# sangminwoo/SVOL

Hardware: AMD Instinct MI355X
Metric: frames/sec (fwd+matcher+bwd), T=32·P=196·d=256 (higher is better)
Workload: dtype bf16

## Files before the change

include/svol_hip.h:

```cpp
#ifndef SVOL_HIP_H
#define SVOL_HIP_H

#include <stdint.h>

#ifdef __cplusplus
extern "C" {
#endif

#define SVOL_F32 0
#define SVOL_BF16 1
#define SVOL_F16 2

#define SVOL_OK 0
#define SVOL_E_INVALID (-1)
#define SVOL_E_UNSUPPORTED (-2)
#define SVOL_E_LAUNCH (-3)

#define SVOL_ACT_NONE 0
#define SVOL_ACT_RELU 1
#define SVOL_ACT_GELU 2
#define SVOL_ACT_SIGMOID 3
#define SVOL_ACT_GELU_D 5
#define SVOL_ACT_RELU_RES 4

int svol_abi_version(void);
const char* svol_strerror(int code);

int svol_cast(const void* src, int dtype_src, void* dst, int dtype_dst, int64_t n, void* stream);
int svol_cast_transpose(const float* src, void* dst, void* dstT, int dtype, int64_t R, int64_t C, void* stream);
int svol_cast_transpose_multi(const void* descs, int32_t n_desc, int64_t total_tiles, int dtype, void* stream);
int svol_cast_split(const float* src, int64_t ld_src, void* dst_hilo, int64_t R, int64_t C, void* stream);

int svol_adamw_flat(float* p, const float* g, float* m, float* v, int64_t n, float lr, float beta1, float beta2, float eps,
                    float weight_decay, int64_t step, float grad_scale, void* stream);
int svol_adamw_flat_zero(float* p, float* g, float* m, float* v, int64_t n, float lr, float beta1, float beta2, float eps,
                         float weight_decay, int64_t step, float grad_scale, void* stream);
int svol_grad_finite(const float* g, int64_t n, float* scaler_state, void* stream);
int svol_adamw_flat_scaled(float* p, const float* g, float* m, float* v, int64_t n, float lr, float beta1, float beta2, float eps,
                           float weight_decay, float grad_mul, const float* scaler_state, void* stream);
int svol_loss_scaler_update(float* scaler_state, float growth_factor, float backoff_factor, int64_t growth_interval, float min_scale,
                            float max_scale, void* stream);
int svol_sgd_flat(float* p, const float* g, float* buf, int64_t n, float lr, float momentum, float weight_decay, float grad_scale,
                  void* stream);
int svol_sgd_flat_zero(float* p, float* g, float* buf, int64_t n, float lr, float momentum, float weight_decay, float grad_scale,
                       void* stream);
int svol_sgd_flat_scaled(float* p, const float* g, float* buf, int64_t n, float lr, float momentum, float weight_decay, float grad_mul,
                         const float* scaler_state, void* stream);
int svol_adam_flat(float* p, const float* g, float* m, float* v, int64_t n, float lr, float beta1, float beta2, float eps,
                   float weight_decay, int64_t step, float grad_scale, void* stream);
int svol_adam_flat_zero(float* p, float* g, float* m, float* v, int64_t n, float lr, float beta1, float beta2, float eps,
                        float weight_decay, int64_t step, float grad_scale, void* stream);
int svol_adam_flat_scaled(float* p, const float* g, float* m, float* v, int64_t n, float lr, float beta1, float beta2, float eps,
                          float weight_decay, float grad_mul, const float* scaler_state, void* stream);
int64_t svol_grad_sqnorm_ws_bytes(int64_t n);
int svol_grad_sqnorm(const float* g, int64_t n, float* ws, float* out, void* stream);
int svol_grad_clip_state(const float* sq, int32_t nb, float grad_mul, float max_norm, float loss_scale, int64_t steps_taken,
                         float* scaler_state, float* state_out, void* stream);
int svol_sgd_flat_grouped(float* p, float* g, float* buf, int64_t n, const int32_t* seg_end, const int32_t* seg_group, int32_t nseg,
                          const float* hyper, int32_t ngroups, const float* state, float grad_mul, int zero, void* stream);
int svol_adam_flat_grouped(float* p, float* g, float* m, float* v, int64_t n, const int32_t* seg_end, const int32_t* seg_group,
                           int32_t nseg, const float* hyper, int32_t ngroups, const float* state, const float* step_count,
                           float grad_mul, int zero, void* stream);
int svol_adamw_flat_grouped(float* p, float* g, float* m, float* v, int64_t n, const int32_t* seg_end, const int32_t* seg_group,
                            int32_t nseg, const float* hyper, int32_t ngroups, const float* state, const float* step_count,
                            float grad_mul, int zero, void* stream);
int svol_flat_step_advance(float* step_count, const float* state, void* stream);

int svol_gemm_nt(const void* A, int64_t lda, const void* A2, int64_t n_split, const void* B, int64_t ldb,
                 void* C, int64_t ldc, const float* bias, const float* colscale, int act, void* pre_act_out,
                 int64_t ldp, const void* residual, int64_t ldr, int out_f32, int64_t M, int64_t N, int64_t K,
                 int dtype, void* stream);
int svol_gemm_nt_split(const void* A, int64_t lda, const void* W_hilo, int64_t ldw, void* C, int64_t ldc, const float* bias,
                       int64_t M, int64_t N, int64_t K, void* stream);
int svol_gemm_nt_dgelu(const void* A, int64_t lda, const void* B, int64_t ldb, void* C, int64_t ldc,
                       const void* pre, int64_t ldp, float* colsum, int64_t M, int64_t N, int64_t K, int dtype,
                       void* stream);
int svol_gemm_nt_dact(const void* A, int64_t lda, const void* B, int64_t ldb, void* C, int64_t ldc,
                      const void* aux, int64_t ldaux, int act, float* colsum, int64_t M, int64_t N, int64_t K,
                      int dtype, void* stream);

int svol_gemm_tn(const void* A, int64_t lda, const void* B, int64_t ldb, float* C, int64_t ldc, float* colsum,
                 int64_t Mc, int64_t N, int64_t K, int dtype, void* stream);
#define SVOL_TN_GROUP_MAX 6
typedef struct svol_tn_problem {
    const void* A; int64_t lda;
    const void* B; int64_t ldb;
    float* C; int64_t ldc;
    float* colsum;
    int64_t Mc, N, K;
} svol_tn_problem;
int svol_gemm_tn_grouped(const svol_tn_problem* problems, int32_t n, int dtype, void* stream);
int svol_colsum(const void* X, int64_t ldx, float* out, int64_t M, int64_t N, int dtype, void* stream);
int svol_act_bwd(const void* dy, const void* aux, void* dpre, int act, int64_t n, int dtype, void* stream);

int svol_layernorm_fwd(const void* x, int x_f32, const float* gamma, const float* beta, float* y32, void* y,
                       void* ypos, const void* pos, int64_t pos_rows, float* mean, float* rstd, int64_t M, int64_t D,
                       float dropout_p, uint64_t seed, const int64_t* seed_offset_dev, int dtype, void* stream);
int svol_layernorm_bwd(const float* dy32, const void* dy, const void* dy2, const void* x, int x_f32,
                       const float* gamma, const float* mean, const float* rstd, float* dx32, void* dx,
                       float* dgamma, float* dbeta, float* dx_colsum, int64_t M, int64_t D, float dropout_p,
                       uint64_t seed, const int64_t* seed_offset_dev, int dtype, void* stream);

int svol_dropout(const void* x, void* y, int64_t n, int64_t row_len, float p, uint64_t seed, int dtype, void* stream);
int svol_dropout_add(const float* t32, const float* res32, float* out32, int64_t n, int64_t row_len, float p, uint64_t seed, void* stream);
int svol_dropout_sd(const void* x, void* y, int64_t n, int64_t row_len, float p, uint64_t seed, const int64_t* seed_step_dev, int dtype,
                    void* stream);
int svol_dropout_add_sd(const float* t32, const float* res32, float* out32, int64_t n, int64_t row_len, float p, uint64_t seed,
                        const int64_t* seed_step_dev, void* stream);

int svol_posenc_sine(const float* mask, void* pos, int64_t B, int64_t L, int64_t D, int dtype, void* stream);

int64_t svol_attn_ws_bytes(int64_t B, int64_t H, int64_t Lq, int64_t Lk, int64_t dh);
int svol_attn_fwd(const void* q, int64_t ldq, const void* k, int64_t ldk, const void* v, int64_t ldv, void* o,
                  int64_t ldo, float* lse2, const float* kbias, int64_t B, int64_t H, int64_t Lq, int64_t Lk,
                  int64_t dh, float scale, float q_premul, void* ws, int64_t ws_bytes, int dtype, void* stream);
int svol_attn_bwd(const void* q, int64_t ldq, const void* k, int64_t ldk, const void* v, int64_t ldv, const void* o,
                  int64_t ldo, const void* d_o, int64_t lddo, const float* lse2, float* delta, const float* kbias,
                  void* dq, int64_t lddq, void* dk, int64_t lddk, void* dv, int64_t lddv, int64_t B, int64_t H,
                  int64_t Lq, int64_t Lk, int64_t dh, float scale, float q_premul, void* ws, int64_t ws_bytes,
                  int dtype, void* stream);

#define SVOL_ATTN_DQ_PREZEROED 1
int64_t svol_attn_bwd_sp_image_bytes(int64_t B, int64_t H, int64_t Lq, int64_t Lk, int64_t dh, int64_t ws_bytes, int dtype);
int svol_attn_bwd_zero_ws(void* ws, int64_t ws_bytes, int64_t B, int64_t H, int64_t Lq, int64_t Lk, int64_t dh, int dtype, void* stream);
int svol_attn_bwd_ex(const void* q, int64_t ldq, const void* k, int64_t ldk, const void* v, int64_t ldv, const void* o,
                     int64_t ldo, const void* d_o, int64_t lddo, const float* lse2, float* delta, const float* kbias,
                     void* dq, int64_t lddq, void* dk, int64_t lddk, void* dv, int64_t lddv, int64_t B, int64_t H,
                     int64_t Lq, int64_t Lk, int64_t dh, float scale, float q_premul, void* ws, int64_t ws_bytes,
                     int dtype, int flags, void* ev_prep, void* stream);

int svol_attn_fwd_dropout(const void* q, int64_t ldq, const void* k, int64_t ldk, const void* v, int64_t ldv, void* o,
                          int64_t ldo, float* lse2, const float* kbias, int64_t B, int64_t H, int64_t Lq, int64_t Lk,
                          int64_t dh, float scale, float q_premul, void* ws, int64_t ws_bytes, float dropout_p, uint64_t seed,
                          int dtype, void* stream);
int svol_attn_bwd_dropout(const void* q, int64_t ldq, const void* k, int64_t ldk, const void* v, int64_t ldv, const void* o,
                          int64_t ldo, const void* d_o, int64_t lddo, const float* lse2, float* delta, const float* kbias,
                          void* dq, int64_t lddq, void* dk, int64_t lddk, void* dv, int64_t lddv, int64_t B, int64_t H,
                          int64_t Lq, int64_t Lk, int64_t dh, float scale, float q_premul, void* ws, int64_t ws_bytes,
                          float dropout_p, uint64_t seed, int dtype, void* stream);
int svol_attn_fwd_dropout_sd(const void* q, int64_t ldq, const void* k, int64_t ldk, const void* v, int64_t ldv, void* o,
                             int64_t ldo, float* lse2, const float* kbias, int64_t B, int64_t H, int64_t Lq, int64_t Lk,
                             int64_t dh, float scale, float q_premul, void* ws, int64_t ws_bytes, float dropout_p, uint64_t seed,
                             const int64_t* seed_step_dev, int dtype, void* stream);
int svol_attn_bwd_dropout_sd(const void* q, int64_t ldq, const void* k, int64_t ldk, const void* v, int64_t ldv, const void* o,
                             int64_t ldo, const void* d_o, int64_t lddo, const float* lse2, float* delta, const float* kbias,
                             void* dq, int64_t lddq, void* dk, int64_t lddk, void* dv, int64_t lddv, int64_t B, int64_t H,
                             int64_t Lq, int64_t Lk, int64_t dh, float scale, float q_premul, void* ws, int64_t ws_bytes,
                             float dropout_p, uint64_t seed, const int64_t* seed_step_dev, int dtype, void* stream);

int svol_gate_fwd(const float* x32, const void* pos, const float* u, const float* gamma, const float* beta,
                  float* y32, void* y, void* ypos, float* a, float* mean, float* rstd, float* ws, int64_t B,
                  int64_t L, int64_t D, int64_t H, int dtype, void* stream);
int svol_gate_bwd(const float* dy32, const void* dy, const void* dy2, const float* x32, const void* pos,
                  const float* u, const float* gamma, const float* a, const float* mean, const float* rstd,
                  const float* ws, float* ws2, float* dx32, float* du, float* dgamma, float* dbeta, int64_t B,
                  int64_t L, int64_t D, int64_t H, int dtype, void* stream);

int svol_layernorm_gate_scores_fwd(const float* x32, const float* gamma, const float* beta, float* y32, void* y, void* ypos,
                                   const void* pos, float* mean, float* rstd, const float* u_next, float* scores_next,
                                   int64_t B, int64_t L, int64_t D, int64_t H, int dtype, void* stream);
int svol_gate_fwd_scored(const float* x32, const void* pos, const float* u, const float* gamma, const float* beta,
                         float* y32, void* y, void* ypos, float* a, float* mean, float* rstd, float* ws, int64_t B,
                         int64_t L, int64_t D, int64_t H, int dtype, void* stream);

int svol_gate_vectors_fwd(const float* skch, const float* W_in, const float* b_in, float* q_out, float* u_out, int64_t B, int64_t D,
                          int64_t H, void* stream);
int svol_gate_vectors_bwd(const float* du, const float* skch, const float* W_in, const float* q, float* dq_ws, float* dskch,
                          float* dW_in, float* db_in, int64_t B, int64_t D, int64_t H, void* stream);
#define SVOL_GATE_VEC_MAX_LAYERS 8
int svol_gate_vectors_fwd_multi(const float* skch, const float* const* W_in, const float* const* b_in, float* const* q_out,
                                float* const* u_out, int64_t n_layers, int64_t B, int64_t D, int64_t H, void* stream);
int svol_gate_vectors_bwd_multi(const float* const* du, const float* skch, const float* const* W_in, const float* const* q,
                                float* const* dq_ws, float* const* dskch, float* const* dW_in, float* const* db_in, int64_t n_layers,
// ... 109 lines not shown
#define SVOL_DIM_F 5
#define SVOL_DIM_DTYPE 6
#define SVOL_DIM_QDTYPE 7
#define SVOL_DIM_ATTN_WS_BYTES 8
#define SVOL_DIM_COUNT 9

#define SVOL_BLK_VIDEO_HALF 0
#define SVOL_BLK_QUERY_SELF 1
#define SVOL_BLK_QUERY_CROSS 2
const char* svol_block_slot_names(int block);
int svol_block_trace_dump(char* buf, int64_t cap);
int svol_clock_probe(uint64_t* samples, int32_t* count, int32_t max_samples, const int32_t* stop, int64_t period_us,
                     int64_t max_ms, int32_t* wall_khz, void* stream);


#define SVOL_VH_SLOTS(X) \
    X(X32) X(POS) X(U) X(G1) X(BT1) X(G2) X(BT2) X(G3) X(BT3) X(B_IN) X(B_O) X(B_FC1) X(B_FC2) X(QSCALE) \
    X(W_IN) X(WV_HILO) X(W_O) X(W_FC1) X(W_FC2) X(W_IN_T) X(W_O_T) X(W_FC1_T) X(W_FC2_T) \
    X(Y1) X(Y1POS) X(A) X(MEAN1) X(RSTD1) X(GATE_WS) X(GATE_PRE) X(U_NEXT) X(GATE_WS_NEXT) \
    X(QKV) X(O) X(LSE) X(S2) X(Y2) X(MEAN2) X(RSTD2) X(PRE) X(HID) X(S3) \
    X(MEAN3) X(RSTD3) X(M32) X(M) X(MPOS) X(Y1_32) X(Y2_32) X(ATTN_WS) \
    X(DM32) X(DM) X(DMPOS) X(DS32_3) X(DS3) X(DPRE) X(DY2) X(DS32_2) X(G2D) X(DO) X(DQKV) X(DELTA) X(DXQP) X(DXQ) X(GATE_WS2) \
    X(DX32) X(DU) \
    X(DG1) X(DBT1) X(DG2) X(DBT2) X(DG3) X(DBT3) X(DW_IN) X(DB_IN) X(DW_O) X(DB_O) X(DW_FC1) X(DB_FC1) X(DW_FC2) X(DB_FC2) \
    X(EV_A0) X(EV_A1) X(EV_CLEAN_IN) X(EV_PREP) X(ATTN_WS_NEXT) X(ZERO_STREAM) X(EV_CLEAN_OUT)
#define SVOL_QS_SLOTS(X) \
    X(O32) X(O) X(OPOS) X(QPOS) X(B_IN) X(B_O) X(G4) X(BT4) X(QSCALE) X(W_IN) X(WV_HILO) X(W_O) X(W_IN_T) X(W_O_T) \
    X(QKV) X(OA) X(LSE) X(S4) X(MEAN4) X(RSTD4) X(Y32) X(Y) X(YPOS) X(ATTN_WS) \
    X(DY32) X(DY) X(DYPOS) X(G) X(DOA) X(DQKV) X(DELTA) X(DO32) X(DXQ) X(DXQP) X(DQPOS) \
    X(DW_IN) X(DB_IN) X(DW_O) X(DB_O) X(DG4) X(DBT4)
#define SVOL_QC_SLOTS(X) \
    X(O32) X(O) X(OPOS) X(MV) X(MPOS) X(KBIAS) X(QPOS) X(B_IN) X(B_O) X(G5) X(BT5) X(B_FC1) X(B_FC2) X(G6) X(BT6) X(QSCALE) \
    X(W_INQ) X(W_INQ_T) X(W_KV) X(W_KV_T) X(WV_HILO) X(W_O) X(W_O_T) X(W_FC1) X(W_FC1_T) X(W_FC2) X(W_FC2_T) \
    X(Q) X(QC) X(KV) X(OA) X(OAQ) X(LSE) X(S5) X(Y5_32) X(Y5) X(MEAN5) X(RSTD5) X(PRE) X(HID) X(S6) X(MEAN6) X(RSTD6) \
    X(Y32) X(Y) X(YPOS) X(ATTN_WS) \
    X(DY32) X(DY) X(DYPOS) X(DS32_6) X(DS6) X(DPRE) X(DY5) X(DS32_5) X(G5D) X(DOAQ) X(DOA) X(DQC) X(DQ) X(DKV) X(DELTA) \
    X(DO32) X(DXQP) X(DMPOS) X(DMV) X(DQPOS) \
    X(DW_IN) X(DB_IN) X(DW_O) X(DB_O) X(DG5) X(DBT5) X(DW_FC1) X(DB_FC1) X(DW_FC2) X(DB_FC2) X(DG6) X(DBT6)
#define SVOL_SLOT_ENUM_VH(n) SVOL_VH_##n,
#define SVOL_SLOT_ENUM_QS(n) SVOL_QS_##n,
#define SVOL_SLOT_ENUM_QC(n) SVOL_QC_##n,
enum { SVOL_VH_SLOTS(SVOL_SLOT_ENUM_VH) SVOL_VH_COUNT };
enum { SVOL_QS_SLOTS(SVOL_SLOT_ENUM_QS) SVOL_QS_COUNT };
enum { SVOL_QC_SLOTS(SVOL_SLOT_ENUM_QC) SVOL_QC_COUNT };

int svol_video_half_fwd(const int64_t* dims, void* const* slots, void* stream);
int svol_video_half_bwd(const int64_t* dims, void* const* slots, int phase, void* stream);
int svol_video_half_wgrad(const int64_t* dims, void* const* slots, void* stream);
int svol_video_half_wgrad_part(const int64_t* dims, void* const* slots, int part, void* stream);
int svol_query_self_fwd(const int64_t* dims, void* const* slots, void* stream);
int svol_query_self_bwd(const int64_t* dims, void* const* slots, void* stream);
int svol_query_self_wgrad(const int64_t* dims, void* const* slots, void* stream);
int svol_query_cross_fwd(const int64_t* dims, void* const* slots, void* stream);
int svol_query_cross_bwd(const int64_t* dims, void* const* slots, void* stream);
int svol_query_cross_wgrad(const int64_t* dims, void* const* slots, void* stream);

#ifdef __cplusplus
}
#endif
#endif
```

svol_amd/_lib.py:

```python
from __future__ import annotations

import ctypes
import os

_HERE = os.path.dirname(os.path.abspath(__file__))
LIB_PATH = os.path.join(_HERE, 'libsvol_hip.so')

_p = ctypes.c_void_p
_i64 = ctypes.c_int64
_i32 = ctypes.c_int32
_int = ctypes.c_int
_f32 = ctypes.c_float
_u64 = ctypes.c_uint64

SIGNATURES = {
    'svol_block_trace_dump': [ctypes.c_char_p, _i64],
    'svol_lsap_solve': [_p, _i64, _i64, _p, _p],
    'svol_heads_fwd': [_p] * 13 + [_i64, _i64, _p],
    'svol_heads_bwd': [_p] * 17 + [_i64, _i64, _p],
    'svol_set_loss_bwd': [_p] * 6 + [_i64, _i64, _p],
    'svol_weighted_total': [_p, _p, _i64, _p, _p],
    'svol_weighted_total_bwd': [_p, _p, _i64, _p, _p],
    'svol_cast': [_p, _int, _p, _int, _i64, _p],
    'svol_cast_transpose': [_p, _p, _p, _int, _i64, _i64, _p],
# ... 60 lines not shown
    'svol_attn_small_fwd_h16': [_p, _i64, _p, _i64, _p, _i64, _p, _i64, _i64, _i64, _i64, _i64, _f32, _int, _p],
    'svol_attn_small_fwd_lse_h16': [_p, _i64, _p, _i64, _p, _i64, _p, _i64, _p, _i64, _i64, _i64, _i64, _f32, _int, _p],
    'svol_attn_small_bwd_h16': [_p, _i64, _p, _i64, _p, _i64, _p, _i64, _p, _i64, _p, _p, _i64, _p, _i64, _p, _i64, _i64, _i64, _i64,
                                _i64, _f32, _int, _p],
    'svol_attn_cls_fwd_h16': [_p, _i64, _p, _i64, _p, _i64, _p, _i64, _p, _i64, _i64, _i64, _i64, _f32, _int, _p],
    'svol_attn_cls_bwd_h16': [_p, _i64, _p, _i64, _p, _i64, _p, _i64, _p, _i64, _p, _p, _i64, _p, _i64, _p, _i64, _i64, _i64, _i64,
                              _i64, _f32, _int, _p],
    'svol_softmax_xent': [_p, _i64, _p, _p, _p, _i64, _p, _i64, _i64, _p],
    'svol_posenc_sine': [_p, _p, _i64, _i64, _i64, _int, _p],
    'svol_attn_ws_bytes': [_i64, _i64, _i64, _i64, _i64],
    'svol_attn_fwd': [_p, _i64, _p, _i64, _p, _i64, _p, _i64, _p, _p, _i64, _i64, _i64, _i64, _i64, _f32, _f32, _p, _i64,
                      _int, _p],
    'svol_attn_bwd': [_p, _i64, _p, _i64, _p, _i64, _p, _i64, _p, _i64, _p, _p, _p, _p, _i64, _p, _i64, _p, _i64,
                      _i64, _i64, _i64, _i64, _i64, _f32, _f32, _p, _i64, _int, _p],
    'svol_attn_bwd_ex': [_p, _i64, _p, _i64, _p, _i64, _p, _i64, _p, _i64, _p, _p, _p, _p, _i64, _p, _i64, _p, _i64,
                         _i64, _i64, _i64, _i64, _i64, _f32, _f32, _p, _i64, _int, _int, _p, _p],
    'svol_attn_bwd_sp_image_bytes': [_i64, _i64, _i64, _i64, _i64, _i64, _int],
    'svol_attn_bwd_zero_ws': [_p, _i64, _i64, _i64, _i64, _i64, _i64, _int, _p],
    'svol_attn_fwd_dropout': [_p, _i64, _p, _i64, _p, _i64, _p, _i64, _p, _p, _i64, _i64, _i64, _i64, _i64, _f32, _f32, _p, _i64,
                              _f32, _u64, _int, _p],
    'svol_attn_bwd_dropout': [_p, _i64, _p, _i64, _p, _i64, _p, _i64, _p, _i64, _p, _p, _p, _p, _i64, _p, _i64, _p, _i64,
                              _i64, _i64, _i64, _i64, _i64, _f32, _f32, _p, _i64, _f32, _u64, _int, _p],
    'svol_dropout': [_p, _p, _i64, _i64, _f32, _u64, _int, _p],
    'svol_dropout_add': [_p, _p, _p, _i64, _i64, _f32, _u64, _p],
    'svol_attn_fwd_dropout_sd': [_p, _i64, _p, _i64, _p, _i64, _p, _i64, _p, _p, _i64, _i64, _i64, _i64, _i64, _f32, _f32, _p, _i64,
                                 _f32, _u64, _p, _int, _p],
    'svol_attn_bwd_dropout_sd': [_p, _i64, _p, _i64, _p, _i64, _p, _i64, _p, _i64, _p, _p, _p, _p, _i64, _p, _i64, _p, _i64,
                                 _i64, _i64, _i64, _i64, _i64, _f32, _f32, _p, _i64, _f32, _u64, _p, _int, _p],
    'svol_dropout_sd': [_p, _p, _i64, _i64, _f32, _u64, _p, _int, _p],
    'svol_dropout_add_sd': [_p, _p, _p, _i64, _i64, _f32, _u64, _p, _p],
    'svol_gate_fwd': [_p, _p, _p, _p, _p, _p, _p, _p, _p, _p, _p, _p, _i64, _i64, _i64, _i64, _int, _p],
    'svol_gate_bwd': [_p, _p, _p, _p, _p, _p, _p, _p, _p, _p, _p, _p, _p, _p, _p, _p, _i64, _i64, _i64, _i64, _int,
                      _p],
    'svol_clock_probe': [_p, _p, _int, _p, _i64, _i64, _p, _p],
    'svol_gate_fwd_scored': [_p, _p, _p, _p, _p, _p, _p, _p, _p, _p, _p, _p, _i64, _i64, _i64, _i64, _int, _p],
    'svol_layernorm_gate_scores_fwd': [_p, _p, _p, _p, _p, _p, _p, _p, _p, _p, _p, _i64, _i64, _i64, _i64, _int, _p],
    'svol_gate_vectors_fwd': [_p, _p, _p, _p, _p, _i64, _i64, _i64, _p],
    'svol_gate_vectors_bwd': [_p, _p, _p, _p, _p, _p, _p, _p, _i64, _i64, _i64, _p],
    'svol_gate_vectors_fwd_multi': [_p, _p, _p, _p, _p, _i64, _i64, _i64, _i64, _p],
    'svol_gate_vectors_bwd_multi': [_p, _p, _p, _p, _p, _p, _p, _p, _i64, _i64, _i64, _i64, _p],
    'svol_match_cost': [_p, _p, _p, _p, _p, _p, _p, _p, _p, _i32, _f32, _f32, _f32, _p, _p],
    'svol_lsap_batched': [_p, _p, _p, _p, _p, _p, _p, _p, _i32, _i32, _p],
    'svol_set_loss': [_p, _p, _p, _p, _p, _p, _p, _p, _i32, _i32, _f32, _p, _i32, _p, _p, _i32, _p],
    'svol_video_half_fwd': [_p, _p, _p],
    'svol_video_half_bwd': [_p, _p, _int, _p],
    'svol_video_half_wgrad': [_p, _p, _p],
    'svol_video_half_wgrad_part': [_p, _p, _int, _p],
    'svol_query_self_fwd': [_p, _p, _p],
    'svol_query_self_bwd': [_p, _p, _p],
    'svol_query_self_wgrad': [_p, _p, _p],
    'svol_query_cross_fwd': [_p, _p, _p],
    'svol_query_cross_bwd': [_p, _p, _p],
    'svol_query_cross_wgrad': [_p, _p, _p],
}



class TnProblem(ctypes.Structure):
    _fields_ = [('A', _p), ('lda', _i64), ('B', _p), ('ldb', _i64), ('C', _p), ('ldc', _i64), ('colsum', _p),
                ('Mc', _i64), ('N', _i64), ('K', _i64)]


_LIB = None


class SvolHipError(RuntimeError):
    pass


def lib():
    global _LIB
    if _LIB is None:
        if not os.path.exists(LIB_PATH):
            raise SvolHipError(
                f'{LIB_PATH} not found: the SVOL hot path has no CPU fallback. '
                'Build it with `python -m svol_amd.build` (hipcc, gfx950).')
        L = ctypes.CDLL(LIB_PATH)
        L.svol_abi_version.restype = _int
        L.svol_abi_version.argtypes = []
        L.svol_strerror.restype = ctypes.c_char_p
        L.svol_strerror.argtypes = [_int]
        for name, at in SIGNATURES.items():
            f = getattr(L, name)
            f.restype = _int
            f.argtypes = at
        L.svol_attn_ws_bytes.restype = _i64
        L.svol_attn_bwd_sp_image_bytes.restype = _i64
        L.svol_grad_sqnorm_ws_bytes.restype = _i64
        L.svol_block_slot_names.restype = ctypes.c_char_p
        L.svol_block_slot_names.argtypes = [_int]
        _LIB = L
    return _LIB


def check(rc: int, name: str):
    if rc != 0:
        msg = lib().svol_strerror(rc).decode()
        raise SvolHipError(f'{name} failed: {msg} (code {rc})')
```

svol_amd/blocks.py:

```python
from __future__ import annotations

import ctypes
import math
import os
import weakref

import torch

from . import _lib, layers, ops, params, wgrad

ENABLED = os.environ.get('SVOL_NO_BLOCKS') is None
GATE_SCORES_FUSE = os.environ.get('SVOL_GATE_SCORES_FUSE') is not None
VH, QS, QC = 0, 1, 2
_F32, _BF16 = 0, 1
_ESZ = {torch.float32: 4, torch.bfloat16: 2, torch.float16: 2}
_SLOTS = {}


def _slots(block):
    m = _SLOTS.get(block)
    if m is None:
        names = _lib.lib().svol_block_slot_names(block).decode().rstrip(',').split(',')
        m = _SLOTS[block] = {n: i for i, n in enumerate(names)}
    return m
# ... 446 lines not shown
        e, R = _ESZ[qdt], B * N
        o32_, o_, opos_, qpos_ = _c(o32), _c(o), _c(opos), _c(qpos)
        assert o32_.dtype == torch.float32 and o_.dtype == qdt and opos_.dtype == qdt and qpos_.dtype == qdt
        wsb = ops.attn_ws_bytes(qdt, B, H, N, N, D // H)
        lay = _open(ctx, pl, QS, (B, N, D, H, qdt), _dims(B, 0, N, D, H, 0, qdt, qdt, wsb), len(params), o.device,
                    lambda: [('QKV', R * 3 * D * e), ('OA', R * D * e), ('LSE', B * H * N * 4), ('S4', R * D * 4), ('MEAN4', R * 4),
                             ('RSTD4', R * 4), ('Y32', R * D * 4), ('Y', R * D * e), ('YPOS', R * D * e)],
                    lambda: [('ATTN_WS', max(wsb, 16))], O32=o32_, O=o_, OPOS=opos_, QPOS=qpos_)
        _call('svol_query_self_fwd', ctx)
        ctx.shape = (B, N, D, H)
        ctx.save_for_backward(o32_, o_, opos_, qpos)
        return (lay.view(ctx.arena, 'Y32', torch.float32, (B, N, D)), lay.view(ctx.arena, 'Y', qdt, (B, N, D)),
                lay.view(ctx.arena, 'YPOS', qdt, (B, N, D)))

    @staticmethod
    def backward(ctx, dy32, dy, dypos):
        if dy32 is None and dy is None and dypos is None:
            return _no_grads(ctx, 5)
        B, N, D, H = ctx.shape
        o32_, o_, opos_, qpos = ctx.saved_tensors
        qdt = ctx.pl.qdt
        e, R = _ESZ[qdt], B * N
        gq = _qpos_target(ctx, qpos, ctx.needs_input_grad[4], N, D)
        lay, tmp, bufs, gs = _open_bwd(ctx, o_.device, lambda: [('G', R * D * e), ('DOA', R * D * e), ('DQKV', R * 3 * D * e),
                                                               ('DELTA', 3 * B * H * N * 4), ('DO32', R * D * 4), ('DXQ', R * D * e),
                                                               ('DXQP', R * D * e)], DY32=dy32, DY=dy, DYPOS=dypos)
        _call('svol_query_self_bwd', ctx)
        pg = _close_bwd(ctx, 'svol_query_self_wgrad', bufs, [ctx.arena, tmp, o_, opos_], 5)
        v = lambda n_, dt_: lay.view(tmp, n_, dt_, (B, N, D))
        return (None, v('DO32', torch.float32), v('DXQ', qdt), v('DXQP', qdt), _qpos_grad(gq, qdt)) + pg


def query_self(layer, out, qpos, dt, qdt):
    pl = plan(layer, QS, dt, qdt)
    o32, o, opos = out
    return QuerySelfFn.apply(pl, o32, o, opos, qpos, *pl.inputs(o32, o, opos))


def _qc_fwd_layout(B, N, L, D, H, F, e, qe):
    R, M = B * N, B * L
    return [('Q', R * D * qe), ('QC', R * D * e), ('KV', M * 2 * D * e), ('OA', R * D * e), ('OAQ', R * D * qe), ('LSE', B * H * N * 4),
            ('S5', R * D * 4), ('Y5_32', R * D * 4), ('Y5', R * D * qe), ('MEAN5', R * 4), ('RSTD5', R * 4), ('PRE', R * F * qe),
            ('HID', R * F * qe), ('S6', R * D * 4), ('MEAN6', R * 4), ('RSTD6', R * 4), ('Y32', R * D * 4), ('Y', R * D * qe),
            ('YPOS', R * D * qe)]


def _qc_bwd_layout(B, N, L, D, H, F, e, qe, merged):
    R, M = B * N, B * L
    return [('DS32_6', R * D * 4), ('DS6', R * D * qe), ('DPRE', R * F * qe), ('DY5', R * D * qe), ('G5D', R * D * qe), ('DOAQ', R * D * qe),
            ('DOA', R * D * e), ('DQC', R * D * e), ('DQ', R * D * qe), ('DKV', M * 2 * D * e), ('DELTA', 3 * B * H * N * 4),
            ('DO32', R * D * 4), ('DXQP', R * D * qe)] + ([] if merged else [('DMPOS', M * D * e)]) + [('DMV', M * D * e)]


class QueryCrossFn(torch.autograd.Function):

    @staticmethod
    def forward(ctx, pl, o32, o, opos, mv, mpos, kbias, qpos, merged, *params):
        B, N, D = o.shape
        L = mv.shape[1]
        layer = pl.layer()
        H, F = layer.nhead, layer.mlp2.fc1.weight.shape[0]
        dt, qdt = pl.dt, pl.qdt
        e, qe = _ESZ[dt], _ESZ[qdt]
        o32_, o_, opos_, mv_, mpos_, kb_, qpos_ = _c(o32), _c(o), _c(opos), _c(mv), _c(mpos), _c(kbias), _c(qpos)
        assert o32_.dtype == torch.float32 and o_.dtype == qdt and opos_.dtype == qdt and qpos_.dtype == qdt
        assert mv_.dtype == dt and mpos_.dtype == dt and kb_.dtype == torch.float32
        wsb = ops.attn_ws_bytes(dt, B, H, N, L, D // H)
        lay = _open(ctx, pl, QC, (B, N, L, D, H, F, dt, qdt, merged), _dims(B, L, N, D, H, F, dt, qdt, wsb), len(params), o.device,
                    lambda: _qc_fwd_layout(B, N, L, D, H, F, e, qe), lambda: [('ATTN_WS', max(wsb, 16))],
                    O32=o32_, O=o_, OPOS=opos_, MV=mv_, MPOS=mpos_, KBIAS=kb_, QPOS=qpos_)
        _call('svol_query_cross_fwd', ctx)
        ctx.shape = (B, N, L, D, H, F)
        ctx.merged = merged
        ctx.save_for_backward(o32_, o_, opos_, mv_, mpos_, kb_, qpos)
        return (lay.view(ctx.arena, 'Y32', torch.float32, (B, N, D)), lay.view(ctx.arena, 'Y', qdt, (B, N, D)),
                lay.view(ctx.arena, 'YPOS', qdt, (B, N, D)))

    @staticmethod
    def backward(ctx, dy32, dy, dypos):
        if dy32 is None and dy is None and dypos is None:
            return _no_grads(ctx, 9)
        B, N, L, D, H, F = ctx.shape
        o32_, o_, opos_, mv_, mpos_, kb_, qpos = ctx.saved_tensors
        dt, qdt = ctx.pl.dt, ctx.pl.qdt
        gq = _qpos_target(ctx, qpos, ctx.needs_input_grad[7], N, D)
        lay, tmp, bufs, gs = _open_bwd(ctx, o_.device, lambda: _qc_bwd_layout(B, N, L, D, H, F, _ESZ[dt], _ESZ[qdt], ctx.merged),
                                       DY32=dy32, DY=dy, DYPOS=dypos)
        _call('svol_query_cross_bwd', ctx)
        pg = _close_bwd(ctx, 'svol_query_cross_wgrad', bufs, [ctx.arena, tmp, opos_, mv_, mpos_], 9)
        vq = lambda n_, dt_: lay.view(tmp, n_, dt_, (B, N, D))
        vm = lambda n_: lay.view(tmp, n_, dt, (B, L, D))
        return (None, vq('DO32', torch.float32), None, vq('DXQP', qdt), vm('DMV'), None if ctx.merged else vm('DMPOS'), None,
                _qpos_grad(gq, qdt), None) + pg


def query_cross(layer, out, mv, mpos, kbias, qpos, dt, qdt):
    pl = plan(layer, QC, dt, qdt)
    o32, o, opos = out
    fn = mv.grad_fn
    merged = fn is not None and fn is mpos.grad_fn and isinstance(fn, VideoHalfFn._backward_cls)
    return QueryCrossFn.apply(pl, o32, o, opos, mv, mpos, kbias, qpos, merged, *pl.inputs(o32, opos, mv, mpos))


def trace_dump() -> str:
    buf = ctypes.create_string_buffer(1 << 20)
    _lib.check(_lib.lib().svol_block_trace_dump(buf, len(buf)), 'svol_block_trace_dump')
    return buf.value.decode()
```

svol_amd/csrc/attention.hip:

```cpp
#include "attn_call.h"

namespace {

constexpr float LOG2E = 1.4426950408889634f;

template <typename T_, int ND_> struct AT {
    typedef T_ T;
    static constexpr int ND = ND_;
    static constexpr bool H = sizeof(T) == 2;
    static_assert(ND == 2 || (ND == 1 && !H), "instances: <float, 1>, <float, 2>, <bf16_t, 2>, <f16_t, 2>");
    static constexpr int EPC = H ? 8 : 4, CPR = (H ? 4 : 8) * ND, NA1 = (H ? 2 : 4) * ND, NA2 = H ? 2 : 4;
    static constexpr int NAT_ROW = (H ? 64 : 128) * ND, TR_STRIDE = H ? 64 * 2 + 16 : 64 * 4 + 16;
    static constexpr int NAT = 64 * NAT_ROW, TR = 32 * ND * TR_STRIDE;
};

template <typename W>
__device__ __forceinline__ int nat_off(int row, int ch) {
    return row * W::NAT_ROW + ((ch ^ (row & (W::CPR - 1))) << 4);
}

template <typename W>
__device__ __forceinline__ void stage_tile(char* nat, char* tr, const typename W::T* g, int64_t ld, int row0, int limit, int dh, int tid) {
    constexpr int EPC = W::EPC, CPR = W::CPR, ST = W::TR_STRIDE;
    for (int c = tid; c < 64 * CPR; c += 256) {
// ... 518 lines not shown
    c.drop_p = dropout_p; c.drop_seed = seed; c.drop_step = seed_step_dev; c.stream = reinterpret_cast<hipStream_t>(stream);
    if (const int rc = check_call(c, false, B, H, Lq, Lk, dh, dtype)) return rc;
    if (dh > 32) return dtype == SVOL_BF16 ? fwd_launch<bf16_t, 2>(c) : dtype == SVOL_F16 ? fwd_launch<f16_t, 2>(c) : fwd_launch<float, 2>(c);
    if (svol_is16(dtype)) return (dtype == SVOL_BF16 ? svol_attn_fwd_bf16_launch : svol_attn_fwd_f16_launch)(c);
    return fwd_launch<float, 1>(c);
}
int svol_attn_fwd_dropout(const void* q, int64_t ldq, const void* k, int64_t ldk, const void* v, int64_t ldv, void* o,
                          int64_t ldo, float* lse2, const float* kbias, int64_t B, int64_t H, int64_t Lq, int64_t Lk, int64_t dh,
                          float scale, float q_premul, void* ws, int64_t ws_bytes, float dropout_p, uint64_t seed, int dtype,
                          void* stream) {
    return svol_attn_fwd_dropout_sd(q, ldq, k, ldk, v, ldv, o, ldo, lse2, kbias, B, H, Lq, Lk, dh, scale, q_premul, ws, ws_bytes,
                                    dropout_p, seed, nullptr, dtype, stream);
}
int svol_attn_fwd(const void* q, int64_t ldq, const void* k, int64_t ldk, const void* v, int64_t ldv, void* o,
                  int64_t ldo, float* lse2, const float* kbias, int64_t B, int64_t H, int64_t Lq, int64_t Lk, int64_t dh,
                  float scale, float q_premul, void* ws, int64_t ws_bytes, int dtype, void* stream) {
    return svol_attn_fwd_dropout(q, ldq, k, ldk, v, ldv, o, ldo, lse2, kbias, B, H, Lq, Lk, dh, scale, q_premul, ws, ws_bytes, 0.f, 0,
                                 dtype, stream);
}

static int attn_bwd_impl(const void* q, int64_t ldq, const void* k, int64_t ldk, const void* v, int64_t ldv, const void* o,
                         int64_t ldo, const void* d_o, int64_t lddo, const float* lse2, float* delta, const float* kbias, void* dq,
                         int64_t lddq, void* dk, int64_t lddk, void* dv, int64_t lddv, int64_t B, int64_t H, int64_t Lq, int64_t Lk,
                         int64_t dh, float scale, float q_premul, void* ws, int64_t ws_bytes, float drop_p, uint64_t drop_seed,
                         const int64_t* drop_step, int dtype, void* stream, int flags = 0, void* ev_prep = nullptr) {
    AttnCall c{};
    c.q = q; c.k = k; c.v = v; c.o = o; c.d_o = d_o; c.lse2 = const_cast<float*>(lse2); c.delta = delta; c.kbias = kbias;
    c.dq = dq; c.dk = dk; c.dv = dv;
    c.ldq = ldq; c.ldk = ldk; c.ldv = ldv; c.ldo = ldo; c.lddo = lddo; c.lddq = lddq; c.lddk = lddk; c.lddv = lddv;
    c.scale = scale; c.premul = q_premul; c.ws = static_cast<float*>(ws); c.ws_bytes = ws_bytes;
    c.drop_p = drop_p; c.drop_seed = drop_seed; c.drop_step = drop_step; c.flags = flags; c.ev_prep = ev_prep; c.stream = reinterpret_cast<hipStream_t>(stream);
    if (const int rc = check_call(c, true, B, H, Lq, Lk, dh, dtype)) return rc;
    if (dh > 32) return dtype == SVOL_BF16 ? bwd_launch<bf16_t, 2>(c) : dtype == SVOL_F16 ? bwd_launch<f16_t, 2>(c) : bwd_launch<float, 2>(c);
    if (svol_is16(dtype)) return (dtype == SVOL_BF16 ? svol_attn_bwd_bf16_launch : svol_attn_bwd_f16_launch)(c);
    return bwd_launch<float, 1>(c);
}

int svol_attn_bwd(const void* q, int64_t ldq, const void* k, int64_t ldk, const void* v, int64_t ldv, const void* o,
                  int64_t ldo, const void* d_o, int64_t lddo, const float* lse2, float* delta, const float* kbias, void* dq,
                  int64_t lddq, void* dk, int64_t lddk, void* dv, int64_t lddv, int64_t B, int64_t H, int64_t Lq, int64_t Lk,
                  int64_t dh, float scale, float q_premul, void* ws, int64_t ws_bytes, int dtype, void* stream) {
    return attn_bwd_impl(q, ldq, k, ldk, v, ldv, o, ldo, d_o, lddo, lse2, delta, kbias, dq, lddq, dk, lddk, dv, lddv, B, H, Lq, Lk, dh,
                         scale, q_premul, ws, ws_bytes, 0.f, 0, nullptr, dtype, stream);
}
int svol_attn_bwd_ex(const void* q, int64_t ldq, const void* k, int64_t ldk, const void* v, int64_t ldv, const void* o,
                     int64_t ldo, const void* d_o, int64_t lddo, const float* lse2, float* delta, const float* kbias, void* dq,
                     int64_t lddq, void* dk, int64_t lddk, void* dv, int64_t lddv, int64_t B, int64_t H, int64_t Lq, int64_t Lk,
                     int64_t dh, float scale, float q_premul, void* ws, int64_t ws_bytes, int dtype, int flags, void* ev_prep,
                     void* stream) {
    if (flags & ~SVOL_ATTN_DQ_PREZEROED) return SVOL_E_INVALID;
    return attn_bwd_impl(q, ldq, k, ldk, v, ldv, o, ldo, d_o, lddo, lse2, delta, kbias, dq, lddq, dk, lddk, dv, lddv, B, H, Lq, Lk, dh,
                         scale, q_premul, ws, ws_bytes, 0.f, 0, nullptr, dtype, stream, flags, ev_prep);
}
int64_t svol_attn_bwd_sp_image_bytes(int64_t B, int64_t H, int64_t Lq, int64_t Lk, int64_t dh, int64_t ws_bytes, int dtype) {
    if (!svol_is16(dtype) || dh > 32 || check_common(B, H, Lq, Lk, dh, dtype)) return 0;
    return (dtype == SVOL_BF16 ? svol_attn_sp_image_bytes_bf16 : svol_attn_sp_image_bytes_f16)((int)B, (int)H, (int)Lq, (int)Lk, (int)dh,
                                                                                              ws_bytes);
}
int svol_attn_bwd_zero_ws(void* ws, int64_t ws_bytes, int64_t B, int64_t H, int64_t Lq, int64_t Lk, int64_t dh, int dtype, void* stream) {
    if (!ws || !aligned16(ws)) return SVOL_E_INVALID;
    if (!svol_is16(dtype)) return SVOL_E_UNSUPPORTED;
    const int rc = check_common(B, H, Lq, Lk, dh, dtype);
    if (rc) return rc;
    if (dh > 32) return SVOL_E_UNSUPPORTED;
    return (dtype == SVOL_BF16 ? svol_attn_sp_zero_bf16_launch : svol_attn_sp_zero_f16_launch)(
        static_cast<float*>(ws), ws_bytes, (int)B, (int)H, (int)Lq, (int)Lk, (int)dh, reinterpret_cast<hipStream_t>(stream));
}
int svol_attn_bwd_dropout(const void* q, int64_t ldq, const void* k, int64_t ldk, const void* v, int64_t ldv, const void* o,
                          int64_t ldo, const void* d_o, int64_t lddo, const float* lse2, float* delta, const float* kbias, void* dq,
                          int64_t lddq, void* dk, int64_t lddk, void* dv, int64_t lddv, int64_t B, int64_t H, int64_t Lq, int64_t Lk,
                          int64_t dh, float scale, float q_premul, void* ws, int64_t ws_bytes, float dropout_p, uint64_t seed,
                          int dtype, void* stream) {
    return attn_bwd_impl(q, ldq, k, ldk, v, ldv, o, ldo, d_o, lddo, lse2, delta, kbias, dq, lddq, dk, lddk, dv, lddv, B, H, Lq, Lk, dh,
                         scale, q_premul, ws, ws_bytes, dropout_p, seed, nullptr, dtype, stream);
}
int svol_attn_bwd_dropout_sd(const void* q, int64_t ldq, const void* k, int64_t ldk, const void* v, int64_t ldv, const void* o,
                             int64_t ldo, const void* d_o, int64_t lddo, const float* lse2, float* delta, const float* kbias,
                             void* dq, int64_t lddq, void* dk, int64_t lddk, void* dv, int64_t lddv, int64_t B, int64_t H, int64_t Lq,
                             int64_t Lk, int64_t dh, float scale, float q_premul, void* ws, int64_t ws_bytes, float dropout_p,
                             uint64_t seed, const int64_t* seed_step_dev, int dtype, void* stream) {
    return attn_bwd_impl(q, ldq, k, ldk, v, ldv, o, ldo, d_o, lddo, lse2, delta, kbias, dq, lddq, dk, lddk, dv, lddv, B, H, Lq, Lk, dh,
                         scale, q_premul, ws, ws_bytes, dropout_p, seed, seed_step_dev, dtype, stream);
}

}
```

svol_amd/csrc/attention_bf16.hip:

```cpp
#include <cstdint>
#include <cstdlib>

#include "attn_call.h"

namespace {

constexpr float LOG2E = 1.4426950408889634f;
constexpr int KT = 128;
constexpr int IMG = KT * 64;
constexpr float LAZY_THR = 4.0f;

struct Args {
    const void *q, *k, *v, *o, *d_o;
    void *out_o, *dq, *dk, *dv;
    const float* kbias;
    float *lse2, *delta;
    int64_t ldq, ldk, ldv, ldo, lddo, lddq, lddk, lddv;
    int B, H, Lq, Lk, dh;
    float scale;
    float premul;
    int ksplit, tiles_per_split;
    float *ws_o, *ws_ml, *ws_dq;
    const int* tile_flags;
    int head_xcd, nxt;
    int tail_last;
    int* redo;
    unsigned *nl2, *nd2;
    float drop_p, drop_inv;
    uint64_t drop_seed;
    const int64_t* drop_step;
    int dq_rot;
};
__device__ __forceinline__ float attn_drop(uint64_t seed, uint64_t row, int key, float p, float inv) {
    return dropout_scale(seed, row, (uint32_t)key, p, inv);
}
__device__ __forceinline__ void attn_drop2(uint32_t rowmix, int key0, uint32_t thr16, float inv, float& s0, float& s1) {
    const uint32_t bits = drop_bits(rowmix, (uint32_t)key0 >> 1);
    s0 = drop_pick(bits, 0u, thr16, inv);
    s1 = drop_pick(bits, 1u, thr16, inv);
}

typedef __attribute__((address_space(3))) h16x4* lds_bf16x4_ptr;

__device__ __forceinline__ int img_off(int row, int ch) { return row * 64 + ((ch ^ ((row >> 2) & 3)) << 4); }

struct Stage { uint4 v[2]; };

__device__ __forceinline__ void load_regs(Stage& s, const h16_t* g, int64_t ld, int row0, int limit, int dh, int tid) {
#pragma unroll
    for (int i = 0; i < 2; ++i) {
        const int c = tid + 256 * i, row = c >> 2, ch = c & 3;
        s.v[i] = (row0 + row < limit && ch * 8 < dh) ? *reinterpret_cast<const uint4*>(g + (int64_t)(row0 + row) * ld + ch * 8)
                                                      : make_uint4(0, 0, 0, 0);
    }
}
__device__ __forceinline__ void store_lds(char* img, const Stage& s, int tid) {
#pragma unroll
    for (int i = 0; i < 2; ++i) {
        const int c = tid + 256 * i, row = c >> 2, ch = c & 3;
        *reinterpret_cast<uint4*>(img + img_off(row, ch)) = s.v[i];
    }
}

typedef __attribute__((address_space(3))) void* lds_vptr;
typedef const __attribute__((address_space(1))) void* gbl_vptr;
__device__ __forceinline__ void dma_piece(char* img, const h16_t* g, int64_t ld, int row0, int piece, int lane) {
    const int row = 16 * piece + (lane >> 2);
    const int ch = (lane & 3) ^ ((lane >> 4) & 3);
    const h16_t* src = g + (int64_t)(row0 + row) * ld + ch * 8;
    __builtin_amdgcn_global_load_lds((gbl_vptr)src, (lds_vptr)(img + piece * 1024), 16, 0, 0);
}
__device__ __forceinline__ void dma_tile(char* img, const h16_t* g, int64_t ld, int row0, int wave, int lane) {
    dma_piece(img, g, ld, row0, 2 * wave, lane);
    dma_piece(img, g, ld, row0, 2 * wave + 1, lane);
}
__device__ __forceinline__ void dma_wait_all() { asm volatile("s_waitcnt vmcnt(0)" ::: "memory"); }
__device__ __forceinline__ void dma_piece_async(char* img, const h16_t* g, int64_t ld, int row0, int piece, int lane) {
    const int row = 16 * piece + (lane >> 2);
    const int ch = (lane & 3) ^ ((lane >> 4) & 3);
    const h16_t* src = g + (int64_t)(row0 + row) * ld + ch * 8;
    const unsigned dst = __builtin_amdgcn_readfirstlane((unsigned)(size_t)(lds_vptr)(img + piece * 1024));
    asm volatile("s_mov_b32 m0, %0\n\tglobal_load_lds_dwordx4 %1, off" ::"s"(dst), "v"(src) : "m0");
}
__device__ __forceinline__ void dma_tile_async(char* img, const h16_t* g, int64_t ld, int row0, int wave, int lane) {
// ... 192 lines not shown
        l += (ls[0] + ls[1]) + (ls[2] + ls[3]);
        if (p.drop_p > 0.f) {
            const uint32_t rm = drop_row(drop_seed32(dseed), (((uint64_t)b * p.H + hh) * p.Lq + (qvalid ? qrow : 0)));
            const uint32_t thr = drop_thr16(p.drop_p);
#pragma unroll
            for (int sub = 0; sub < 4; ++sub)
#pragma unroll
                for (int g = 0; g < 4; ++g)
#pragma unroll
                    for (int e = 0; e < 4; e += 2) {
                        float s0, s1;
                        attn_drop2(rm, t * KT + sub * 32 + 8 * g + 4 * h + e, thr, p.drop_inv, s0, s1);
                        S[sub][4 * g + e] *= s0;
                        S[sub][4 * g + e + 1] *= s1;
                    }
        }
#pragma unroll
        for (int sub = 0; sub < 4; ++sub) {
            uint4 va[2];
            read_tr(va, vimg, sub, lane);
            mma_second(O, va, S[sub]);
        }
        if (t + 1 < nt) {
            store_lds(sK + (cur ^ 1) * IMG, sk, tid);
            store_lds(sV + (cur ^ 1) * IMG, sv, tid);
            if (MASKED) stage_bias(sB + (cur ^ 1) * KT, kb, (t + 1) * KT, p.Lk, tid);
        }
        __syncthreads();
    }
    const float lt = l + __shfl_xor(l, 32, 64);
    const float m2 = MASKED ? m : m * c;
    if (p.ksplit > 1) {
        if (qvalid) {
            float* wo = p.ws_o + (((int64_t)sp * p.B + b) * p.Lq + qrow) * (p.H * p.dh) + hh * p.dh;
#pragma unroll
            for (int g = 0; g < 4; ++g) {
                const int d0 = 8 * g + 4 * h;
                if (d0 < p.dh) *reinterpret_cast<f32x4*>(wo + d0) = f32x4{O[4 * g], O[4 * g + 1], O[4 * g + 2], O[4 * g + 3]};
            }
            if (h == 0) {
                float* wm = p.ws_ml + ((((int64_t)sp * p.B + b) * p.H + hh) * p.Lq + qrow) * 2;
                wm[0] = m2;
                wm[1] = lt;
            }
        }
        return;
    }
    const float inv = lt > 0.f ? 1.f / lt : 0.f;
    h16_t* Oo = reinterpret_cast<h16_t*>(p.out_o) + (int64_t)b * p.Lq * p.ldo + hh * p.dh;
    store_acc(O, Oo, p.ldo, qrow, qvalid, p.dh, h, inv);
    if (qvalid && h == 0) p.lse2[((int64_t)b * p.H + hh) * p.Lq + qrow] = m2 + __builtin_amdgcn_logf(lt);
}

__global__ void attn_combine_bf16(Args p) {
    const int64_t idx = (int64_t)blockIdx.x * blockDim.x + threadIdx.x;
    const int64_t total = (int64_t)p.B * p.Lq * p.H;
    if (idx >= total) return;
    const int hh = (int)(idx % p.H);
    const int64_t row = idx / p.H;
    const int b = (int)(row / p.Lq), q = (int)(row % p.Lq);
    float M = -INFINITY;
    for (int i = 0; i < p.ksplit; ++i) M = fmaxf(M, p.ws_ml[((((int64_t)i * p.B + b) * p.H + hh) * p.Lq + q) * 2]);
    float L = 0.f, acc[32];
#pragma unroll
    for (int d = 0; d < 32; ++d) acc[d] = 0.f;
    for (int i = 0; i < p.ksplit; ++i) {
        const float* ml = p.ws_ml + ((((int64_t)i * p.B + b) * p.H + hh) * p.Lq + q) * 2;
        if (ml[0] == -INFINITY) continue;
        const float w = __builtin_amdgcn_exp2f(ml[0] - M);
        L += w * ml[1];
        const float* po = p.ws_o + (((int64_t)i * p.B + b) * p.Lq + q) * (p.H * p.dh) + hh * p.dh;
#pragma unroll
        for (int d = 0; d < 32; d += 4) {
            if (d < p.dh) {
                const f32x4 t = *reinterpret_cast<const f32x4*>(po + d);
#pragma unroll
                for (int e = 0; e < 4; ++e) acc[d + e] += w * t[e];
            }
        }
    }
    const float inv = L > 0.f ? 1.f / L : 0.f;
    h16_t* o = reinterpret_cast<h16_t*>(p.out_o) + row * p.ldo + hh * p.dh;
#pragma unroll
    for (int d = 0; d < 32; d += 4) {
        if (d < p.dh) {
            h16x4 v;
#pragma unroll
            for (int e = 0; e < 4; ++e) v[e] = (h16_t)(acc[d + e] * inv);
            *reinterpret_cast<h16x4*>(o + d) = v;
        }
    }
    p.lse2[((int64_t)b * p.H + hh) * p.Lq + q] = M + __builtin_amdgcn_logf(L);
}

__global__ void attn_delta_bf16(Args p) {
    const int64_t idx = (int64_t)blockIdx.x * blockDim.x + threadIdx.x;
    const int64_t total = (int64_t)p.B * p.Lq * p.H;
    if (idx >= total) return;
    const int hh = (int)(idx % p.H);
    const int64_t row = idx / p.H;
    const int b = (int)(row / p.Lq), q = (int)(row % p.Lq);
    const h16_t* o = reinterpret_cast<const h16_t*>(p.o) + row * p.ldo + hh * p.dh;
    const h16_t* d = reinterpret_cast<const h16_t*>(p.d_o) + row * p.lddo + hh * p.dh;
    float s = 0.f;
    for (int i = 0; i < p.dh; i += 8) {
        const h16x8 a = *reinterpret_cast<const h16x8*>(o + i), c = *reinterpret_cast<const h16x8*>(d + i);
#pragma unroll
        for (int e = 0; e < 8; ++e) s += (float)a[e] * (float)c[e];
    }
    p.delta[((int64_t)b * p.H + hh) * p.Lq + q] = s;
    if (p.ksplit > 1) {
        float* z = p.ws_dq + row * (p.H * p.dh) + hh * p.dh;
        for (int i = 0; i < p.dh; i += 4) *reinterpret_cast<f32x4*>(z + i) = f32x4{0.f, 0.f, 0.f, 0.f};
    }
}

__global__ void attn_dq_finish_bf16(Args p) {
    const int64_t idx = (int64_t)blockIdx.x * blockDim.x + threadIdx.x;
    const int64_t total = (int64_t)p.B * p.Lq * p.H;
    if (idx >= total) return;
    const int hh = (int)(idx % p.H);
    const int64_t row = idx / p.H;
    const float* z = p.ws_dq + row * (p.H * p.dh) + hh * p.dh;
    h16_t* o = reinterpret_cast<h16_t*>(p.dq) + row * p.lddq + hh * p.dh;
    for (int i = 0; i < p.dh; i += 4) {
        const f32x4 t = *reinterpret_cast<const f32x4*>(z + i);
        h16x4 v;
#pragma unroll
        for (int e = 0; e < 4; ++e) v[e] = (h16_t)(t[e] * p.scale);
        *reinterpret_cast<h16x4*>(o + i) = v;
    }
}

template <bool MASKED>
__global__ __launch_bounds__(256, 2) void attn_bwd_dq_bf16(Args p) {
    const uint64_t dseed = drop_seed_at(p.drop_seed, p.drop_step);
    __shared__ __attribute__((aligned(16))) char smem[4 * IMG + 2 * KT * 4];
    char* sK = smem;
    char* sV = smem + 2 * IMG;
    float* sB = reinterpret_cast<float*>(smem + 4 * IMG);

    const int tid = threadIdx.x, lane = tid & 63, wave = tid >> 6;
    const int r = lane & 31, h = lane >> 5;
    const int b = blockIdx.z, hh = blockIdx.y;
    const int qt = blockIdx.x / p.ksplit, sp = blockIdx.x % p.ksplit;
    const int qrow = qt * 128 + wave * 32 + r;
    const bool qvalid = qrow < p.Lq;
    const h16_t* Q = reinterpret_cast<const h16_t*>(p.q) + (int64_t)b * p.Lq * p.ldq + hh * p.dh;
    const h16_t* dO = reinterpret_cast<const h16_t*>(p.d_o) + (int64_t)b * p.Lq * p.lddo + hh * p.dh;
    const h16_t* K = reinterpret_cast<const h16_t*>(p.k) + (int64_t)b * p.Lk * p.ldk + hh * p.dh;
    const h16_t* V = reinterpret_cast<const h16_t*>(p.v) + (int64_t)b * p.Lk * p.ldv + hh * p.dh;
    const float* kb = p.kbias ? p.kbias + (int64_t)b * p.Lk : nullptr;
    const float c = p.premul != 0.f ? 1.f : p.scale * LOG2E;

    uint4 qb[2], dob[2];
    load_lane_block(qb, Q, p.ldq, qrow, qvalid, p.dh, h);
    load_lane_block(dob, dO, p.lddo, qrow, qvalid, p.dh, h);
    const int64_t sidx = ((int64_t)b * p.H + hh) * p.Lq + qrow;
    const float nlse = qvalid ? -p.lse2[sidx] : -INFINITY;
    const float dl = qvalid ? p.delta[sidx] : 0.f;

    f32x16 dQ = zero16();
    const int t0 = sp * p.tiles_per_split;
    const int nt = min((p.Lk + KT - 1) / KT, t0 + p.tiles_per_split);
    Stage sk, sv;
    load_regs(sk, K, p.ldk, t0 * KT, p.Lk, p.dh, tid);
    load_regs(sv, V, p.ldv, t0 * KT, p.Lk, p.dh, tid);
    store_lds(sK, sk, tid);
    store_lds(sV, sv, tid);
    if (MASKED) stage_bias(sB, kb, t0 * KT, p.Lk, tid);
    __syncthreads();

    for (int t = t0; t < nt; ++t) {
        const int cur = (t - t0) & 1;
        if (t + 1 < nt) {
            load_regs(sk, K, p.ldk, (t + 1) * KT, p.Lk, p.dh, tid);
            load_regs(sv, V, p.ldv, (t + 1) * KT, p.Lk, p.dh, tid);
        }
        const char* kimg = sK + cur * IMG;
        const char* vimg = sV + cur * IMG;
        const float* bias = sB + cur * KT;
#pragma unroll 2
        for (int sub = 0; sub < 4; ++sub) {
// ... 1994 lines not shown
    const int hx = (pl.pre && (B * H) % 8 == 0) ? (((B * H) % 16 == 0 && H % 2 == 0 && dh == 32) ? 2 : 1) : 0;
    auto grid = [&](int nx) {
        return hx ? Grid{dim3((unsigned)(B * H * nx)), hx, nx, 0} : Grid{dim3((unsigned)nx, (unsigned)H, (unsigned)B), 0, 0, 0};
    };
    pl.gf = grid(nq128 * pl.fwd_ksplit);
    pl.gq = pl.pre ? grid((Lq + 255) / 256) : grid(nq128 * pl.bwd_ksplit);
    if (hx) pl.gq.tail_last = (Lq % 256 >= 1 && Lq % 256 <= 128 && pl.gq.nxt > 1) ? 1 : 0;
    pl.gk = grid((Lk + 127) / 128);
    if (pl.pre && pl.masked) pl.fwd = Fwd::pre_masked;
    else if (pl.pre) pl.fwd = (hx && dh == 32 && ws && ws_bytes >= 4 * pl.need_redo) ? Fwd::fast2_redo : Fwd::pre_all;
    else if (pl.fwd_ksplit > 1) pl.fwd = pl.masked ? Fwd::ksplit_m : Fwd::ksplit_u;
    else pl.fwd = pl.masked ? Fwd::general_m : Fwd::general_u;
    if (pl.pre && pl.masked) pl.bwd = Bwd::bwd_pre_masked;
    else if (pl.pre && hx && sp_shape && ws && ws_bytes >= 4 * pl.need_sp) pl.bwd = Bwd::bwd_sp;
    else if (pl.pre && dh == 32) pl.bwd = Lq % KT == 0 ? Bwd::bwd_rot_dma : Bwd::bwd_rot;
    else if (pl.pre) pl.bwd = Bwd::bwd_pre;
    else if (!no_fewq && !det && pl.bwd_ksplit > 1 && Lq <= KT && dh == 32 && !dropout) pl.bwd = kbias ? Bwd::fq_m : Bwd::fq_u;
    else pl.bwd = pl.masked ? Bwd::two_pass_m : Bwd::two_pass_u;
    const int chunks = min(ntk, max(1, 512 / (B * H)));
    pl.fq_tps = (ntk + chunks - 1) / chunks;
    pl.fq_grid = dim3((unsigned)((ntk + pl.fq_tps - 1) / pl.fq_tps), (unsigned)H, (unsigned)B);
    return pl;
}
static Plan attn_plan(const AttnCall& c) {
    return attn_plan(c.B, c.H, c.Lq, c.Lk, c.dh, c.premul != 0.f, c.kbias != nullptr, c.drop_p > 0.f, c.ws != nullptr, c.ws_bytes);
}
int64_t svol_attn_ws_floats_bf16(int B, int H, int Lq, int Lk, int dh) {
    return attn_plan(B, H, Lq, Lk, dh, false, false, false,  false, 0).need;
}
static bool sp_planned(int B, int H, int Lq, int Lk, int dh, bool ws, int64_t ws_bytes) {
    return attn_plan(B, H, Lq, Lk, dh,  true,  false,  false, ws, ws_bytes).bwd == Bwd::bwd_sp;
}
int64_t svol_attn_sp_image_bytes_bf16(int B, int H, int Lq, int Lk, int dh, int64_t ws_bytes) {
    return sp_planned(B, H, Lq, Lk, dh, true, ws_bytes) ? (int64_t)B * Lq * H * 32 * 4 : 0;
}
constexpr int SP_ZERO_WGS = 64;
int svol_attn_sp_zero_bf16_launch(float* ws, int64_t ws_bytes, int B, int H, int Lq, int Lk, int dh, hipStream_t s) {
    if (!sp_planned(B, H, Lq, Lk, dh, ws != nullptr, ws_bytes)) return SVOL_E_UNSUPPORTED;
    const int64_t n4 = (int64_t)B * Lq * H * 32 / 4;
    const int64_t want = (n4 + 255) / 256;
    hipLaunchKernelGGL(attn_sp_zero_image, dim3((unsigned)(want < SP_ZERO_WGS ? want : SP_ZERO_WGS)), dim3(256), 0, s, ws, n4);
    return hipGetLastError() == hipSuccess ? SVOL_OK : SVOL_E_LAUNCH;
}
static Args make_args(const AttnCall& c, int ksplit, int tiles_per_split, const Grid& g) {
    Args p{};
    attn_fill(p, c);
    p.ksplit = ksplit; p.tiles_per_split = tiles_per_split;
    if (ksplit > 1) {
        p.ws_o = c.ws;
        p.ws_ml = p.ws_o + (int64_t)p.ksplit * p.B * p.Lq * p.H * p.dh;
        p.ws_dq = p.ws_ml + (int64_t)p.ksplit * p.B * p.H * p.Lq * 2;
    }
    p.head_xcd = g.head_xcd; p.nxt = g.nxt; p.tail_last = g.tail_last;
    return p;
}

int svol_attn_fwd_bf16_launch(const AttnCall& c) {
    const Plan pl = attn_plan(c);
    Args p = make_args(c, pl.fwd_ksplit, pl.fwd_tps, pl.gf);
    const dim3 grid = pl.gf.dim, wg(256);
    hipStream_t s = c.stream;
    switch (pl.fwd) {
    case Fwd::pre_masked:
        p.tile_flags = reinterpret_cast<const int*>(c.ws);
        hipLaunchKernelGGL(attn_tile_flags_bf16, dim3((unsigned)pl.ntk, (unsigned)c.B), dim3(64), 0, s, c.kbias, c.Lk, pl.ntk, reinterpret_cast<int*>(c.ws));
        hipLaunchKernelGGL(attn_fwd_bf16_pre_masked, grid, wg, 0, s, p);
        break;
    case Fwd::fast2_redo:
        p.redo = reinterpret_cast<int*>(c.ws);
        hipLaunchKernelGGL(attn_fwd_bf16_fast2, grid, wg, 0, s, p);
        [[fallthrough]];
    case Fwd::pre_all: hipLaunchKernelGGL(attn_fwd_bf16_pre, grid, wg, 0, s, p); break;
    case Fwd::general_m:
    case Fwd::ksplit_m: hipLaunchKernelGGL(attn_fwd_bf16<true>, grid, wg, 0, s, p); break;
    case Fwd::general_u:
    case Fwd::ksplit_u: hipLaunchKernelGGL(attn_fwd_bf16<false>, grid, wg, 0, s, p); break;
    }
    const int64_t total = (int64_t)c.B * c.Lq * c.H;
    if (pl.fwd_ksplit > 1) hipLaunchKernelGGL(attn_combine_bf16, dim3((unsigned)((total + 127) / 128)), dim3(128), 0, s, p);
    return hipGetLastError() == hipSuccess ? SVOL_OK : SVOL_E_LAUNCH;
}

int svol_attn_bwd_bf16_launch(const AttnCall& c) {
    const Plan pl = attn_plan(c);
    Args pq = make_args(c, pl.bwd_ksplit, pl.bwd_tps, pl.gq), pk = make_args(c, pl.bwd_ksplit, pl.bwd_tps, pl.gk);
    const int64_t total = (int64_t)c.B * c.Lq * c.H;
    const dim3 gd((unsigned)((total + 255) / 256)), wg(256);
    hipStream_t s = c.stream;
    auto bind_rows = [&](Args& a) { a.nl2 = reinterpret_cast<unsigned*>(c.delta + total); a.nd2 = reinterpret_cast<unsigned*>(c.delta + 2 * total); };
    void (*dq)(Args) = nullptr, (*dkdv)(Args) = nullptr;
    if (!pl.pre) hipLaunchKernelGGL(attn_delta_bf16, gd, wg, 0, s, pq);
    switch (pl.bwd) {
    case Bwd::bwd_pre_masked:
        pq.tile_flags = pk.tile_flags = reinterpret_cast<const int*>(c.ws);
        hipLaunchKernelGGL(attn_tile_flags_bf16, dim3((unsigned)pl.ntk, (unsigned)c.B), dim3(64), 0, s, c.kbias, c.Lk, pl.ntk, reinterpret_cast<int*>(c.ws));
        dq = attn_bwd_dq_bf16_pre_masked, dkdv = attn_bwd_dkdv_bf16_pre_masked;
        break;
    case Bwd::bwd_sp:
        pq.ws_dq = c.ws;
        bind_rows(pq);
        hipLaunchKernelGGL((c.flags & SVOL_ATTN_DQ_PREZEROED) ? attn_bwd_sp_prep_bf16<false> : attn_bwd_sp_prep_bf16<true>,
                           dim3((unsigned)((int64_t)c.B * c.Lq / 32)), wg, 0, s, pq);
        break;
    case Bwd::bwd_rot_dma:
        bind_rows(pq), bind_rows(pk);
        dq = attn_bwd_dq_bf16_rot, dkdv = attn_bwd_dkdv_bf16_pre_dma;
        break;
// ... 26 lines not shown
```

svol_amd/csrc/attn_call.h:

```cpp
#pragma once
#include "common.h"

struct AttnCall {
    const void *q, *k, *v, *o, *d_o;
    void *out_o, *dq, *dk, *dv;
    const float* kbias;
    float *lse2, *delta;
    int64_t ldq, ldk, ldv, ldo, lddo, lddq, lddk, lddv;
    int B, H, Lq, Lk, dh;
    float scale, premul, drop_p;
    uint64_t drop_seed;
    const int64_t* drop_step;
    float* ws;
    int64_t ws_bytes;
    int flags;
    void* ev_prep;
    hipStream_t stream;
};

template <typename A> static inline void attn_fill(A& p, const AttnCall& c) {
    p.q = c.q; p.k = c.k; p.v = c.v; p.o = c.o; p.d_o = c.d_o; p.out_o = c.out_o; p.dq = c.dq; p.dk = c.dk; p.dv = c.dv;
    p.kbias = c.kbias; p.lse2 = c.lse2; p.delta = c.delta;
    p.ldq = c.ldq; p.ldk = c.ldk; p.ldv = c.ldv; p.ldo = c.ldo; p.lddo = c.lddo; p.lddq = c.lddq; p.lddk = c.lddk; p.lddv = c.lddv;
    p.B = c.B; p.H = c.H; p.Lq = c.Lq; p.Lk = c.Lk; p.dh = c.dh; p.scale = c.scale; p.premul = c.premul;
    p.drop_p = c.drop_p; p.drop_inv = c.drop_p > 0.f ? 1.f / (1.f - c.drop_p) : 1.f; p.drop_seed = c.drop_seed; p.drop_step = c.drop_step;
}

#define SVOL_ATTN_H16_ENTRIES(T)                                                                                      \
    int svol_attn_fwd_##T##_launch(const AttnCall& c);                                                                \
    int svol_attn_bwd_##T##_launch(const AttnCall& c);                                                                \
    int64_t svol_attn_ws_floats_##T(int B, int H, int Lq, int Lk, int dh);                                            \
    int64_t svol_attn_sp_image_bytes_##T(int B, int H, int Lq, int Lk, int dh, int64_t ws_bytes);                     \
    int svol_attn_sp_zero_##T##_launch(float* ws, int64_t ws_bytes, int B, int H, int Lq, int Lk, int dh, hipStream_t s);
SVOL_ATTN_H16_ENTRIES(bf16)
SVOL_ATTN_H16_ENTRIES(f16)
#undef SVOL_ATTN_H16_ENTRIES
```

svol_amd/csrc/blocks.hip:

```cpp
#include <math.h>
#include <stdio.h>
#include <stdlib.h>
#include <string.h>

#include <map>
#include <mutex>
#include <string>
#include <vector>

#include "common.h"

namespace {

const bool kTrace = getenv("SVOL_BLOCK_TRACE") != nullptr;
struct TraceRec { const char* prog; const char* site; hipEvent_t e0, e1; };
std::mutex g_trace_mu;
std::vector<TraceRec> g_trace_log;
struct Trace {
    const char* prog;
    hipStream_t s;
    hipEvent_t last = nullptr;
    Trace* prev;
    static thread_local Trace* cur;
    Trace(const char* prog_, void* s_) : prog(prog_), s(static_cast<hipStream_t>(s_)), prev(cur) {
// ... 238 lines not shown
    if (!d.ok() || d.N <= 0) return SVOL_E_INVALID;
    const int64_t R = d.B * d.N, D = d.D, dh = D / d.H;
    const int qdt = d.qdt, xf = qdt != SVOL_F32;
#define P(n) p[SVOL_QS_##n]
    RUN(nt(P(OPOS), D, P(W_IN), D, P(QKV), 3 * D, P(B_IN), P(QSCALE), R, 2 * D, D, qdt, s));
    if (P(WV_HILO))
        RUN(svol_gemm_nt_split(P(O), D, P(WV_HILO), 2 * D, at(P(QKV), 2 * D, qdt), 3 * D, f32(P(B_IN)) + 2 * D, R, D, D, s));
    else
        RUN(nt(P(O), D, at(P(W_IN), 2 * D * D, qdt), D, at(P(QKV), 2 * D, qdt), 3 * D, f32(P(B_IN)) + 2 * D, nullptr, R, D, D, qdt, s));
    RUN(svol_attn_fwd(P(QKV), 3 * D, at(P(QKV), D, qdt), 3 * D, at(P(QKV), 2 * D, qdt), 3 * D, P(OA), D, f32(P(LSE)), nullptr, d.B, d.H,
                      d.N, d.N, dh, attn_scale(dh), attn_premul(dh, qdt), P(ATTN_WS), d.ws_bytes, qdt, s));
    RUN(nt_res(P(OA), D, P(W_O), D, P(S4), P(B_O), P(O32), R, D, D, qdt, s));
    RUN(svol_layernorm_fwd(P(S4), xf, f32(P(G4)), f32(P(BT4)), f32(P(Y32)), P(Y), P(YPOS), P(QPOS), d.N, f32(P(MEAN4)), f32(P(RSTD4)), R, D,
                           0.f, 0, nullptr, qdt, s));
    return SVOL_OK;
}

int svol_query_self_bwd(const int64_t* dims, void* const* p, void* s) {
    if (!dims || !p) return SVOL_E_INVALID;
    Trace tr_("query_self_bwd", s);
    const Dims d(dims);
    if (!d.ok() || d.N <= 0) return SVOL_E_INVALID;
    const int64_t R = d.B * d.N, D = d.D, dh = D / d.H;
    const int qdt = d.qdt, xf = qdt != SVOL_F32;
    RUN(svol_layernorm_bwd(f32(P(DY32)), P(DY), P(DYPOS), P(S4), xf, f32(P(G4)), f32(P(MEAN4)), f32(P(RSTD4)), f32(P(DO32)), P(G),
                           f32(P(DG4)), f32(P(DBT4)), f32(P(DB_O)), R, D, 0.f, 0, nullptr, qdt, s));
    if (P(DQPOS) && P(DYPOS))
        RUN(svol_colsum(P(DYPOS), d.N * D, f32(P(DQPOS)), d.B, d.N * D, qdt, s));
    RUN(nt(P(G), D, P(W_O_T), D, P(DOA), D, nullptr, nullptr, R, D, D, qdt, s));
    RUN(svol_attn_bwd(P(QKV), 3 * D, at(P(QKV), D, qdt), 3 * D, at(P(QKV), 2 * D, qdt), 3 * D, P(OA), D, P(DOA), D, f32(P(LSE)),
                      f32(P(DELTA)), nullptr, P(DQKV), 3 * D, at(P(DQKV), D, qdt), 3 * D, at(P(DQKV), 2 * D, qdt), 3 * D, d.B, d.H, d.N,
                      d.N, dh, attn_scale(dh), attn_premul(dh, qdt), P(ATTN_WS), d.ws_bytes, qdt, s));
    RUN(nt(P(DQKV), 3 * D, P(W_IN_T), 3 * D, P(DXQP), D, nullptr, nullptr, R, D, 2 * D, qdt, s));
    RUN(nt(at(P(DQKV), 2 * D, qdt), 3 * D, at(P(W_IN_T), 2 * D, qdt), 3 * D, P(DXQ), D, nullptr, nullptr, R, D, D, qdt, s));
    return SVOL_OK;
}

int svol_query_self_wgrad(const int64_t* dims, void* const* p, void* s) {
    if (!dims || !p) return SVOL_E_INVALID;
    Trace tr_("query_self_wgrad", s);
    const Dims d(dims);
    if (!d.ok()) return SVOL_E_INVALID;
    const int64_t R = d.B * d.N, D = d.D;
    const int qdt = d.qdt;
    const svol_tn_problem pr[3] = {
        {P(G), D, P(OA), D, f32(P(DW_O)), D, nullptr, R, D, D},
        {P(DQKV), 3 * D, P(OPOS), D, f32(P(DW_IN)), D, f32(P(DB_IN)), R, 2 * D, D},
        {at(P(DQKV), 2 * D, qdt), 3 * D, P(O), D, f32(P(DW_IN)) + 2 * D * D, D, f32(P(DB_IN)) + 2 * D, R, D, D}};
    RUN(svol_gemm_tn_grouped(pr, 3, qdt, s));
    return SVOL_OK;
#undef P
}

int svol_query_cross_fwd(const int64_t* dims, void* const* p, void* s) {
    if (!dims || !p) return SVOL_E_INVALID;
    Trace tr_("query_cross_fwd", s);
    const Dims d(dims);
    if (!d.ok() || d.N <= 0 || d.L <= 0 || d.F <= 0) return SVOL_E_INVALID;
    const int64_t R = d.B * d.N, M = d.B * d.L, D = d.D, F = d.F, dh = D / d.H;
    const int dt = d.dt, qdt = d.qdt, xf = qdt != SVOL_F32;
    const bool mixed = qdt != dt;
#define P(n) p[SVOL_QC_##n]
    if (mixed) {
        RUN(nt(P(OPOS), D, P(W_INQ), D, P(Q), D, P(B_IN), P(QSCALE), R, D, D, qdt, s));
        RUN(svol_cast(P(Q), qdt, P(QC), dt, R * D, s));
    } else {
        RUN(nt(P(OPOS), D, P(W_KV), D, P(QC), D, P(B_IN), P(QSCALE), R, D, D, dt, s));
    }
    RUN(nt(P(MPOS), D, at(P(W_KV), D * D, dt), D, P(KV), 2 * D, f32(P(B_IN)) + D, nullptr, M, D, D, dt, s));
    if (P(WV_HILO))
        RUN(svol_gemm_nt_split(P(MV), D, P(WV_HILO), 2 * D, at(P(KV), D, dt), 2 * D, f32(P(B_IN)) + 2 * D, M, D, D, s));
    else
        RUN(nt(P(MV), D, at(P(W_KV), 2 * D * D, dt), D, at(P(KV), D, dt), 2 * D, f32(P(B_IN)) + 2 * D, nullptr, M, D, D, dt, s));
    RUN(svol_attn_fwd(P(QC), D, P(KV), 2 * D, at(P(KV), D, dt), 2 * D, P(OA), D, f32(P(LSE)), f32(P(KBIAS)), d.B, d.H, d.N, d.L, dh,
                      attn_scale(dh), attn_premul(dh, dt), P(ATTN_WS), d.ws_bytes, dt, s));
    const void* oq = P(OA);
    if (mixed) {
        RUN(svol_cast(P(OA), dt, P(OAQ), qdt, R * D, s));
        oq = P(OAQ);
    }
    RUN(nt_res(oq, D, P(W_O), D, P(S5), P(B_O), P(O32), R, D, D, qdt, s));
    RUN(svol_layernorm_fwd(P(S5), xf, f32(P(G5)), f32(P(BT5)), f32(P(Y5_32)), P(Y5), nullptr, nullptr, 0, f32(P(MEAN5)), f32(P(RSTD5)), R,
                           D, 0.f, 0, nullptr, qdt, s));
    RUN(svol_gemm_nt(P(Y5), D, nullptr, 0, P(W_FC1), D, P(HID), F, f32(P(B_FC1)), nullptr, SVOL_ACT_GELU, P(PRE), F, nullptr, 0, 0, R, F, D,
                     qdt, s));
    RUN(nt_res(P(HID), F, P(W_FC2), F, P(S6), P(B_FC2), P(Y5_32), R, D, F, qdt, s));
    RUN(svol_layernorm_fwd(P(S6), xf, f32(P(G6)), f32(P(BT6)), f32(P(Y32)), P(Y), P(YPOS), P(QPOS), d.N, f32(P(MEAN6)), f32(P(RSTD6)), R, D,
                           0.f, 0, nullptr, qdt, s));
    return SVOL_OK;
}

int svol_query_cross_bwd(const int64_t* dims, void* const* p, void* s) {
    if (!dims || !p) return SVOL_E_INVALID;
    Trace tr_("query_cross_bwd", s);
    const Dims d(dims);
    if (!d.ok() || d.N <= 0 || d.L <= 0 || d.F <= 0) return SVOL_E_INVALID;
    const int64_t R = d.B * d.N, M = d.B * d.L, D = d.D, F = d.F, dh = D / d.H;
    const int dt = d.dt, qdt = d.qdt, xf = qdt != SVOL_F32;
    const bool mixed = qdt != dt;
    RUN(svol_layernorm_bwd(f32(P(DY32)), P(DY), P(DYPOS), P(S6), xf, f32(P(G6)), f32(P(MEAN6)), f32(P(RSTD6)), f32(P(DS32_6)), P(DS6),
                           f32(P(DG6)), f32(P(DBT6)), f32(P(DB_FC2)), R, D, 0.f, 0, nullptr, qdt, s));
    if (P(DQPOS) && P(DYPOS)) RUN(svol_colsum(P(DYPOS), d.N * D, f32(P(DQPOS)), d.B, d.N * D, qdt, s));
    RUN(svol_gemm_nt_dact(P(DS6), D, P(W_FC2_T), D, P(DPRE), F, P(PRE), F, SVOL_ACT_GELU, f32(P(DB_FC1)), R, F, D, qdt, s));
    RUN(nt(P(DPRE), F, P(W_FC1_T), F, P(DY5), D, nullptr, nullptr, R, D, F, qdt, s));
    RUN(svol_layernorm_bwd(f32(P(DS32_6)), P(DY5), nullptr, P(S5), xf, f32(P(G5)), f32(P(MEAN5)), f32(P(RSTD5)), f32(P(DO32)), P(G5D),
                           f32(P(DG5)), f32(P(DBT5)), f32(P(DB_O)), R, D, 0.f, 0, nullptr, qdt, s));
    RUN(nt(P(G5D), D, P(W_O_T), D, P(DOAQ), D, nullptr, nullptr, R, D, D, qdt, s));
    const void* d_o = P(DOAQ);
    if (mixed) {
        RUN(svol_cast(P(DOAQ), qdt, P(DOA), dt, R * D, s));
        d_o = P(DOA);
    }
    RUN(svol_attn_bwd(P(QC), D, P(KV), 2 * D, at(P(KV), D, dt), 2 * D, P(OA), D, d_o, D, f32(P(LSE)), f32(P(DELTA)), f32(P(KBIAS)), P(DQC), D,
                      P(DKV), 2 * D, at(P(DKV), D, dt), 2 * D, d.B, d.H, d.N, d.L, dh, attn_scale(dh), attn_premul(dh, dt), P(ATTN_WS),
                      d.ws_bytes, dt, s));
    if (P(DMPOS)) {
        RUN(nt(P(DKV), 2 * D, at(P(W_KV_T), D, dt), 3 * D, P(DMPOS), D, nullptr, nullptr, M, D, D, dt, s));
        RUN(nt(at(P(DKV), D, dt), 2 * D, at(P(W_KV_T), 2 * D, dt), 3 * D, P(DMV), D, nullptr, nullptr, M, D, D, dt, s));
    } else {
        RUN(nt(P(DKV), 2 * D, at(P(W_KV_T), D, dt), 3 * D, P(DMV), D, nullptr, nullptr, M, D, 2 * D, dt, s));
    }
    const void* dq = P(DQC);
    if (mixed) {
        RUN(svol_cast(P(DQC), dt, P(DQ), qdt, R * D, s));
        dq = P(DQ);
    }
    RUN(nt(dq, D, mixed ? P(W_INQ_T) : P(W_KV_T), 3 * D, P(DXQP), D, nullptr, nullptr, R, D, D, qdt, s));
    return SVOL_OK;
}

int svol_query_cross_wgrad(const int64_t* dims, void* const* p, void* s) {
    if (!dims || !p) return SVOL_E_INVALID;
    Trace tr_("query_cross_wgrad", s);
    const Dims d(dims);
    if (!d.ok()) return SVOL_E_INVALID;
    const int64_t R = d.B * d.N, M = d.B * d.L, D = d.D, F = d.F;
    const int dt = d.dt, qdt = d.qdt;
    const bool mixed = qdt != dt;
    const svol_tn_problem pv[2] = {
        {P(DKV), 2 * D, P(MPOS), D, f32(P(DW_IN)) + D * D, D, f32(P(DB_IN)) + D, M, D, D},
        {at(P(DKV), D, dt), 2 * D, P(MV), D, f32(P(DW_IN)) + 2 * D * D, D, f32(P(DB_IN)) + 2 * D, M, D, D}};
    RUN(svol_gemm_tn_grouped(pv, 2, dt, s));
    const svol_tn_problem pq[4] = {
        {P(DS6), D, P(HID), F, f32(P(DW_FC2)), F, nullptr, R, D, F},
        {P(DPRE), F, P(Y5), D, f32(P(DW_FC1)), D, nullptr, R, F, D},
        {P(G5D), D, mixed ? P(OAQ) : P(OA), D, f32(P(DW_O)), D, nullptr, R, D, D},
        {mixed ? P(DQ) : P(DQC), D, P(OPOS), D, f32(P(DW_IN)), D, f32(P(DB_IN)), R, D, D}};
    RUN(svol_gemm_tn_grouped(pq, 4, qdt, s));
    return SVOL_OK;
#undef P
}

}
```

svol_amd/csrc/common.h:

```cpp
#pragma once
#include <hip/hip_runtime.h>
#include <stdint.h>

#include "../../include/svol_hip.h"

typedef __bf16 bf16_t;
typedef __attribute__((ext_vector_type(8))) __bf16 bf16x8;
typedef __attribute__((ext_vector_type(4))) __bf16 bf16x4;
typedef __attribute__((ext_vector_type(2))) __bf16 bf16x2;
typedef _Float16 f16_t;
typedef __attribute__((ext_vector_type(8))) _Float16 f16x8;
typedef __attribute__((ext_vector_type(4))) _Float16 f16x4;
typedef __attribute__((ext_vector_type(2))) _Float16 f16x2;
typedef __attribute__((ext_vector_type(4))) float f32x4;
typedef __attribute__((ext_vector_type(16))) float f32x16;

#ifdef SVOL_H16_FP16
typedef f16_t h16_t;
typedef f16x8 h16x8;
typedef f16x4 h16x4;
typedef f16x2 h16x2;
#define SVOL_MFMA_16x16x32_H16 __builtin_amdgcn_mfma_f32_16x16x32_f16
#define SVOL_MFMA_32x32x16_H16 __builtin_amdgcn_mfma_f32_32x32x16_f16
#define SVOL_DS_READ_TR16_H16 svol_ds_read_tr16_f16
#define SVOL_H16_ASM "f16"
#define SVOL_H16_ONE2 0x3C003C00u
#define SVOL_H16_NINF_LO 0x0000FC00u
#define SVOL_H16_DTYPE SVOL_F16
#define SVOL_H16_NEG_BIG (-6.0e4f)
#define SVOL_H16_PSUM_MAX 6.5e4f
#define svol_gemm_nt_bf16_fast svol_gemm_nt_f16_fast
#define svol_gemm_tn_bf16_fast svol_gemm_tn_f16_fast
#define svol_gemm_tn_bf16_grouped svol_gemm_tn_f16_grouped
#define svol_conv_wgrad_bf16_fast svol_conv_wgrad_f16_fast
#define svol_conv_nhwc_bf16_launch svol_conv_nhwc_f16_launch
#define svol_gemm_ws_bf16 svol_gemm_ws_f16
#define svol_gemm_n256_bf16 svol_gemm_n256_f16
#define svol_attn_fwd_bf16_launch svol_attn_fwd_f16_launch
#define svol_attn_bwd_bf16_launch svol_attn_bwd_f16_launch
#define svol_attn_ws_floats_bf16 svol_attn_ws_floats_f16
#define svol_attn_sp_image_bytes_bf16 svol_attn_sp_image_bytes_f16
#define svol_attn_sp_zero_bf16_launch svol_attn_sp_zero_f16_launch
#else
typedef bf16_t h16_t;
typedef bf16x8 h16x8;
typedef bf16x4 h16x4;
typedef bf16x2 h16x2;
#define SVOL_MFMA_16x16x32_H16 __builtin_amdgcn_mfma_f32_16x16x32_bf16
#define SVOL_MFMA_32x32x16_H16 __builtin_amdgcn_mfma_f32_32x32x16_bf16
#define SVOL_DS_READ_TR16_H16 __builtin_amdgcn_ds_read_tr16_b64_v4bf16
#define SVOL_H16_ASM "bf16"
#define SVOL_H16_ONE2 0x3F803F80u
#define SVOL_H16_NINF_LO 0x0000FF80u
#define SVOL_H16_DTYPE SVOL_BF16
#define SVOL_H16_NEG_BIG (-3.0e38f)
#define SVOL_H16_PSUM_MAX 1.0e30f
#endif
typedef __attribute__((ext_vector_type(4))) short i16x4;
__device__ __forceinline__ f16x4 svol_ds_read_tr16_f16(__attribute__((address_space(3))) f16x4* p) {
    return __builtin_bit_cast(f16x4, __builtin_amdgcn_ds_read_tr16_b64_v4i16((__attribute__((address_space(3))) i16x4*)p));
}
typedef __attribute__((ext_vector_type(2))) float f32x2;
__device__ __forceinline__ h16x2 cvt_pk_h16(float a, float b) {
#ifdef SVOL_H16_FP16
    return __builtin_convertvector((f32x2){a, b}, f16x2);
#else
    return h16x2{(bf16_t)a, (bf16_t)b};
#endif
}
static inline bool svol_is16(int dtype) { return dtype == SVOL_BF16 || dtype == SVOL_F16; }

template <typename T> struct H16;
template <> struct H16<bf16_t> {
    typedef bf16x8 v8;
    typedef bf16x4 v4;
    typedef __attribute__((address_space(3))) bf16x4* lds_v4_ptr;
    static __device__ __forceinline__ f32x4 mfma16(v8 a, v8 b, f32x4 c) { return __builtin_amdgcn_mfma_f32_16x16x32_bf16(a, b, c, 0, 0, 0); }
    static __device__ __forceinline__ f32x16 mfma32(v8 a, v8 b, f32x16 c) { return __builtin_amdgcn_mfma_f32_32x32x16_bf16(a, b, c, 0, 0, 0); }
    static __device__ __forceinline__ v4 read_tr(lds_v4_ptr p) { return __builtin_amdgcn_ds_read_tr16_b64_v4bf16(p); }
    static __device__ __forceinline__ v4 cvt4(f32x4 x) { return v4{(bf16_t)x[0], (bf16_t)x[1], (bf16_t)x[2], (bf16_t)x[3]}; }
};
template <> struct H16<f16_t> {
    typedef f16x8 v8;
    typedef f16x4 v4;
    typedef __attribute__((address_space(3))) f16x4* lds_v4_ptr;
    static __device__ __forceinline__ f32x4 mfma16(v8 a, v8 b, f32x4 c) { return __builtin_amdgcn_mfma_f32_16x16x32_f16(a, b, c, 0, 0, 0); }
    static __device__ __forceinline__ f32x16 mfma32(v8 a, v8 b, f32x16 c) { return __builtin_amdgcn_mfma_f32_32x32x16_f16(a, b, c, 0, 0, 0); }
    static __device__ __forceinline__ v4 read_tr(lds_v4_ptr p) { return svol_ds_read_tr16_f16(p); }
    static __device__ __forceinline__ v4 cvt4(f32x4 x) { return __builtin_convertvector(x, f16x4); }
};

#define SVOL_CHECK_LAUNCH()                                   \
// ... 184 lines not shown
```

svol_amd/csrc/gemm.hip:

```cpp
#include "gemm_call.h"

namespace {

template <typename T> struct Tr;
template <> struct Tr<bf16_t> { static constexpr int EPC = 8; };
template <> struct Tr<f16_t> { static constexpr int EPC = 8; };
template <> struct Tr<float> { static constexpr int EPC = 4; };

__device__ __forceinline__ void mma_chunk(f32x4& acc, const uint4& a, const uint4& b, bf16_t) {
    acc = __builtin_amdgcn_mfma_f32_16x16x32_bf16(__builtin_bit_cast(bf16x8, a), __builtin_bit_cast(bf16x8, b), acc,
                                                  0, 0, 0);
}
__device__ __forceinline__ void mma_chunk(f32x4& acc, const uint4& a, const uint4& b, f16_t) {
    acc = __builtin_amdgcn_mfma_f32_16x16x32_f16(__builtin_bit_cast(f16x8, a), __builtin_bit_cast(f16x8, b), acc, 0, 0, 0);
}
__device__ __forceinline__ void mma_chunk(f32x4& acc, const uint4& a, const uint4& b, float) {
    f32x4 af = __builtin_bit_cast(f32x4, a), bf = __builtin_bit_cast(f32x4, b);
#pragma unroll
    for (int e = 0; e < 4; ++e) acc = __builtin_amdgcn_mfma_f32_16x16x4f32(af[e], bf[e], acc, 0, 0, 0);
}

struct NtArgs {
    const void* A; const void* A2; const void* B; void* C;
    const float* bias; const float* colscale; void* pre; const void* res;
// ... 336 lines not shown
        int lo = 0, hi = n_desc - 1;
        while (lo < hi) {
            const int mid = (lo + hi + 1) >> 1;
            if (descs[mid].tile_begin <= (int)blockIdx.x) lo = mid; else hi = mid - 1;
        }
        which = lo;
    }
    __syncthreads();
    const CastDesc d = descs[which];
    const int t = blockIdx.x - d.tile_begin;
    const int tx = threadIdx.x & 31, ty = threadIdx.x >> 5;
    const int r0 = (t / d.tiles_c) * 32, c0 = (t % d.tiles_c) * 32;
    T* dst = reinterpret_cast<T*>(d.dst);
    T* dstT = reinterpret_cast<T*>(d.dstT);
#pragma unroll
    for (int j = 0; j < 4; ++j) {
        const int r = r0 + ty + 8 * j, c = c0 + tx;
        float v = (r < d.R && c < d.C) ? d.src[(int64_t)r * d.C + c] : 0.f;
        tile[ty + 8 * j][tx] = v;
        if (dst && r < d.R && c < d.C) dst[(int64_t)r * d.C + c] = from_f32<T>(v);
        if (d.dstS && r < d.R && c < d.C) store_split(d.dstS, r, c, d.C, v);
    }
    __syncthreads();
    if (dstT) {
#pragma unroll
        for (int j = 0; j < 4; ++j) {
            const int c = c0 + ty + 8 * j, r = r0 + tx;
            if (r < d.R && c < d.C) dstT[(int64_t)c * d.R + r] = from_f32<T>(tile[tx][ty + 8 * j]);
        }
    }
}

template <typename T>
__global__ void act_bwd_kernel(const T* dy, const T* aux, T* dpre, int act, int64_t n) {
    int64_t i = (int64_t)blockIdx.x * blockDim.x + threadIdx.x;
    const int64_t stride = (int64_t)gridDim.x * blockDim.x;
    for (; i < n; i += stride) {
        const float g = to_f32(dy[i]), a = to_f32(aux[i]);
        float d;
        if (act == SVOL_ACT_RELU) d = a > 0.f ? g : 0.f;
        else if (act == SVOL_ACT_GELU) d = g * dgelu_f(a);
        else if (act == SVOL_ACT_GELU_D) d = g * a;
        else if (act == SVOL_ACT_SIGMOID) d = g * a * (1.f - a);
        else d = g;
        dpre[i] = from_f32<T>(d);
    }
}

struct SkArgs {
    const float* A; const float* B; float* C;
    const float* bias; const float* colscale; float* pre; const float* res; const float* aux; float* colsum;
    int64_t lda, ldb, ldc, ldp, ldr, ldaux;
    int M, N, K, act, epi;
};
constexpr int SKF_T = 32, SKF_LD = SKF_T + 4;

__global__ __launch_bounds__(256) void gemm_nt_f32_skinny(SkArgs p) {
    __shared__ __attribute__((aligned(16))) float red[4][SKF_T][SKF_LD];
    const int tid = threadIdx.x, lane = tid & 63, wave = tid >> 6;
    const int r = lane & 31, h = lane >> 5;
    const int bm = blockIdx.y * SKF_T, bn = blockIdx.x * SKF_T;
    const int kslice = p.K >> 2;
    const int nb = kslice >> 5;
    const bool va = bm + r < p.M, vb = bn + r < p.N;
    const float* pa = p.A + (int64_t)(bm + r) * p.lda + wave * kslice + h * 4;
    const float* pb = p.B + (int64_t)(bn + r) * p.ldb + wave * kslice + h * 4;
    const f32x4 z4 = f32x4{0.f, 0.f, 0.f, 0.f};
    f32x4 a[4], b[4], na[4], nb_[4];
    auto load = [&](f32x4 (&xa)[4], f32x4 (&xb)[4], int bt) {
#pragma unroll
        for (int c = 0; c < 4; ++c) {
            xa[c] = va ? *reinterpret_cast<const f32x4*>(pa + bt * 32 + c * 8) : z4;
            xb[c] = vb ? *reinterpret_cast<const f32x4*>(pb + bt * 32 + c * 8) : z4;
        }
    };
    f32x16 acc;
#pragma unroll
    for (int i = 0; i < 16; ++i) acc[i] = 0.f;
    load(a, b, 0);
    for (int bt = 0; bt < nb; ++bt) {
        if (bt + 1 < nb) load(na, nb_, bt + 1);
#pragma unroll
        for (int c = 0; c < 4; ++c)
#pragma unroll
            for (int e = 0; e < 4; ++e) acc = __builtin_amdgcn_mfma_f32_32x32x2f32(a[c][e], b[c][e], acc, 0, 0, 0);
        if (bt + 1 < nb) {
#pragma unroll
            for (int c = 0; c < 4; ++c) { a[c] = na[c]; b[c] = nb_[c]; }
        }
    }
#pragma unroll
    for (int g = 0; g < 4; ++g)
#pragma unroll
        for (int e = 0; e < 4; ++e) red[wave][8 * g + 4 * h + e][r] = acc[4 * g + e];
    __syncthreads();
    const int row = tid >> 3, c0 = (tid & 7) * 4;
    const int m = bm + row, n0 = bn + c0;
    f32x4 v = *reinterpret_cast<const f32x4*>(&red[0][row][c0]);
#pragma unroll
    for (int w = 1; w < 4; ++w) {
        const f32x4 u = *reinterpret_cast<const f32x4*>(&red[w][row][c0]);
#pragma unroll
        for (int e = 0; e < 4; ++e) v[e] += u[e];
    }
    const bool mv = m < p.M;
    if (p.epi == 0) {
        if (mv) {
#pragma unroll
            for (int e = 0; e < 4; ++e) {
                if (p.bias) v[e] += p.bias[n0 + e];
                if (p.colscale) v[e] *= p.colscale[n0 + e];
            }
            if (p.pre) {
                f32x4 sv = v;
                if (p.act == SVOL_ACT_GELU_D) {
#pragma unroll
                    for (int e = 0; e < 4; ++e) sv[e] = dgelu_f(v[e]);
                }
                *reinterpret_cast<f32x4*>(p.pre + (int64_t)m * p.ldp + n0) = sv;
            }
#pragma unroll
            for (int e = 0; e < 4; ++e) {
                if (p.act == SVOL_ACT_RELU) v[e] = fmaxf(v[e], 0.f);
                else if (act_is_gelu(p.act)) v[e] = gelu_f(v[e]);
                else if (p.act == SVOL_ACT_SIGMOID) v[e] = 1.f / (1.f + __expf(-v[e]));
            }
            if (p.res) {
                const f32x4 rr = *reinterpret_cast<const f32x4*>(p.res + (int64_t)m * p.ldr + n0);
#pragma unroll
                for (int e = 0; e < 4; ++e) v[e] += rr[e];
            }
            if (p.act == SVOL_ACT_RELU_RES) {
#pragma unroll
                for (int e = 0; e < 4; ++e) v[e] = fmaxf(v[e], 0.f);
            }
        }
    } else {
        if (mv) {
            const f32x4 x = *reinterpret_cast<const f32x4*>(p.aux + (int64_t)m * p.ldaux + n0);
#pragma unroll
            for (int e = 0; e < 4; ++e) v[e] *= p.act == SVOL_ACT_RELU ? (x[e] > 0.f ? 1.f : 0.f) : (p.act == SVOL_ACT_GELU_D ? x[e] : dgelu_f(x[e]));
        } else {
            v = f32x4{0.f, 0.f, 0.f, 0.f};
        }
        if (p.colsum) {
            __syncthreads();
            *reinterpret_cast<f32x4*>(&red[0][row][c0]) = v;
            __syncthreads();
            if (tid < SKF_T) {
                float sacc = 0.f;
#pragma unroll 8
                for (int i = 0; i < SKF_T; ++i) sacc += red[0][i][tid];
                atomicAdd(p.colsum + bn + tid, sacc);
            }
        }
    }
    if (mv) *reinterpret_cast<f32x4*>(p.C + (int64_t)m * p.ldc + n0) = v;
}

inline bool skinny_f32_ok(const GemmCall& c) {
    constexpr int64_t max_m = 2048;
    auto rows16 = [](const void* p, int64_t ld) { return !p || (ld % 4 == 0 && aligned16(p)); };
    return c.kwrap == c.K && c.M <= max_m && c.K % 128 == 0 && c.N % 32 == 0 && c.lda % 4 == 0 && c.ldb % 4 == 0 && c.ldc % 4 == 0 && aligned16(c.A) &&
           aligned16(c.B) && aligned16(c.C) && (c.M + 31) / 32 <= 65535 && rows16(c.res, c.ldr) && rows16(c.pre, c.ldp) && rows16(c.aux, c.ldaux);
}

inline int grid_1d(int64_t n, int block) {
    int64_t g = (n + block - 1) / block;
    return (int)(g > 4096 ? 4096 : (g < 1 ? 1 : g));
}

}

static int tn_generic_plan(const svol_tn_problem& q, int dtype, TnArgs& out, int64_t& wgs) {
    const int64_t Mc = q.Mc, N = q.N, K = q.K;
    const int epc = svol_is16(dtype) ? 8 : 4;
    if (N % epc || K % epc || q.lda % epc || q.ldb % epc) return SVOL_E_UNSUPPORTED;
    if (!aligned16(q.A) || !aligned16(q.B)) return SVOL_E_INVALID;
    if (Mc > (1 << 30) || N > (1 << 30) || K > (1 << 30)) return SVOL_E_UNSUPPORTED;
    const int ct = svol_is16(dtype) ? 64 : 32;
    const int64_t tiles = ((N + 127) / 128) * ((K + 127) / 128);
    constexpr int small_wgs = 64;
    const int target_wgs = (dtype == SVOL_F32 && Mc <= 4096) ? small_wgs : (tiles <= 8 ? 256 : 512);
    int64_t want = (target_wgs + tiles - 1) / tiles;
    if (svol_deterministic()) want = 1;
    int64_t chunk = (Mc + want - 1) / want;
    chunk = ((chunk + ct - 1) / ct) * ct;
    const int64_t floor_rows = (dtype == SVOL_F32 && Mc <= 4096) ? ct : 4 * ct;
    if (chunk < floor_rows) chunk = floor_rows;
    int64_t splits = (Mc + chunk - 1) / chunk;
    if (splits > 8 && splits % 8) {
        const int64_t s8 = (splits + 7) / 8 * 8;
        int64_t c8 = (Mc + s8 - 1) / s8;
        c8 = ((c8 + ct - 1) / ct) * ct;
        if (c8 >= floor_rows && (Mc + c8 - 1) / c8 == s8) { chunk = c8; splits = s8; }
    }
    const int64_t ktiles = (K + 127) / 128;
    if (splits * tiles > (1ll << 30)) return SVOL_E_UNSUPPORTED;
    out = TnArgs{q.A, q.B, q.C, q.colsum, q.lda, q.ldb, q.ldc, (int)Mc, (int)N, (int)K, (int)chunk, (int)ktiles, (int)splits};
    wgs = splits * tiles;
    return SVOL_OK;
}

extern "C" {

int svol_abi_version(void) { return 7; }

const char* svol_strerror(int code) {
    switch (code) {
        case SVOL_OK: return "ok";
        case SVOL_E_INVALID: return "invalid argument (null pointer, bad size or misaligned buffer)";
        case SVOL_E_UNSUPPORTED: return "shape not supported by the gfx950 kernels";
        case SVOL_E_LAUNCH: return "kernel launch failed";
        default: return "unknown error";
    }
}

static int gemm_nt_dispatch(const GemmCall& c, const void* A2, int64_t n_split, int dtype) {
    const int64_t M = c.M, N = c.N, K = c.K;
    if (!c.A || !c.B || !c.C || (c.epi && !c.aux) || M < 0 || N < 0 || K <= 0) return SVOL_E_INVALID;
    const bool act_ok = c.epi ? (c.act == SVOL_ACT_GELU || c.act == SVOL_ACT_RELU || c.act == SVOL_ACT_GELU_D) : (c.act != SVOL_ACT_GELU_D || c.pre);
    if (!act_ok) return SVOL_E_INVALID;
    if (M == 0 || N == 0) return SVOL_OK;
    if (c.epi && c.colsum && svol_deterministic()) {
        GemmCall d = c; d.colsum = nullptr;
        const int rc = gemm_nt_dispatch(d, A2, n_split, dtype);
        return rc ? rc : svol_colsum(c.C, c.ldc, c.colsum, M, N, dtype, c.stream);
    }
    if (!c.epi) {
        const int epc = svol_is16(dtype) ? 8 : 4;
        if (!svol_is16(dtype) && dtype != SVOL_F32) return SVOL_E_INVALID;
        if (K % epc || c.lda % epc || c.ldb % epc) return SVOL_E_UNSUPPORTED;
        if (!aligned16(c.A) || !aligned16(c.B) || (A2 && !aligned16(A2))) return SVOL_E_INVALID;
        if (A2 && (n_split % 128)) return SVOL_E_UNSUPPORTED;
        if (M > (1 << 30) || N > (1 << 30) || K > (1 << 30)) return SVOL_E_UNSUPPORTED;
        if ((M + 127) / 128 > 65535) return SVOL_E_UNSUPPORTED;
    }
    if (svol_is16(dtype) && !A2) {
        const int rc = (dtype == SVOL_BF16 ? svol_gemm_nt_bf16_fast : svol_gemm_nt_f16_fast)(c);
        if (rc != SVOL_E_UNSUPPORTED) return rc;
    }
    if (dtype == SVOL_F32 && !A2 && skinny_f32_ok(c)) {
        SkArgs q{(const float*)c.A, (const float*)c.B, (float*)c.C, c.bias, c.colscale, (float*)c.pre, (const float*)c.res, (const float*)c.aux,
                 c.colsum, c.lda, c.ldb, c.ldc, c.ldp, c.ldr, c.ldaux, (int)M, (int)N, (int)K, c.act, c.epi};
        hipLaunchKernelGGL(gemm_nt_f32_skinny, dim3((unsigned)(N / 32), (unsigned)((M + 31) / 32)), dim3(256), 0, c.stream, q);
        SVOL_CHECK_LAUNCH();
        return SVOL_OK;
    }
    if (c.epi) {
        if (c.ldc != N || c.ldaux != N) return SVOL_E_UNSUPPORTED;
        GemmCall g = c;
        g.aux = nullptr; g.ldaux = 0; g.colsum = nullptr; g.act = SVOL_ACT_NONE; g.epi = 0;
        if (const int rc = gemm_nt_dispatch(g, nullptr, 0, dtype)) return rc;
        if (const int rc = svol_act_bwd(c.C, c.aux, c.C, c.act, M * N, dtype, c.stream)) return rc;
        return c.colsum ? svol_colsum(c.C, c.ldc, c.colsum, M, N, dtype, c.stream) : SVOL_OK;
    }
    NtArgs p{c.A, A2, c.B, c.C, c.bias, c.colscale, c.pre, c.res, c.lda, c.ldb, c.ldc, c.ldr, c.ldp, n_split, (int)M, (int)N, (int)K, c.act, (int)c.kwrap};
    const dim3 grid((unsigned)((N + 127) / 128), (unsigned)((M + 127) / 128)), g64((unsigned)((N + 63) / 64), (unsigned)((M + 63) / 64));
    const bool small = (int64_t)grid.x * grid.y < 256 && (M + 63) / 64 <= 65535;
    void (*kern)(NtArgs) = dtype == SVOL_BF16 ? (c.out_f32 ? gemm_nt_kernel<bf16_t, float> : gemm_nt_kernel<bf16_t, bf16_t>)
                           : dtype == SVOL_F16 ? (c.out_f32 ? gemm_nt_kernel<f16_t, float> : gemm_nt_kernel<f16_t, f16_t>)
                           : small ? gemm_nt_kernel<float, float, 64> : gemm_nt_kernel<float, float>;
    hipLaunchKernelGGL(kern, dtype == SVOL_F32 && small ? g64 : grid, dim3(256), 0, c.stream, p);
    SVOL_CHECK_LAUNCH();
    return SVOL_OK;
}

int svol_gemm_nt(const void* A, int64_t lda, const void* A2, int64_t n_split, const void* B, int64_t ldb, void* C,
                 int64_t ldc, const float* bias, const float* colscale, int act, void* pre_act_out, int64_t ldp,
                 const void* residual, int64_t ldr, int out_f32, int64_t M, int64_t N, int64_t K, int dtype, void* stream) {
    GemmCall c{};
    c.A = A; c.lda = lda; c.B = B; c.ldb = ldb; c.C = C; c.ldc = ldc; c.pre = pre_act_out; c.ldp = ldp; c.res = residual; c.ldr = ldr;
    c.bias = bias; c.colscale = colscale; c.act = act; c.out_f32 = out_f32; c.M = M; c.N = N; c.K = K; c.kwrap = K;
    c.stream = reinterpret_cast<hipStream_t>(stream);
    return gemm_nt_dispatch(c, A2, n_split, dtype);
}

int svol_gemm_nt_split(const void* A, int64_t lda, const void* W_hilo, int64_t ldw, void* C, int64_t ldc, const float* bias,
                       int64_t M, int64_t N, int64_t K, void* stream) {
    if (K <= 0 || K % 8) return SVOL_E_UNSUPPORTED;
    GemmCall c{};
    c.A = A; c.lda = lda; c.B = W_hilo; c.ldb = ldw; c.C = C; c.ldc = ldc; c.bias = bias;
    c.M = M; c.N = N; c.K = 2 * K; c.kwrap = K;
    c.stream = reinterpret_cast<hipStream_t>(stream);
    return gemm_nt_dispatch(c, nullptr, 0, SVOL_BF16);
}

int svol_gemm_nt_dact(const void* A, int64_t lda, const void* B, int64_t ldb, void* C, int64_t ldc, const void* aux,
                      int64_t ldaux, int act, float* colsum, int64_t M, int64_t N, int64_t K, int dtype, void* stream) {
    GemmCall c{};
    c.A = A; c.lda = lda; c.B = B; c.ldb = ldb; c.C = C; c.ldc = ldc; c.aux = aux; c.ldaux = ldaux; c.colsum = colsum;
    c.M = M; c.N = N; c.K = K; c.kwrap = K; c.act = act; c.epi = 1;
    c.stream = reinterpret_cast<hipStream_t>(stream);
    return gemm_nt_dispatch(c, nullptr, 0, dtype);
}

int svol_gemm_nt_dgelu(const void* A, int64_t lda, const void* B, int64_t ldb, void* C, int64_t ldc, const void* pre,
                       int64_t ldp, float* colsum, int64_t M, int64_t N, int64_t K, int dtype, void* stream) {
    return svol_gemm_nt_dact(A, lda, B, ldb, C, ldc, pre, ldp, SVOL_ACT_GELU, colsum, M, N, K, dtype, stream);
}

static int gemm_tn_dispatch(const svol_tn_problem& q, int dtype, hipStream_t s) {
    if (!q.A || !q.B || !q.C || q.Mc < 0 || q.N <= 0 || q.K <= 0) return SVOL_E_INVALID;
    if (q.Mc == 0) return SVOL_OK;
    if (!svol_is16(dtype) && dtype != SVOL_F32) return SVOL_E_INVALID;
    if (svol_is16(dtype)) {
        const int rc = (dtype == SVOL_BF16 ? svol_gemm_tn_bf16_fast : svol_gemm_tn_f16_fast)(q, s);
        if (rc != SVOL_E_UNSUPPORTED) return rc;
    }
    TnArgs p{};
    int64_t wgs = 0;
    if (const int rc = tn_generic_plan(q, dtype, p, wgs)) return rc;
    if (dtype == SVOL_BF16) hipLaunchKernelGGL(gemm_tn_kernel<bf16_t>, dim3((unsigned)wgs), dim3(256), 0, s, p);
    else if (dtype == SVOL_F16) hipLaunchKernelGGL(gemm_tn_kernel<f16_t>, dim3((unsigned)wgs), dim3(256), 0, s, p);
    else hipLaunchKernelGGL(gemm_tn_kernel<float>, dim3((unsigned)wgs), dim3(256), 0, s, p);
    SVOL_CHECK_LAUNCH();
    return SVOL_OK;
}

int svol_gemm_tn(const void* A, int64_t lda, const void* B, int64_t ldb, float* C, int64_t ldc, float* colsum, int64_t Mc,
                 int64_t N, int64_t K, int dtype, void* stream) {
    return gemm_tn_dispatch(svol_tn_problem{A, lda, B, ldb, C, ldc, colsum, Mc, N, K}, dtype, reinterpret_cast<hipStream_t>(stream));
}

int svol_gemm_tn_grouped(const svol_tn_problem* pr, int32_t n, int dtype, void* stream) {
    if (!pr || n < 0) return SVOL_E_INVALID;
    if (!svol_is16(dtype) && dtype != SVOL_F32) return SVOL_E_INVALID;
    hipStream_t s = reinterpret_cast<hipStream_t>(stream);
// ... 151 lines not shown
```

svol_amd/csrc/norm.hip:

```cpp
#include "common.h"

namespace {

constexpr int LN_MAX_PASSES = 4;

template <typename T, typename TX, int NP>
__global__ __launch_bounds__(256) void ln_fwd_kernel(const TX* __restrict__ x, const float* __restrict__ gamma,
                                                     const float* __restrict__ beta, float* __restrict__ y32,
                                                     T* __restrict__ y, T* __restrict__ ypos, const T* __restrict__ pos,
                                                     int64_t pos_rows, float* __restrict__ mean, float* __restrict__ rstd,
                                                     int64_t M, int D, float p, float inv_keep, uint64_t seed0,
                                                     const int64_t* __restrict__ soff) {
    const uint64_t seed = seed0 + (soff ? ((uint64_t)soff[0] << 8) : 0ull);
    const int lane = threadIdx.x & 63;
    const int64_t row = (int64_t)blockIdx.x * 4 + (threadIdx.x >> 6);
    if (row >= M) return;
    const TX* xr = x + row * D;
    float v[NP][4];
    float s = 0.f;
    const T* pr = pos ? pos + (row % pos_rows) * D : nullptr;
    Vec4<TX> t[NP];
    Vec4<T> pv[NP];
    Vec4<float> gv[NP], bv[NP];
#pragma unroll
    for (int j = 0; j < NP; ++j) {
        const int c = (lane + 64 * j) * 4;
        if (c < D) {
            t[j].load(xr + c);
            if (pr) pv[j].load(pr + c);
            gv[j].load(gamma + c);
            bv[j].load(beta + c);
        }
    }
#pragma unroll
    for (int j = 0; j < NP; ++j) {
        const int c = (lane + 64 * j) * 4;
#pragma unroll
        for (int e = 0; e < 4; ++e) {
            v[j][e] = c < D ? t[j].get(e) : 0.f;
            s += v[j][e];
        }
    }
    const float mu = wave_sum(s) / (float)D;
    float q = 0.f;
#pragma unroll
    for (int j = 0; j < NP; ++j) {
        const int c = (lane + 64 * j) * 4;
        if (c < D) {
#pragma unroll
            for (int e = 0; e < 4; ++e) { const float d = v[j][e] - mu; q += d * d; }
        }
    }
    const float rs = rsqrtf(wave_sum(q) / (float)D + 1e-5f);
    if (lane == 0) { mean[row] = mu; rstd[row] = rs; }
#pragma unroll
    for (int j = 0; j < NP; ++j) {
        const int c = (lane + 64 * j) * 4;
        if (c < D) {
            Vec4<T> o, op;
            Vec4<float> o32;
#pragma unroll
            for (int e = 0; e < 4; ++e) {
                float r = (v[j][e] - mu) * rs * gv[j].get(e) + bv[j].get(e);
                if (p > 0.f) r *= dropout_scale(seed, (uint64_t)row, (uint32_t)(c + e), p, inv_keep);
                o.set(e, r);
                o32.set(e, r);
                if (pr) op.set(e, r + pv[j].get(e));
            }
            if (y32) o32.store(y32 + row * D + c);
            if (y) o.store(y + row * D + c);
            if (ypos) op.store(ypos + row * D + c);
        }
    }
}

template <typename T, typename TX, int NP>
__global__ __launch_bounds__(256) void ln_bwd_kernel(const float* __restrict__ dy32, const T* __restrict__ dy,
                                                     const T* __restrict__ dy2, const TX* __restrict__ x,
                                                     const float* __restrict__ gamma, const float* __restrict__ mean,
                                                     const float* __restrict__ rstd, float* __restrict__ dx32,
                                                     T* __restrict__ dx, float* __restrict__ dgamma,
                                                     float* __restrict__ dbeta, float* __restrict__ dxsum, int64_t M, int D,
                                                     float p, float inv_keep, uint64_t seed0, const int64_t* __restrict__ soff, int rows_per_wave,
                                                     float* __restrict__ det_part) {
    const uint64_t seed = seed0 + (soff ? ((uint64_t)soff[0] << 8) : 0ull);
    const int lane = threadIdx.x & 63;
    const int64_t wave_id = (int64_t)blockIdx.x * 4 + (threadIdx.x >> 6);
    const int64_t r0 = wave_id * rows_per_wave;
    float dg[NP][4], db[NP][4], dxs[NP][4], gm[NP][4];
#pragma unroll
    for (int j = 0; j < NP; ++j) {
        const int c = (lane + 64 * j) * 4;
#pragma unroll
        for (int e = 0; e < 4; ++e) { dg[j][e] = 0.f; db[j][e] = 0.f; dxs[j][e] = 0.f; gm[j][e] = c < D ? gamma[c + e] : 0.f; }
    }
    struct Row { Vec4<float> a32[NP]; Vec4<T> a[NP], b[NP]; Vec4<TX> xv[NP]; float mu, rs; };
    auto fetch = [&](int64_t row, Row& r) {
#pragma unroll
        for (int j = 0; j < NP; ++j) {
            const int c = (lane + 64 * j) * 4;
            if (c < D) {
                if (dy32) r.a32[j].load(dy32 + row * D + c);
                if (dy) r.a[j].load(dy + row * D + c);
                if (dy2) r.b[j].load(dy2 + row * D + c);
                r.xv[j].load(x + row * D + c);
            }
        }
        r.mu = mean[row];
        r.rs = rstd[row];
    };
    const int64_t rend = (r0 + rows_per_wave < M) ? r0 + rows_per_wave : M;
    Row cur, nxt;
    if (r0 < rend) fetch(r0, cur);
    for (int64_t row = r0; row < rend; ++row) {
        if (row + 1 < rend) fetch(row + 1, nxt);
        const float mu = cur.mu, rs = cur.rs;
        float g[NP][4], xh[NP][4];
        float s1 = 0.f, s2 = 0.f;
#pragma unroll
        for (int j = 0; j < NP; ++j) {
            const int c = (lane + 64 * j) * 4;
            if (c < D) {
#pragma unroll
                for (int e = 0; e < 4; ++e) {
                    float d = (dy32 ? cur.a32[j].get(e) : 0.f) + (dy ? cur.a[j].get(e) : 0.f) + (dy2 ? cur.b[j].get(e) : 0.f);
                    if (p > 0.f) d *= dropout_scale(seed, (uint64_t)row, (uint32_t)(c + e), p, inv_keep);
                    const float h = (cur.xv[j].get(e) - mu) * rs;
                    xh[j][e] = h;
                    dg[j][e] += d * h;
                    db[j][e] += d;
                    const float gg = d * gm[j][e];
                    g[j][e] = gg;
                    s1 += gg;
                    s2 += gg * h;
                }
            }
        }
        s1 = wave_sum(s1) / (float)D;
        s2 = wave_sum(s2) / (float)D;
#pragma unroll
        for (int j = 0; j < NP; ++j) {
            const int c = (lane + 64 * j) * 4;
            if (c < D) {
                Vec4<T> o;
                Vec4<float> o32;
#pragma unroll
                for (int e = 0; e < 4; ++e) {
                    const float r = rs * (g[j][e] - s1 - xh[j][e] * s2);
                    dxs[j][e] += r;
                    o.set(e, r);
                    o32.set(e, r);
                }
                if (dx32) o32.store(dx32 + row * D + c);
                if (dx) o.store(dx + row * D + c);
            }
        }
        cur = nxt;
    }
    __shared__ float red[3][NP * 256];
    const int wave = threadIdx.x >> 6;
    for (int w = 0; w < 4; ++w) {
        if (wave == w) {
#pragma unroll
            for (int j = 0; j < NP; ++j) {
                const int c = (lane + 64 * j) * 4;
                if (c < D) {
#pragma unroll
                    for (int e = 0; e < 4; ++e) {
                        if (w == 0) { red[0][c + e] = dg[j][e]; red[1][c + e] = db[j][e]; red[2][c + e] = dxs[j][e]; }
                        else { red[0][c + e] += dg[j][e]; red[1][c + e] += db[j][e]; red[2][c + e] += dxs[j][e]; }
                    }
                }
            }
        }
        __syncthreads();
    }
    if (det_part) {
        float* row = det_part + (int64_t)blockIdx.x * 3 * D;
        for (int c = threadIdx.x; c < D; c += 256) { row[c] = red[0][c]; row[D + c] = red[1][c]; row[2 * D + c] = red[2][c]; }
        return;
// ... 39 lines not shown
        if constexpr (sizeof(T) == 4) {
            for (int t = 0; t < ntok; ++t) {
                const float a = xe[t] / dim_t;
                out[(int64_t)t * D] = from_f32<T>(odd ? cosf(a) : sinf(a));
            }
        } else {
            const float inv = 0.15915494309189535f / dim_t;
            for (int t = 0; t < ntok; ++t) {
                const float rev = xe[t] * inv;
                out[(int64_t)t * D] = from_f32<T>(odd ? __builtin_amdgcn_cosf(rev) : __builtin_amdgcn_sinf(rev));
            }
        }
    }
}


template <typename T>
__global__ __launch_bounds__(256) void dropout_kernel(const T* __restrict__ x, T* __restrict__ y, int64_t n, int64_t row_len, float p,
                                                      float inv_keep, uint64_t seed, const int64_t* __restrict__ step) {
    const uint32_t s0 = drop_seed32(drop_seed_at(seed, step));
    int64_t i = ((int64_t)blockIdx.x * blockDim.x + threadIdx.x) * 4;
    const int64_t stride = (int64_t)gridDim.x * blockDim.x * 4;
    for (; i < n; i += stride) {
        int64_t r = i / row_len;
        int64_t k = i - r * row_len;
        uint32_t rm = drop_row(s0, (uint64_t)r);
#pragma unroll
        for (int e = 0; e < 4; ++e) {
            if (i + e >= n) break;
            y[i + e] = from_f32<T>(to_f32(x[i + e]) * drop_scale_rk(rm, (uint32_t)k, p, inv_keep));
            if (++k == row_len) { k = 0; ++r; rm = drop_row(s0, (uint64_t)r); }
        }
    }
}
__global__ __launch_bounds__(256) void dropout_add_kernel(const float* t, const float* res, float* out, int64_t n, int64_t row_len, float p,
                                                          float inv_keep, uint64_t seed, const int64_t* __restrict__ step) {
    const uint32_t s0 = drop_seed32(drop_seed_at(seed, step));
    int64_t i = ((int64_t)blockIdx.x * blockDim.x + threadIdx.x) * 4;
    const int64_t stride = (int64_t)gridDim.x * blockDim.x * 4;
    for (; i < n; i += stride) {
        int64_t r = i / row_len;
        int64_t k = i - r * row_len;
        uint32_t rm = drop_row(s0, (uint64_t)r);
#pragma unroll
        for (int e = 0; e < 4; ++e) {
            if (i + e >= n) break;
            out[i + e] = res[i + e] + t[i + e] * drop_scale_rk(rm, (uint32_t)k, p, inv_keep);
            if (++k == row_len) { k = 0; ++r; rm = drop_row(s0, (uint64_t)r); }
        }
    }
}
}

extern "C" {

int svol_layernorm_fwd(const void* x, int x_f32, const float* gamma, const float* beta, float* y32, void* y,
                       void* ypos, const void* pos, int64_t pos_rows, float* mean, float* rstd, int64_t M, int64_t D,
                       float dropout_p, uint64_t seed, const int64_t* seed_offset_dev, int dtype, void* stream) {
    if (!x || !gamma || !beta || (!y && !y32) || !mean || !rstd || M < 0 || D <= 0) return SVOL_E_INVALID;
    if (!aligned16(gamma) || !aligned16(beta)) return SVOL_E_INVALID;
    if ((ypos != nullptr) != (pos != nullptr)) return SVOL_E_INVALID;
    if (pos && pos_rows <= 0) return SVOL_E_INVALID;
    if (D % 4 || D > LN_MAX_PASSES * 256) return SVOL_E_UNSUPPORTED;
    if (dropout_p < 0.f || dropout_p >= 1.f) return SVOL_E_INVALID;
    if (!svol_is16(dtype) && dtype != SVOL_F32) return SVOL_E_INVALID;
    if (M == 0) return SVOL_OK;
    const float inv_keep = 1.f / (1.f - dropout_p);
    const unsigned grid = (unsigned)((M + 3) / 4);
    hipStream_t s = reinterpret_cast<hipStream_t>(stream);
#define SVOL_LNF(TT, TXX, NPP)                                                                                              \
    hipLaunchKernelGGL((ln_fwd_kernel<TT, TXX, NPP>), dim3(grid), dim3(256), 0, s, (const TXX*)x, gamma, beta, y32, (TT*)y,      \
                       (TT*)ypos, (const TT*)pos, pos_rows, mean, rstd, M, (int)D, dropout_p, inv_keep, seed, seed_offset_dev)
#define SVOL_LNF_NP(TT, TXX)                     \
    do {                                         \
        if (D <= 256) SVOL_LNF(TT, TXX, 1);      \
        else if (D <= 512) SVOL_LNF(TT, TXX, 2); \
        else SVOL_LNF(TT, TXX, 4);               \
    } while (0)
    if (dtype == SVOL_BF16 && x_f32) SVOL_LNF_NP(bf16_t, float);
    else if (dtype == SVOL_BF16) SVOL_LNF_NP(bf16_t, bf16_t);
    else if (dtype == SVOL_F16 && x_f32) SVOL_LNF_NP(f16_t, float);
    else if (dtype == SVOL_F16) SVOL_LNF_NP(f16_t, f16_t);
    else SVOL_LNF_NP(float, float);
#undef SVOL_LNF_NP
#undef SVOL_LNF
    SVOL_CHECK_LAUNCH();
    return SVOL_OK;
}

int svol_layernorm_bwd(const float* dy32, const void* dy, const void* dy2, const void* x, int x_f32, const float* gamma,
                       const float* mean, const float* rstd, float* dx32, void* dx, float* dgamma, float* dbeta,
                       float* dx_colsum, int64_t M, int64_t D, float dropout_p, uint64_t seed, const int64_t* seed_offset_dev,
                       int dtype, void* stream) {
    if ((!dy32 && !dy && !dy2) || !x || !gamma || !mean || !rstd || (!dx && !dx32) || !dgamma || !dbeta || M < 0 || D <= 0)
        return SVOL_E_INVALID;
    if (D % 4 || D > LN_MAX_PASSES * 256) return SVOL_E_UNSUPPORTED;
    if (dropout_p < 0.f || dropout_p >= 1.f) return SVOL_E_INVALID;
    if (!svol_is16(dtype) && dtype != SVOL_F32) return SVOL_E_INVALID;
    if (M == 0) return SVOL_OK;
    const float inv_keep = 1.f / (1.f - dropout_p);
    int64_t rpw = (M + 2047) / 2048;
    if (rpw < 1) rpw = 1;
    const int64_t waves = (M + rpw - 1) / rpw;
    const unsigned grid = (unsigned)((waves + 3) / 4);
    hipStream_t s = reinterpret_cast<hipStream_t>(stream);
    const bool det_mode = svol_deterministic();
    DetScratch det(det_mode ? (size_t)grid * 3 * (size_t)D : 0, s);
    if (det_mode && !det.p) return SVOL_E_LAUNCH;
#define SVOL_LNB(TT, TXX, NPP)                                                                                                      \
    hipLaunchKernelGGL((ln_bwd_kernel<TT, TXX, NPP>), dim3(grid), dim3(256), 0, s, dy32, (const TT*)dy, (const TT*)dy2, (const TXX*)x, \
                       gamma, mean, rstd, dx32, (TT*)dx, dgamma, dbeta, dx_colsum, M, (int)D, dropout_p, inv_keep, seed,              \
                       seed_offset_dev, (int)rpw, det.p)
#define SVOL_LNB_NP(TT, TXX)                  \
    do {                                      \
        if (D <= 256) SVOL_LNB(TT, TXX, 1);   \
        else if (D <= 512) SVOL_LNB(TT, TXX, 2); \
        else SVOL_LNB(TT, TXX, 4);            \
    } while (0)
    if (dtype == SVOL_BF16 && x_f32) SVOL_LNB_NP(bf16_t, float);
    else if (dtype == SVOL_BF16) SVOL_LNB_NP(bf16_t, bf16_t);
    else if (dtype == SVOL_F16 && x_f32) SVOL_LNB_NP(f16_t, float);
    else if (dtype == SVOL_F16) SVOL_LNB_NP(f16_t, f16_t);
    else SVOL_LNB_NP(float, float);
#undef SVOL_LNB_NP
#undef SVOL_LNB
    if (det_mode) {
        det_fold(det.p, (int)grid, 3 * D, dgamma, D, s);
        det_fold(det.p + D, (int)grid, 3 * D, dbeta, D, s);
        det_fold(det.p + 2 * D, (int)grid, 3 * D, dx_colsum, D, s);
    }
    SVOL_CHECK_LAUNCH();
    return SVOL_OK;
}

int svol_dropout_sd(const void* x, void* y, int64_t n, int64_t row_len, float p, uint64_t seed, const int64_t* seed_step_dev, int dtype,
                    void* stream) {
    if (!x || !y || n < 0 || row_len <= 0 || row_len > 0xffffffffll || !(p >= 0.f && p < 1.f)) return SVOL_E_INVALID;
    if (n == 0) return SVOL_OK;
    const float inv = 1.f / (1.f - p);
    int64_t g = (n + 1023) / 1024;
    if (g > 8192) g = 8192;
    hipStream_t s = reinterpret_cast<hipStream_t>(stream);
    if (dtype == SVOL_F32) hipLaunchKernelGGL(dropout_kernel<float>, dim3((unsigned)g), dim3(256), 0, s, (const float*)x, (float*)y, n, row_len, p, inv, seed, seed_step_dev);
    else if (dtype == SVOL_BF16) hipLaunchKernelGGL(dropout_kernel<bf16_t>, dim3((unsigned)g), dim3(256), 0, s, (const bf16_t*)x, (bf16_t*)y, n, row_len, p, inv, seed, seed_step_dev);
    else if (dtype == SVOL_F16) hipLaunchKernelGGL(dropout_kernel<f16_t>, dim3((unsigned)g), dim3(256), 0, s, (const f16_t*)x, (f16_t*)y, n, row_len, p, inv, seed, seed_step_dev);
    else return SVOL_E_INVALID;
    SVOL_CHECK_LAUNCH();
    return SVOL_OK;
}

int svol_dropout(const void* x, void* y, int64_t n, int64_t row_len, float p, uint64_t seed, int dtype, void* stream) {
    return svol_dropout_sd(x, y, n, row_len, p, seed, nullptr, dtype, stream);
}

int svol_dropout_add_sd(const float* t32, const float* res32, float* out32, int64_t n, int64_t row_len, float p, uint64_t seed,
                        const int64_t* seed_step_dev, void* stream) {
    if (!t32 || !res32 || !out32 || n < 0 || row_len <= 0 || row_len > 0xffffffffll || !(p >= 0.f && p < 1.f)) return SVOL_E_INVALID;
    if (n == 0) return SVOL_OK;
    int64_t g = (n + 1023) / 1024;
    if (g > 8192) g = 8192;
    hipLaunchKernelGGL(dropout_add_kernel, dim3((unsigned)g), dim3(256), 0, reinterpret_cast<hipStream_t>(stream), t32, res32, out32, n,
                       row_len, p, 1.f / (1.f - p), seed, seed_step_dev);
    SVOL_CHECK_LAUNCH();
    return SVOL_OK;
}
int svol_dropout_add(const float* t32, const float* res32, float* out32, int64_t n, int64_t row_len, float p, uint64_t seed, void* stream) {
    return svol_dropout_add_sd(t32, res32, out32, n, row_len, p, seed, nullptr, stream);
}

int svol_posenc_sine(const float* mask, void* pos, int64_t B, int64_t L, int64_t D, int dtype, void* stream) {
    if (!mask || !pos || B <= 0 || L <= 0 || D <= 0) return SVOL_E_INVALID;
    if (L > (1 << 24) || D > 4096) return SVOL_E_UNSUPPORTED;
    hipStream_t s = reinterpret_cast<hipStream_t>(stream);
    if (B > 65535) return SVOL_E_UNSUPPORTED;
    dim3 grid((unsigned)((L + 63) / 64), (unsigned)B);
    if (dtype == SVOL_BF16)
        hipLaunchKernelGGL(posenc_kernel<bf16_t>, grid, dim3(256), 0, s, mask, (bf16_t*)pos, (int)L, (int)D);
    else if (dtype == SVOL_F16)
        hipLaunchKernelGGL(posenc_kernel<f16_t>, grid, dim3(256), 0, s, mask, (f16_t*)pos, (int)L, (int)D);
    else if (dtype == SVOL_F32)
        hipLaunchKernelGGL(posenc_kernel<float>, grid, dim3(256), 0, s, mask, (float*)pos, (int)L, (int)D);
    else return SVOL_E_INVALID;
    SVOL_CHECK_LAUNCH();
    return SVOL_OK;
}
// ... 3 lines not shown
```

svol_amd/layers.py:

```python
from __future__ import annotations

import math
import os

import torch

from . import _lib
from .ops import (ACT_GELU, ACT_NONE, ACT_RELU, _DT, _ptr, _stream, act_bwd, attn_bwd, attn_fwd, attn_weights_mean, cast, colsum,
                  dropout, dropout_add, gemm_nt, gemm_nt_dact, gemm_nt_split, layernorm_bwd, layernorm_fwd)
from .params import SPLIT_V, GradGroup, claim, sink_view, unless_sunk, weights


def _pos_grad(dypos, pos_shape, D):
    rows = 1
    for n in pos_shape[:-1]:
        rows *= n
    g = colsum(dypos.reshape(-1, rows * D).contiguous())
    return cast(g.view(pos_shape), dypos.dtype)


class LayerNormFn(torch.autograd.Function):

    @staticmethod
    def forward(ctx, x, gamma, beta, p, seed, seed_dev):
        shp = x.shape
        x2 = x.reshape(-1, shp[-1])
        _, y, _, mean, rstd = layernorm_fwd(x2, gamma, beta, x.dtype, None, p, seed, seed_dev=seed_dev)
        ctx.save_for_backward(x2, gamma, mean, rstd, seed_dev)
        ctx.p, ctx.seed, ctx.shp = p, seed, shp
        ctx.sinks = (claim(gamma, ctx.needs_input_grad[1]), claim(beta, ctx.needs_input_grad[2]))
        return y.view(shp)

    @staticmethod
    def backward(ctx, dy):
        x2, gamma, mean, rstd, seed_dev = ctx.saved_tensors
        sg, sb = ctx.sinks
        _, dx, dg, db = layernorm_bwd(None, dy, None, x2, gamma, mean, rstd, x2.dtype, ctx.p, ctx.seed, seed_dev=seed_dev,
                                      dg_out=sink_view(sg), db_out=sink_view(sb))
        return dx.view(ctx.shp), unless_sunk(sg, dg), unless_sunk(sb, db), None, None, None


def layer_norm(x, gamma, beta, p=0.0, seed=0, seed_dev=None):
    return LayerNormFn.apply(x, gamma, beta, p, seed, seed_dev)


class LinearFn(torch.autograd.Function):

    @staticmethod
    def forward(ctx, x, W, b, act, out_f32):
        if act == ACT_GELU:
            raise _lib.SvolHipError('LinearFn: GELU is only available fused in MLPLNFn')
        shp = x.shape
        x2 = x.reshape(-1, shp[-1])
        Wc, WcT = weights.get(W, x.dtype)
        y = gemm_nt(x2, Wc, b, act, out_f32=out_f32)
        ctx.save_for_backward(x2, y if act != ACT_NONE else None)
        ctx.WcT, ctx.act, ctx.shp, ctx.has_b = WcT, act, shp, b is not None
        ctx.need_dx = ctx.needs_input_grad[0]
        epc = 4 if x.dtype == torch.float32 else 8
        ok = W.shape[0] % epc == 0
        ctx.sinks = (claim(W, ok and ctx.needs_input_grad[1]), claim(b, ok and ctx.needs_input_grad[2]))
        return y.view(*shp[:-1], W.shape[0])

    @staticmethod
    def backward(ctx, dy):
        x2, y = ctx.saved_tensors
        N = dy.shape[-1]
        d = dy.reshape(-1, N)
        if not d.is_contiguous():
            d = d.contiguous()
        if d.dtype != x2.dtype:
            d = cast(d, x2.dtype)
        if ctx.act != ACT_NONE:
            d = act_bwd(d, y, ctx.act)
        epc = 4 if d.dtype == torch.float32 else 8
        WcT = ctx.WcT
        Np = (N + epc - 1) // epc * epc
        if N % epc:
            dp = torch.zeros((d.shape[0], Np), dtype=d.dtype, device=d.device)
            dp[:, :N] = d
            wp = torch.zeros((WcT.shape[0], Np), dtype=WcT.dtype, device=WcT.device)
            wp[:, :N] = WcT
            d, WcT = dp, wp
        K_ = x2.shape[1]
        sW, sb = ctx.sinks
        grads = GradGroup(((sW, (Np, K_)), (sb, (Np,), ctx.has_b)), d.device)
        grads.tn(d, x2, 0, 1 if ctx.has_b else None)
        dW, db = grads.finish()
        if N != Np:
            dW, db = dW[:N], db[:N] if ctx.has_b else None
        dx = gemm_nt(d, WcT).view(ctx.shp) if ctx.need_dx else None
        return dx, dW, db, None, None


def linear(x, W, b=None, act=ACT_NONE, out_f32=False):
    return LinearFn.apply(x, W, b, act, out_f32)
# ... 500 lines not shown
```

svol_amd/modeling/cross_modal_transformer.py:

```python
from __future__ import annotations

import copy
import os

import torch
from torch import nn

from .. import _lib, blocks, layers, ops
from ..params import GradGroup, claim, weights

D_FF = 2048


class MLP(nn.Module):

    def __init__(self, in_features, hidden_features):
        super().__init__()
        self.fc1 = nn.Linear(in_features, hidden_features)
        self.fc2 = nn.Linear(hidden_features, in_features)


OVERLAP_QUERY_STREAM = os.environ.get('SVOL_NO_STREAM_OVERLAP') is None
QUERY_FP32 = os.environ.get('SVOL_QUERY_BF16') is None
_SIDE = {}
# ... 108 lines not shown
    return list(_GateVectorsAllFn.apply(skch, layers[0].nhead, *params))


class CrossModalTransformerLayer(nn.Module):
    def __init__(self, d_model=512, nhead=8, dim_feedforward=D_FF):
        super().__init__()
        self.sketch_video_cross_attn = nn.MultiheadAttention(d_model, nhead)
        self.norm1 = nn.LayerNorm(d_model)
        self.content_self_attn = nn.MultiheadAttention(d_model, nhead)
        self.norm2 = nn.LayerNorm(d_model)
        self.mlp1 = MLP(d_model, dim_feedforward)
        self.norm3 = nn.LayerNorm(d_model)
        self.token_self_attn = nn.MultiheadAttention(d_model, nhead)
        self.norm4 = nn.LayerNorm(d_model)
        self.content_token_cross_attn = nn.MultiheadAttention(d_model, nhead)
        self.norm5 = nn.LayerNorm(d_model)
        self.mlp2 = MLP(d_model, dim_feedforward)
        self.norm6 = nn.LayerNorm(d_model)
        self.d_model, self.nhead = d_model, nhead

    def gate_vectors(self, skch):
        m = self.sketch_video_cross_attn
        return _GateVectorsFn.apply(skch, m.in_proj_weight, m.in_proj_bias, self.nhead)

    def forward(self, mem32, skch32, out, pos, qpos, kbias, u=None):
        m32, m, mpos = self.video_half(mem32, skch32, pos, u)
        return m32, self.query_half(out, m, mpos, qpos, kbias)

    def video_half(self, mem32, skch32, pos, u=None, u_next=None, sc_in=None):
        if blocks.ENABLED:
            uu = self.gate_vectors(skch32) if u is None else u
            m32, m, mpos, sc = blocks.video_half(self, mem32, pos, uu, pos.dtype, u_next, sc_in)
            return (m32, m, mpos) if u_next is None else (m32, m, mpos, sc)
        assert sc_in is None
        h = self.nhead
        n = lambda m: (m.weight, m.bias)
        mha = lambda m: (m.in_proj_weight, m.in_proj_bias, m.out_proj.weight, m.out_proj.bias)
        mlp = lambda m: (m.fc1.weight, m.fc1.bias, m.fc2.weight, m.fc2.bias)
        m32, m, mpos = layers.gate(mem32, pos, self.gate_vectors(skch32) if u is None else u, *n(self.norm1), h)
        m32, m = layers.self_attn_ln(m32, m, mpos, *mha(self.content_self_attn), *n(self.norm2), None, h)
        return layers.mlp_ln(m32, m, *mlp(self.mlp1), *n(self.norm3), pos)

    def query_half(self, out, m, mpos, qpos, kbias):
        return self.query_cross(self.query_self(out, qpos, m.dtype), m, mpos, qpos, kbias)

    def query_self(self, out, qpos, dt=None):
        if blocks.ENABLED:
            return blocks.query_self(self, out, qpos, dt if dt is not None else qpos.dtype, qpos.dtype)
        n = lambda m_: (m_.weight, m_.bias)
        mha = lambda m_: (m_.in_proj_weight, m_.in_proj_bias, m_.out_proj.weight, m_.out_proj.bias)
        o32, o, opos = out
        return layers.self_attn_ln(o32, o, opos, *mha(self.token_self_attn), *n(self.norm4), qpos, self.nhead)

    def query_cross(self, out, m, mpos, qpos, kbias):
        n = lambda m_: (m_.weight, m_.bias)
        mha = lambda m_: (m_.in_proj_weight, m_.in_proj_bias, m_.out_proj.weight, m_.out_proj.bias)
        mlp = lambda m_: (m_.fc1.weight, m_.fc1.bias, m_.fc2.weight, m_.fc2.bias)
        if blocks.ENABLED:
            return blocks.query_cross(self, out, m, mpos, kbias, qpos, m.dtype, qpos.dtype)
        o32, o, opos = out
        o32, o = layers.cross_attn_ln(o32, o, opos, mpos, m, *mha(self.content_token_cross_attn), *n(self.norm5), None, self.nhead,
                                   kbias)
        return layers.mlp_ln(o32, o, *mlp(self.mlp2), *n(self.norm6), qpos)


class CrossModalTransformer(nn.Module):
    def __init__(self, d_model=512, nhead=8, num_layers=6, dim_feedforward=D_FF):
        super().__init__()
        layer = CrossModalTransformerLayer(d_model, nhead, dim_feedforward)
        self.layers = nn.ModuleList([copy.deepcopy(layer) for _ in range(num_layers)])
        for p in self.parameters():
            if p.dim() > 1:
                nn.init.xavier_uniform_(p)
        self.d_model, self.nhead, self.num_layers = d_model, nhead, num_layers
        self._epoch_seen = -1

    def forward(self, src_vid32, src_skch32, kbias, vid_pos, query_embed, us=None):
        if weights.epoch == self._epoch_seen:
            weights.new_epoch()
        self._epoch_seen = weights.epoch
        B = src_vid32.shape[0]
        dt = torch.float32 if QUERY_FP32 else vid_pos.dtype
        qpos = layers.cast_ag(query_embed, dt)
        N, d = qpos.shape
        def initial_queries():
            return (torch.zeros((B, N, d), dtype=torch.float32, device=vid_pos.device),
                    torch.zeros((B, N, d), dtype=dt, device=vid_pos.device),
                    qpos.unsqueeze(0).expand(B, -1, -1).contiguous())
        mem32 = src_vid32
        outputs = []
        if us is None:
            us = all_gate_vectors(list(self.layers), src_skch32)
        if not OVERLAP_QUERY_STREAM:
            out = initial_queries()
            for layer, u in zip(self.layers, us):
                mem32, out = layer(mem32, src_skch32, out, vid_pos, qpos, kbias, u)
                outputs.append(out[0])
            return torch.stack(outputs)
        main = torch.cuda.current_stream()
        side = _side_stream(main.device)
        side.wait_stream(main)
        qpos.record_stream(side)
        kbias.record_stream(side)
        with torch.cuda.stream(side):
            out = initial_queries()
        sc = None
        for li, (layer, u) in enumerate(zip(self.layers, us)):
            with torch.cuda.stream(side):
                out_sa = layer.query_self(out, qpos, vid_pos.dtype)
            if blocks.ENABLED and blocks.GATE_SCORES_FUSE and li + 1 < len(us):
                m32, m, mpos, sc = layer.video_half(mem32, src_skch32, vid_pos, u, us[li + 1], sc)
            elif sc is not None:
                m32, m, mpos = layer.video_half(mem32, src_skch32, vid_pos, u, None, sc)
            else:
                m32, m, mpos = layer.video_half(mem32, src_skch32, vid_pos, u)
            side.wait_stream(main)
            m.record_stream(side)
            mpos.record_stream(side)
            with torch.cuda.stream(side):
                out = layer.query_cross(out_sa, m, mpos, qpos, kbias)
                outputs.append(out[0])
            mem32 = m32
        main.wait_stream(side)
        for t in outputs:
            t.record_stream(main)
        return torch.stack(outputs)


def build_cross_modal_transformer(args):
    return CrossModalTransformer(d_model=args.hidden_dim, nhead=args.nheads, num_layers=args.num_layers,
                                 dim_feedforward=D_FF)
```

svol_amd/modeling/svanet.py:

```python
from __future__ import annotations

import os

import torch
from torch import nn

from .. import layers, ops, params
from . import cross_modal_transformer as cmt
from .cross_modal_transformer import build_cross_modal_transformer
from .position_encoding import build_position_encoding

INPUT_OVERLAP = os.environ.get('SVOL_NO_INPUT_OVERLAP') is None

_DTYPES = {'bf16': torch.bfloat16, 'fp32': torch.float32, 'fp16': torch.float16, torch.float16: torch.float16, torch.bfloat16: torch.bfloat16,
           torch.float32: torch.float32}


class MLP(nn.Module):

    def __init__(self, input_dim, hidden_dim, output_dim, num_layers):
        super().__init__()
        self.num_layers = num_layers
        h = [hidden_dim] * (num_layers - 1)
        self.layers = nn.ModuleList(nn.Linear(n, k) for n, k in zip([input_dim] + h, h + [output_dim]))

    def forward(self, x, last_act=ops.ACT_NONE):
        for i, layer in enumerate(self.layers):
            act = ops.ACT_RELU if i < self.num_layers - 1 else last_act
            x = layers.linear(x, layer.weight, layer.bias, act)
        return x


class LinearLayer(nn.Module):

    def __init__(self, in_hsz, out_hsz, layer_norm=True, dropout=0.1, relu=True):
        super().__init__()
        self.relu = relu
        self.layer_norm = layer_norm
        self.p = dropout
        if layer_norm:
            self.LayerNorm = nn.LayerNorm(in_hsz)
        self.net = nn.Sequential(nn.Dropout(dropout), nn.Linear(in_hsz, out_hsz))

    def forward(self, x, seed=0, out_f32=False, seed_dev=None):
        p = self.p if self.training else 0.0
        if self.layer_norm:
            x = layers.layer_norm(x, self.LayerNorm.weight, self.LayerNorm.bias, p, seed, seed_dev)
        elif p > 0.0:
            raise NotImplementedError('dropout without LayerNorm is not on the reference path')
        lin = self.net[1]
        return layers.linear(x, lin.weight, lin.bias, ops.ACT_RELU if self.relu else ops.ACT_NONE, out_f32)


class SVANet(nn.Module):
    def __init__(self, transformer, sketch_position_embed, video_position_embed, input_vid_dim, input_skch_dim,
                 num_queries, input_dropout=0.1, aux_loss=True, use_sketch_pos=True, n_input_proj=2, num_classes=2,
                 vis_mode=None, compute_dtype='bf16'):
        super().__init__()
        self.num_queries = num_queries
        self.num_classes = num_classes
        self.transformer = transformer
        self.sketch_position_embed = sketch_position_embed
        self.video_position_embed = video_position_embed
        hidden_dim = transformer.d_model
        self.bbox_embed = MLP(hidden_dim, hidden_dim, 4, 3)
        self.use_sketch_pos = use_sketch_pos
        self.class_embed = nn.Linear(hidden_dim, 2)
        self.n_input_proj = n_input_proj
        self.class_head = nn.Linear(hidden_dim, num_classes)
        self.query_embed = nn.Embedding(num_queries, hidden_dim)
        relu_args = [True] * 3
        relu_args[n_input_proj - 1] = False
        self.input_video_proj = nn.Sequential(*[
            LinearLayer(input_vid_dim, hidden_dim, dropout=input_dropout, relu=relu_args[0]),
            LinearLayer(hidden_dim, hidden_dim, dropout=input_dropout, relu=relu_args[1]),
            LinearLayer(hidden_dim, hidden_dim, dropout=input_dropout, relu=relu_args[2])][:n_input_proj])
        self.input_sketch_proj = nn.Sequential(*[
            LinearLayer(input_skch_dim, hidden_dim, dropout=input_dropout, relu=relu_args[0]),
            LinearLayer(hidden_dim, hidden_dim, dropout=input_dropout, relu=relu_args[1]),
            LinearLayer(hidden_dim, hidden_dim, dropout=input_dropout, relu=relu_args[2])][:n_input_proj])
        self.vis_mode = vis_mode
        self.aux_loss = aux_loss
        self.compute_dtype = _DTYPES[compute_dtype]
        self._step = 0
        self.base_seed = 1
        self.step_dev = None

    def _proj(self, seq, x, salt):
        n = len(seq)
        for j, layer in enumerate(seq):
            x = layer(x, seed=(self.base_seed << 32) + (self._step << 8) + salt * 16 + j, out_f32=(j == n - 1),
                      seed_dev=self.step_dev)
        return x

    def forward(self, src_sketch, src_sketch_mask, src_video, src_video_mask):
        if not src_video.is_cuda:
            raise RuntimeError('svol_amd.SVANet runs on the MI355X HIP kernels only; move the module and its '
                               'inputs to cuda (there is no CPU path — the CPU oracle lives under oracle/).')
        dt = self.compute_dtype
        d = self.transformer.d_model
        overlap = INPUT_OVERLAP and cmt.OVERLAP_QUERY_STREAM and isinstance(self.transformer, cmt.CrossModalTransformer)
        if not overlap:
            params.weights.new_epoch()
        if self.training:
            self._step += 1
        def mask_side(with_us):
            mask_f = src_video_mask.to(torch.float32)
            pos_video = self.video_position_embed(mask_f, d, dt)
            skch = self._proj(self.input_sketch_proj, layers.cast_ag(src_sketch.float(), dt), 1)
            skch = skch.reshape(skch.shape[0], -1)
            kbias = torch.zeros_like(mask_f).masked_fill_(mask_f == 0, float('-inf'))
            us = cmt.all_gate_vectors(list(self.transformer.layers), skch) if with_us else None
            return pos_video, skch, kbias, us

        if overlap:
            main = torch.cuda.current_stream()
            side = cmt._side_stream(main.device)
            side.wait_stream(main)
            with torch.cuda.stream(side):
                params.weights.new_epoch()
                casts_done = side.record_event()
            xv = layers.cast_ag(src_video.float(), dt)
            with torch.cuda.stream(side):
                pos_video, skch, kbias, us = mask_side(True)
            main.wait_event(casts_done)
            vid = self._proj(self.input_video_proj, xv, 0)
            main.wait_stream(side)
            for t in [pos_video, skch, kbias] + list(us or []):
                t.record_stream(main)
        else:
            vid = self._proj(self.input_video_proj, layers.cast_ag(src_video.float(), dt), 0)
            pos_video, skch, kbias, us = mask_side(False)
        hs = (self.transformer(vid, skch, kbias, pos_video, self.query_embed.weight, us) if us is not None else
              self.transformer(vid, skch, kbias, pos_video, self.query_embed.weight))
        if layers.heads_fusable(hs, self.class_embed, self.bbox_embed):
            outputs_class, outputs_coord = layers.heads(hs, self.class_embed, self.bbox_embed)
        else:
            outputs_class = layers.linear(hs, self.class_embed.weight, self.class_embed.bias)
            outputs_coord = self.bbox_embed(hs, last_act=ops.ACT_SIGMOID)
        out = {'pred_logits': outputs_class[-1], 'pred_boxes': outputs_coord[-1]}
        if self.aux_loss:
            out['aux_outputs'] = [{'pred_logits': a, 'pred_boxes': b}
                                  for a, b in zip(outputs_class[:-1], outputs_coord[:-1])]
        out['_svol_stacked'] = (outputs_class, outputs_coord)
        if self.vis_mode is not None:
            return out, hs
        return out


def build_svanet(args):
    transformer = build_cross_modal_transformer(args)
    sketch_position_embed, video_position_embed = build_position_encoding(args)
    return SVANet(transformer, sketch_position_embed, video_position_embed, input_vid_dim=args.input_vid_dim,
                  input_skch_dim=args.input_skch_dim, num_queries=args.num_queries,
                  input_dropout=args.input_dropout, aux_loss=args.aux_loss, use_sketch_pos=args.use_sketch_pos,
                  n_input_proj=args.n_input_proj, vis_mode=args.vis_mode,
                  compute_dtype=getattr(args, 'compute_dtype', 'bf16'))
```

svol_amd/ops.py:

```python
from __future__ import annotations

import ctypes
import math
import os
from typing import Optional

import torch

from . import _lib, wgrad

ACT_NONE, ACT_RELU, ACT_GELU, ACT_SIGMOID, ACT_RELU_RES, ACT_GELU_D = 0, 1, 2, 3, 4, 5
_DT = {torch.float32: 0, torch.bfloat16: 1, torch.float16: 2}


def _dt(t: torch.Tensor) -> int:
    try:
        return _DT[t.dtype]
    except KeyError:
        raise _lib.SvolHipError(f'unsupported dtype {t.dtype}')


_RAW_STREAM = getattr(torch._C, '_cuda_getCurrentRawStream', None)
_CUR_DEVICE = getattr(torch._C, '_cuda_getDevice', None)

# ... 136 lines not shown
    arr = (_lib.TnProblem * n)()
    dt = None
    for i, (A, B, out, cs) in enumerate(problems):
        assert A.dim() == 2 and B.dim() == 2 and A.shape[0] == B.shape[0] and A.stride(1) == 1 and B.stride(1) == 1 and A.dtype == B.dtype
        assert dt is None or dt == A.dtype
        dt = A.dtype
        arr[i] = _lib.TnProblem(_ptr(A), A.stride(0), _ptr(B), B.stride(0), _ptr(out), out.stride(0), _ptr(cs), A.shape[0], A.shape[1],
                                B.shape[1])
    rc = _lib.lib().svol_gemm_tn_grouped(ctypes.cast(arr, ctypes.c_void_p), n, _DT[dt], _stream() if stream is None else stream)
    _lib.check(rc, 'svol_gemm_tn_grouped')


def gemm_tn_sink(A, B, out, colsum=None):
    if not wgrad.issue(lambda ws: gemm_tn(A, B, out=out, colsum=colsum, stream=ws.cuda_stream), (A, B), _current_stream_obj()):
        gemm_tn(A, B, out=out, colsum=colsum)
    return out


def gemm_nt_dact(A, B, aux, act, want_colsum=True, colsum_out=None):
    M, K = A.shape
    N = B.shape[0]
    out = torch.empty((M, N), dtype=A.dtype, device=A.device)
    cs = colsum_out
    if cs is None and want_colsum:
        cs = torch.zeros((N,), dtype=torch.float32, device=A.device)
    rc = _lib.lib().svol_gemm_nt_dact(_ptr(A), A.stride(0), _ptr(B), B.stride(0), _ptr(out), out.stride(0), _ptr(aux),
                                      aux.stride(0), act, _ptr(cs), M, N, K, _dt(A), _stream())
    _lib.check(rc, 'svol_gemm_nt_dact')
    return out, cs


def gemm_nt_dgelu(A, B, pre, want_colsum=True, colsum_out=None):
    return gemm_nt_dact(A, B, pre, ACT_GELU, want_colsum, colsum_out)


def colsum(X, out=None):
    assert X.dim() == 2 and X.stride(1) == 1
    M, N = X.shape
    if out is None:
        out = torch.zeros((N,), dtype=torch.float32, device=X.device)
    _lib.check(_lib.lib().svol_colsum(_ptr(X), X.stride(0), _ptr(out), M, N, _dt(X), _stream()), 'svol_colsum')
    return out


def act_bwd(dy, aux, act):
    dy = dy.contiguous()
    aux = aux.contiguous()
    out = torch.empty_like(dy)
    _lib.check(_lib.lib().svol_act_bwd(_ptr(dy), _ptr(aux), _ptr(out), act, dy.numel(), _dt(dy), _stream()),
               'svol_act_bwd')
    return out


def layernorm_fwd(x, gamma, beta, dtype, pos=None, p=0.0, seed=0, want32=False, want_t=True, seed_dev=None):
    x = x.contiguous()
    M, D = x.shape
    x_f32 = 1 if (x.dtype == torch.float32 and dtype != torch.float32) else 0
    assert x.dtype in (dtype, torch.float32)
    y32 = torch.empty((M, D), dtype=torch.float32, device=x.device) if want32 else None
    y = torch.empty((M, D), dtype=dtype, device=x.device) if want_t else None
    ypos = torch.empty((M, D), dtype=dtype, device=x.device) if pos is not None else None
    mean = torch.empty((M,), dtype=torch.float32, device=x.device)
    rstd = torch.empty((M,), dtype=torch.float32, device=x.device)
    if pos is not None:
        pos = pos.contiguous()
        assert pos.dtype == dtype and pos.shape[-1] == D
    rc = _lib.lib().svol_layernorm_fwd(_ptr(x), x_f32, _ptr(gamma), _ptr(beta), _ptr(y32), _ptr(y), _ptr(ypos),
                                       _ptr(pos), pos.numel() // D if pos is not None else 0, _ptr(mean), _ptr(rstd),
                                       M, D, float(p), int(seed), _ptr(seed_dev), _DT[dtype], _stream())
    _lib.check(rc, 'svol_layernorm_fwd')
    return y32, y, ypos, mean, rstd


def layernorm_bwd(dy32, dy, dy2, x, gamma, mean, rstd, dtype, p=0.0, seed=0, want32=False, want_t=True,
                  want_colsum=False, seed_dev=None, dg_out=None, db_out=None, cs_out=None):
    M, D = x.shape
    x_f32 = 1 if (x.dtype == torch.float32 and dtype != torch.float32) else 0
    cont = lambda t: None if t is None else t.reshape(M, D).contiguous()
    dy32, dy, dy2 = cont(dy32), cont(dy), cont(dy2)
    assert dy32 is None or dy32.dtype == torch.float32
    assert (dy is None or dy.dtype == dtype) and (dy2 is None or dy2.dtype == dtype)
    dx32 = torch.empty((M, D), dtype=torch.float32, device=x.device) if want32 else None
    dx = torch.empty((M, D), dtype=dtype, device=x.device) if want_t else None
    dg, db, cs = dg_out, db_out, (cs_out if want_colsum else None)
    if dg is None or db is None or (want_colsum and cs is None):
        red = torch.zeros((3, D), dtype=torch.float32, device=x.device)
        dg = red[0] if dg is None else dg
        db = red[1] if db is None else db
        cs = (red[2] if cs is None else cs) if want_colsum else None
    rc = _lib.lib().svol_layernorm_bwd(_ptr(dy32), _ptr(dy), _ptr(dy2), _ptr(x), x_f32, _ptr(gamma), _ptr(mean),
                                       _ptr(rstd), _ptr(dx32), _ptr(dx), _ptr(dg), _ptr(db), _ptr(cs), M, D, float(p),
                                       int(seed), _ptr(seed_dev), _DT[dtype], _stream())
    _lib.check(rc, 'svol_layernorm_bwd')
    if want_colsum:
        return dx32, dx, dg, db, cs
    return dx32, dx, dg, db


def posenc_sine(mask_f32: torch.Tensor, D: int, dtype: torch.dtype) -> torch.Tensor:
    mask_f32 = mask_f32.contiguous()
    B, L = mask_f32.shape
    pos = torch.empty((B, L, D), dtype=dtype, device=mask_f32.device)
    _lib.check(_lib.lib().svol_posenc_sine(_ptr(mask_f32), _ptr(pos), B, L, D, _DT[dtype], _stream()),
               'svol_posenc_sine')
    return pos


def attn_ws_bytes(dtype, B, H, Lq, Lk, dh):
    return max(int(_lib.lib().svol_attn_ws_bytes(B, H, Lq, Lk, dh)), 0) if dtype != torch.float32 else 0


def _attn_ws(q, B, H, Lq, Lk, dh):
    n = attn_ws_bytes(q.dtype, B, H, Lq, Lk, dh)
    return torch.empty((n // 4,), dtype=torch.float32, device=q.device) if n else None


def dropout(x, p, seed, out=None, seed_dev=None):
    assert x.is_contiguous()
    out = torch.empty_like(x) if out is None else out
    args = (_ptr(x), _ptr(out), x.numel(), max(1, x.shape[-1] if x.dim() else 1), float(p), int(seed))
    if seed_dev is None:
        _lib.check(_lib.lib().svol_dropout(*args, _dt(x), _stream()), 'svol_dropout')
    else:
        _lib.check(_lib.lib().svol_dropout_sd(*args, _ptr(seed_dev), _dt(x), _stream()), 'svol_dropout_sd')
    return out


def dropout_add(t32, res32, p, seed, seed_dev=None):
    assert t32.is_contiguous() and res32.is_contiguous() and t32.dtype == torch.float32 and res32.dtype == torch.float32
    args = (_ptr(t32), _ptr(res32), _ptr(t32), t32.numel(), max(1, t32.shape[-1]), float(p), int(seed))
    if seed_dev is None:
        _lib.check(_lib.lib().svol_dropout_add(*args, _stream()), 'svol_dropout_add')
    else:
        _lib.check(_lib.lib().svol_dropout_add_sd(*args, _ptr(seed_dev), _stream()), 'svol_dropout_add_sd')
    return t32


def _attn_drop(drop):
    if drop is None or drop[0] <= 0.0:
        return 0.0, 0, None
    return float(drop[0]), int(drop[1]), (drop[2] if len(drop) > 2 else None)


def attn_fwd(q, k, v, B, H, Lq, Lk, dh, kbias=None, premul=0.0, drop=None):
    o = torch.empty((B * Lq, H * dh), dtype=q.dtype, device=q.device)
    lse2 = torch.empty((B, H, Lq), dtype=torch.float32, device=q.device)
# ... 275 lines not shown
```

Before: 15050.

## Fuse f32 widening/casts into attention, layernorm, GEMM and precompute cross-attn Q

Adds f32-aware variants of attention forward and backward that write or read f32 copies (o32, d_o32, dq32) inside the combine, delta and dq kernels, so separate cast passes are no longer needed. Adds layernorm entry points that take f32 input directly, so the video projection no longer runs a separate cast to bf16 first. Adds a GEMM variant that emits both f32 and 16-bit outputs. Splits query-cross forward so its Q projection runs earlier on the side stream, overlapping with the video half. The cost is more kernel entry points and extra plumbing of pre-computed state through autograd.

```diff
diff --git a/include/svol_hip.h b/include/svol_hip.h
--- a/include/svol_hip.h
+++ b/include/svol_hip.h
@@ -70,6 +70,8 @@
                  void* C, int64_t ldc, const float* bias, const float* colscale, int act, void* pre_act_out,
                  int64_t ldp, const void* residual, int64_t ldr, int out_f32, int64_t M, int64_t N, int64_t K,
                  int dtype, void* stream);
+int svol_gemm_nt_f32_c16(const void* A, int64_t lda, const void* B, int64_t ldb, void* C, int64_t ldc, const float* bias,
+                         const float* colscale, void* C16, int64_t ldc16, int dtype16, int64_t M, int64_t N, int64_t K, void* stream);
 int svol_gemm_nt_split(const void* A, int64_t lda, const void* W_hilo, int64_t ldw, void* C, int64_t ldc, const float* bias,
                        int64_t M, int64_t N, int64_t K, void* stream);
 int svol_gemm_nt_dgelu(const void* A, int64_t lda, const void* B, int64_t ldb, void* C, int64_t ldc,
@@ -100,6 +102,12 @@
                        const float* gamma, const float* mean, const float* rstd, float* dx32, void* dx,
                        float* dgamma, float* dbeta, float* dx_colsum, int64_t M, int64_t D, float dropout_p,
                        uint64_t seed, const int64_t* seed_offset_dev, int dtype, void* stream);
+int svol_layernorm_fwd_x32r(const float* x32, const float* gamma, const float* beta, float* y32, void* y, void* ypos, const void* pos,
+                            int64_t pos_rows, float* mean, float* rstd, int64_t M, int64_t D, float dropout_p, uint64_t seed,
+                            const int64_t* seed_offset_dev, int dtype, void* stream);
+int svol_layernorm_bwd_x32r(const float* dy32, const void* dy, const void* dy2, const float* x32, const float* gamma, const float* mean,
+                            const float* rstd, float* dx32, void* dx, float* dgamma, float* dbeta, float* dx_colsum, int64_t M, int64_t D,
+                            float dropout_p, uint64_t seed, const int64_t* seed_offset_dev, int dtype, void* stream);
 
 int svol_dropout(const void* x, void* y, int64_t n, int64_t row_len, float p, uint64_t seed, int dtype, void* stream);
 int svol_dropout_add(const float* t32, const float* res32, float* out32, int64_t n, int64_t row_len, float p, uint64_t seed, void* stream);
@@ -119,6 +127,13 @@
                   void* dq, int64_t lddq, void* dk, int64_t lddk, void* dv, int64_t lddv, int64_t B, int64_t H,
                   int64_t Lq, int64_t Lk, int64_t dh, float scale, float q_premul, void* ws, int64_t ws_bytes,
                   int dtype, void* stream);
+int svol_attn_fwd_o32(const void* q, int64_t ldq, const void* k, int64_t ldk, const void* v, int64_t ldv, void* o, int64_t ldo,
+                      float* o32, float* lse2, const float* kbias, int64_t B, int64_t H, int64_t Lq, int64_t Lk, int64_t dh, float scale,
+                      float q_premul, void* ws, int64_t ws_bytes, int dtype, void* stream);
+int svol_attn_bwd_x32(const void* q, int64_t ldq, const void* k, int64_t ldk, const void* v, int64_t ldv, const void* o, int64_t ldo,
+                      const float* d_o32, void* d_o, int64_t lddo, const float* lse2, float* delta, const float* kbias, void* dq,
+                      int64_t lddq, float* dq32, void* dk, int64_t lddk, void* dv, int64_t lddv, int64_t B, int64_t H, int64_t Lq,
+                      int64_t Lk, int64_t dh, float scale, float q_premul, void* ws, int64_t ws_bytes, int dtype, void* stream);
 
 #define SVOL_ATTN_DQ_PREZEROED 1
 int64_t svol_attn_bwd_sp_image_bytes(int64_t B, int64_t H, int64_t Lq, int64_t Lk, int64_t dh, int64_t ws_bytes, int dtype);
@@ -334,6 +349,7 @@
 int svol_query_self_bwd(const int64_t* dims, void* const* slots, void* stream);
 int svol_query_self_wgrad(const int64_t* dims, void* const* slots, void* stream);
 int svol_query_cross_fwd(const int64_t* dims, void* const* slots, void* stream);
+int svol_query_cross_fwd_phase(const int64_t* dims, void* const* slots, int phase, void* stream);
 int svol_query_cross_bwd(const int64_t* dims, void* const* slots, void* stream);
 int svol_query_cross_wgrad(const int64_t* dims, void* const* slots, void* stream);
 
diff --git a/svol_amd/_lib.py b/svol_amd/_lib.py
--- a/svol_amd/_lib.py
+++ b/svol_amd/_lib.py
@@ -136,6 +136,14 @@
     'svol_query_cross_fwd': [_p, _p, _p],
     'svol_query_cross_bwd': [_p, _p, _p],
     'svol_query_cross_wgrad': [_p, _p, _p],
+    'svol_query_cross_fwd_phase': [_p, _p, _int, _p],
+    'svol_gemm_nt_f32_c16': [_p, _i64, _p, _i64, _p, _i64, _p, _p, _p, _i64, _int, _i64, _i64, _i64, _p],
+    'svol_attn_fwd_o32': [_p, _i64, _p, _i64, _p, _i64, _p, _i64, _p, _p, _p, _i64, _i64, _i64, _i64, _i64, _f32, _f32, _p, _i64,
+                          _int, _p],
+    'svol_attn_bwd_x32': [_p, _i64, _p, _i64, _p, _i64, _p, _i64, _p, _p, _i64, _p, _p, _p, _p, _i64, _p, _p, _i64, _p, _i64,
+                          _i64, _i64, _i64, _i64, _i64, _f32, _f32, _p, _i64, _int, _p],
+    'svol_layernorm_fwd_x32r': [_p, _p, _p, _p, _p, _p, _p, _i64, _p, _p, _i64, _i64, _f32, _u64, _p, _int, _p],
+    'svol_layernorm_bwd_x32r': [_p, _p, _p, _p, _p, _p, _p, _p, _p, _p, _p, _p, _i64, _i64, _f32, _u64, _p, _int, _p],
 }
 
 
diff --git a/svol_amd/blocks.py b/svol_amd/blocks.py
--- a/svol_amd/blocks.py
+++ b/svol_amd/blocks.py
@@ -522,10 +522,33 @@
             ('DO32', R * D * 4), ('DXQP', R * D * qe)] + ([] if merged else [('DMPOS', M * D * e)]) + [('DMV', M * D * e)]
 
 
+class CrossQ:
+    __slots__ = ('pl', 'opos', 'buf', 'q', 'qc')
+
+
+def query_cross_q(layer, out, dt, qdt):
+    pl = plan(layer, QC, dt, qdt)
+    opos = _c(out[2].detach())
+    B, N, D = opos.shape
+    R = B * N
+    h = CrossQ()
+    h.pl, h.opos = pl, opos
+    nq = _align(R * D * _ESZ[qdt])
+    h.buf = torch.empty((nq + _align(R * D * _ESZ[dt]),), dtype=torch.uint8, device=opos.device)
+    h.q, h.qc = h.buf.data_ptr(), h.buf.data_ptr() + nq
+    tbl = _Table(QC, pl.tpl)
+    tbl.set('OPOS', opos.data_ptr())
+    tbl.set('Q', h.q)
+    tbl.set('QC', h.qc)
+    dims = _dims(B, 0, N, D, layer.nhead, 0, dt, qdt, 0)
+    _lib.check(_lib.lib().svol_query_cross_fwd_phase(dims, tbl.arr, 1, ops._stream()), 'svol_query_cross_fwd_phase')
+    return h
+
+
 class QueryCrossFn(torch.autograd.Function):
 
     @staticmethod
-    def forward(ctx, pl, o32, o, opos, mv, mpos, kbias, qpos, merged, *params):
+    def forward(ctx, pl, o32, o, opos, mv, mpos, kbias, qpos, merged, pre, *params):
         B, N, D = o.shape
         L = mv.shape[1]
         layer = pl.layer()
@@ -539,7 +562,14 @@
         lay = _open(ctx, pl, QC, (B, N, L, D, H, F, dt, qdt, merged), _dims(B, L, N, D, H, F, dt, qdt, wsb), len(params), o.device,
                     lambda: _qc_fwd_layout(B, N, L, D, H, F, e, qe), lambda: [('ATTN_WS', max(wsb, 16))],
                     O32=o32_, O=o_, OPOS=opos_, MV=mv_, MPOS=mpos_, KBIAS=kb_, QPOS=qpos_)
-        _call('svol_query_cross_fwd', ctx)
+        if pre is not None:
+            assert pre.pl is pl and pre.opos.data_ptr() == opos_.data_ptr()
+            ctx.tbl.set('Q', pre.q)
+            ctx.tbl.set('QC', pre.qc)
+            ctx.pre = pre
+            _call('svol_query_cross_fwd_phase', ctx, 2)
+        else:
+            _call('svol_query_cross_fwd', ctx)
         ctx.shape = (B, N, L, D, H, F)
         ctx.merged = merged
         ctx.save_for_backward(o32_, o_, opos_, mv_, mpos_, kb_, qpos)
@@ -549,7 +579,7 @@
     @staticmethod
     def backward(ctx, dy32, dy, dypos):
         if dy32 is None and dy is None and dypos is None:
-            return _no_grads(ctx, 9)
+            return _no_grads(ctx, 10)
         B, N, L, D, H, F = ctx.shape
         o32_, o_, opos_, mv_, mpos_, kb_, qpos = ctx.saved_tensors
         dt, qdt = ctx.pl.dt, ctx.pl.qdt
@@ -557,19 +587,19 @@
         lay, tmp, bufs, gs = _open_bwd(ctx, o_.device, lambda: _qc_bwd_layout(B, N, L, D, H, F, _ESZ[dt], _ESZ[qdt], ctx.merged),
                                        DY32=dy32, DY=dy, DYPOS=dypos)
         _call('svol_query_cross_bwd', ctx)
-        pg = _close_bwd(ctx, 'svol_query_cross_wgrad', bufs, [ctx.arena, tmp, opos_, mv_, mpos_], 9)
+        pg = _close_bwd(ctx, 'svol_query_cross_wgrad', bufs, [ctx.arena, tmp, opos_, mv_, mpos_], 10)
         vq = lambda n_, dt_: lay.view(tmp, n_, dt_, (B, N, D))
         vm = lambda n_: lay.view(tmp, n_, dt, (B, L, D))
         return (None, vq('DO32', torch.float32), None, vq('DXQP', qdt), vm('DMV'), None if ctx.merged else vm('DMPOS'), None,
-                _qpos_grad(gq, qdt), None) + pg
-
-
-def query_cross(layer, out, mv, mpos, kbias, qpos, dt, qdt):
-    pl = plan(layer, QC, dt, qdt)
+                _qpos_grad(gq, qdt), None, None) + pg
+
+
+def query_cross(layer, out, mv, mpos, kbias, qpos, dt, qdt, pre=None):
+    pl = plan(layer, QC, dt, qdt) if pre is None else pre.pl
     o32, o, opos = out
     fn = mv.grad_fn
     merged = fn is not None and fn is mpos.grad_fn and isinstance(fn, VideoHalfFn._backward_cls)
-    return QueryCrossFn.apply(pl, o32, o, opos, mv, mpos, kbias, qpos, merged, *pl.inputs(o32, opos, mv, mpos))
+    return QueryCrossFn.apply(pl, o32, o, opos, mv, mpos, kbias, qpos, merged, pre, *pl.inputs(o32, opos, mv, mpos))
 
 
 def trace_dump() -> str:
diff --git a/svol_amd/csrc/attention.hip b/svol_amd/csrc/attention.hip
--- a/svol_amd/csrc/attention.hip
+++ b/svol_amd/csrc/attention.hip
@@ -594,6 +594,55 @@
     return attn_bwd_impl(q, ldq, k, ldk, v, ldv, o, ldo, d_o, lddo, lse2, delta, kbias, dq, lddq, dk, lddk, dv, lddv, B, H, Lq, Lk, dh,
                          scale, q_premul, ws, ws_bytes, 0.f, 0, nullptr, dtype, stream, flags, ev_prep);
 }
+int svol_attn_fwd_o32(const void* q, int64_t ldq, const void* k, int64_t ldk, const void* v, int64_t ldv, void* o, int64_t ldo,
+                      float* o32, float* lse2, const float* kbias, int64_t B, int64_t H, int64_t Lq, int64_t Lk, int64_t dh, float scale,
+                      float q_premul, void* ws, int64_t ws_bytes, int dtype, void* stream) {
+    if (!o32 || !aligned16(o32) || !svol_is16(dtype)) return SVOL_E_INVALID;
+    AttnCall c{};
+    c.q = q; c.k = k; c.v = v; c.out_o = o; c.lse2 = lse2; c.kbias = kbias;
+    c.ldq = ldq; c.ldk = ldk; c.ldv = ldv; c.ldo = ldo;
+    c.scale = scale; c.premul = q_premul; c.ws = static_cast<float*>(ws); c.ws_bytes = ws_bytes;
+    c.stream = reinterpret_cast<hipStream_t>(stream);
+    if (const int rc = check_call(c, false, B, H, Lq, Lk, dh, dtype)) return rc;
+    const bool fused = dh <= 32 && ((dtype == SVOL_BF16 ? svol_attn_x32_fused_bf16 : svol_attn_x32_fused_f16)(c) & SVOL_ATTN_X32_O);
+    if (!fused && ldo != H * dh) return SVOL_E_UNSUPPORTED;
+    if (fused) c.o32 = o32;
+    int rc;
+    if (dh > 32) rc = dtype == SVOL_BF16 ? fwd_launch<bf16_t, 2>(c) : fwd_launch<f16_t, 2>(c);
+    else rc = (dtype == SVOL_BF16 ? svol_attn_fwd_bf16_launch : svol_attn_fwd_f16_launch)(c);
+    if (rc || fused) return rc;
+    return svol_cast(o, dtype, o32, SVOL_F32, B * Lq * H * dh, stream);
+}
+
+int svol_attn_bwd_x32(const void* q, int64_t ldq, const void* k, int64_t ldk, const void* v, int64_t ldv, const void* o, int64_t ldo,
+                      const float* d_o32, void* d_o, int64_t lddo, const float* lse2, float* delta, const float* kbias, void* dq,
+                      int64_t lddq, float* dq32, void* dk, int64_t lddk, void* dv, int64_t lddv, int64_t B, int64_t H, int64_t Lq,
+                      int64_t Lk, int64_t dh, float scale, float q_premul, void* ws, int64_t ws_bytes, int dtype, void* stream) {
+    if (!d_o32 || !dq32 || !aligned16(d_o32) || !aligned16(dq32) || !svol_is16(dtype)) return SVOL_E_INVALID;
+    AttnCall c{};
+    c.q = q; c.k = k; c.v = v; c.o = o; c.d_o = d_o; c.lse2 = const_cast<float*>(lse2); c.delta = delta; c.kbias = kbias;
+    c.dq = dq; c.dk = dk; c.dv = dv;
+    c.ldq = ldq; c.ldk = ldk; c.ldv = ldv; c.ldo = ldo; c.lddo = lddo; c.lddq = lddq; c.lddk = lddk; c.lddv = lddv;
+    c.scale = scale; c.premul = q_premul; c.ws = static_cast<float*>(ws); c.ws_bytes = ws_bytes;
+    c.stream = reinterpret_cast<hipStream_t>(stream);
+    if (const int rc = check_call(c, true, B, H, Lq, Lk, dh, dtype)) return rc;
+    const int fused = dh <= 32 ? (dtype == SVOL_BF16 ? svol_attn_x32_fused_bf16 : svol_attn_x32_fused_f16)(c) : 0;
+    const int64_t n = B * Lq * H * dh;
+    if (!(fused & SVOL_ATTN_X32_DO)) {
+        if (lddo != H * dh) return SVOL_E_UNSUPPORTED;
+        if (const int rc = svol_cast(d_o32, SVOL_F32, d_o, dtype, n, stream)) return rc;
+    } else {
+        c.d_o32 = d_o32;
+    }
+    if (fused & SVOL_ATTN_X32_DQ) c.dq32 = dq32;
+    else if (lddq != H * dh) return SVOL_E_UNSUPPORTED;
+    int rc;
+    if (dh > 32) rc = dtype == SVOL_BF16 ? bwd_launch<bf16_t, 2>(c) : bwd_launch<f16_t, 2>(c);
+    else rc = (dtype == SVOL_BF16 ? svol_attn_bwd_bf16_launch : svol_attn_bwd_f16_launch)(c);
+    if (rc || (fused & SVOL_ATTN_X32_DQ)) return rc;
+    return svol_cast(dq, dtype, dq32, SVOL_F32, n, stream);
+}
+
 int64_t svol_attn_bwd_sp_image_bytes(int64_t B, int64_t H, int64_t Lq, int64_t Lk, int64_t dh, int64_t ws_bytes, int dtype) {
     if (!svol_is16(dtype) || dh > 32 || check_common(B, H, Lq, Lk, dh, dtype)) return 0;
     return (dtype == SVOL_BF16 ? svol_attn_sp_image_bytes_bf16 : svol_attn_sp_image_bytes_f16)((int)B, (int)H, (int)Lq, (int)Lk, (int)dh,
diff --git a/svol_amd/csrc/attention_bf16.hip b/svol_amd/csrc/attention_bf16.hip
--- a/svol_amd/csrc/attention_bf16.hip
+++ b/svol_amd/csrc/attention_bf16.hip
@@ -30,6 +30,9 @@
     uint64_t drop_seed;
     const int64_t* drop_step;
     int dq_rot;
+    float* o32;
+    const float* d_o32;
+    float* dq32;
 };
 __device__ __forceinline__ float attn_drop(uint64_t seed, uint64_t row, int key, float p, float inv) {
     return dropout_scale(seed, row, (uint32_t)key, p, inv);
@@ -328,6 +331,13 @@
     if (qvalid && h == 0) p.lse2[((int64_t)b * p.H + hh) * p.Lq + qrow] = m2 + __builtin_amdgcn_logf(lt);
 }
 
+__device__ __forceinline__ f32x4 widen_stored(h16x4 v) {
+    uint2 bits = __builtin_bit_cast(uint2, v);
+    asm volatile("" : "+v"(bits.x), "+v"(bits.y));
+    const h16x4 w = __builtin_bit_cast(h16x4, bits);
+    return f32x4{(float)w[0], (float)w[1], (float)w[2], (float)w[3]};
+}
+
 __global__ void attn_combine_bf16(Args p) {
     const int64_t idx = (int64_t)blockIdx.x * blockDim.x + threadIdx.x;
     const int64_t total = (int64_t)p.B * p.Lq * p.H;
@@ -364,6 +374,7 @@
 #pragma unroll
             for (int e = 0; e < 4; ++e) v[e] = (h16_t)(acc[d + e] * inv);
             *reinterpret_cast<h16x4*>(o + d) = v;
+            if (p.o32) *reinterpret_cast<f32x4*>(p.o32 + row * (p.H * p.dh) + hh * p.dh + d) = widen_stored(v);
         }
     }
     p.lse2[((int64_t)b * p.H + hh) * p.Lq + q] = M + __builtin_amdgcn_logf(L);
@@ -378,9 +389,19 @@
     const int b = (int)(row / p.Lq), q = (int)(row % p.Lq);
     const h16_t* o = reinterpret_cast<const h16_t*>(p.o) + row * p.ldo + hh * p.dh;
     const h16_t* d = reinterpret_cast<const h16_t*>(p.d_o) + row * p.lddo + hh * p.dh;
+    const float* d32 = p.d_o32 ? p.d_o32 + row * (p.H * p.dh) + hh * p.dh : nullptr;
     float s = 0.f;
     for (int i = 0; i < p.dh; i += 8) {
-        const h16x8 a = *reinterpret_cast<const h16x8*>(o + i), c = *reinterpret_cast<const h16x8*>(d + i);
+        const h16x8 a = *reinterpret_cast<const h16x8*>(o + i);
+        h16x8 c;
+        if (d32) {
+            const f32x4 lo = *reinterpret_cast<const f32x4*>(d32 + i), hi = *reinterpret_cast<const f32x4*>(d32 + i + 4);
+#pragma unroll
+            for (int e = 0; e < 4; ++e) { c[e] = (h16_t)lo[e]; c[4 + e] = (h16_t)hi[e]; }
+            *reinterpret_cast<h16x8*>(const_cast<h16_t*>(d) + i) = c;
+        } else {
+            c = *reinterpret_cast<const h16x8*>(d + i);
+        }
 #pragma unroll
         for (int e = 0; e < 8; ++e) s += (float)a[e] * (float)c[e];
     }
@@ -405,6 +426,7 @@
 #pragma unroll
         for (int e = 0; e < 4; ++e) v[e] = (h16_t)(t[e] * p.scale);
         *reinterpret_cast<h16x4*>(o + i) = v;
+        if (p.dq32) *reinterpret_cast<f32x4*>(p.dq32 + row * (p.H * p.dh) + hh * p.dh + i) = widen_stored(v);
     }
 }
 
@@ -2505,7 +2527,16 @@
         p.ws_dq = p.ws_ml + (int64_t)p.ksplit * p.B * p.H * p.Lq * 2;
     }
     p.head_xcd = g.head_xcd; p.nxt = g.nxt; p.tail_last = g.tail_last;
+    p.o32 = c.o32; p.d_o32 = c.d_o32; p.dq32 = c.dq32;
     return p;
+}
+int svol_attn_x32_fused_bf16(const AttnCall& c) {
+    const Plan pl = attn_plan(c);
+    int m = 0;
+    if (pl.fwd_ksplit > 1) m |= SVOL_ATTN_X32_O;
+    if (!pl.pre) m |= SVOL_ATTN_X32_DO;
+    if (pl.bwd == Bwd::fq_m || pl.bwd == Bwd::fq_u || ((pl.bwd == Bwd::two_pass_m || pl.bwd == Bwd::two_pass_u) && pl.bwd_ksplit > 1)) m |= SVOL_ATTN_X32_DQ;
+    return m;
 }
 
 int svol_attn_fwd_bf16_launch(const AttnCall& c) {
diff --git a/svol_amd/csrc/attn_call.h b/svol_amd/csrc/attn_call.h
--- a/svol_amd/csrc/attn_call.h
+++ b/svol_amd/csrc/attn_call.h
@@ -1,5 +1,9 @@
 #pragma once
 #include "common.h"
+
+#define SVOL_ATTN_X32_O 1
+#define SVOL_ATTN_X32_DO 2
+#define SVOL_ATTN_X32_DQ 4
 
 struct AttnCall {
     const void *q, *k, *v, *o, *d_o;
@@ -15,6 +19,9 @@
     int64_t ws_bytes;
     int flags;
     void* ev_prep;
+    float* o32;
+    const float* d_o32;
+    float* dq32;
     hipStream_t stream;
 };
 
@@ -29,6 +36,7 @@
 #define SVOL_ATTN_H16_ENTRIES(T)                                                                                      \
     int svol_attn_fwd_##T##_launch(const AttnCall& c);                                                                \
     int svol_attn_bwd_##T##_launch(const AttnCall& c);                                                                \
+    int svol_attn_x32_fused_##T(const AttnCall& c);                                                                   \
     int64_t svol_attn_ws_floats_##T(int B, int H, int Lq, int Lk, int dh);                                            \
     int64_t svol_attn_sp_image_bytes_##T(int B, int H, int Lq, int Lk, int dh, int64_t ws_bytes);                     \
     int svol_attn_sp_zero_##T##_launch(float* ws, int64_t ws_bytes, int B, int H, int Lq, int Lk, int dh, hipStream_t s);
diff --git a/svol_amd/csrc/blocks.hip b/svol_amd/csrc/blocks.hip
--- a/svol_amd/csrc/blocks.hip
+++ b/svol_amd/csrc/blocks.hip
@@ -314,32 +314,44 @@
 #undef P
 }
 
-int svol_query_cross_fwd(const int64_t* dims, void* const* p, void* s) {
-    if (!dims || !p) return SVOL_E_INVALID;
-    Trace tr_("query_cross_fwd", s);
-    const Dims d(dims);
-    if (!d.ok() || d.N <= 0 || d.L <= 0 || d.F <= 0) return SVOL_E_INVALID;
+int svol_query_cross_fwd_phase(const int64_t* dims, void* const* p, int phase, void* s) {
+    if (!dims || !p || phase < 0 || phase > 2) return SVOL_E_INVALID;
+    Trace tr_(phase == 1 ? "query_cross_fwd.q" : "query_cross_fwd", s);
+    const Dims d(dims);
+    if (!d.ok() || d.N <= 0 || (phase != 1 && (d.L <= 0 || d.F <= 0))) return SVOL_E_INVALID;
     const int64_t R = d.B * d.N, M = d.B * d.L, D = d.D, F = d.F, dh = D / d.H;
     const int dt = d.dt, qdt = d.qdt, xf = qdt != SVOL_F32;
     const bool mixed = qdt != dt;
+    const bool fuse = mixed && qdt == SVOL_F32;
 #define P(n) p[SVOL_QC_##n]
-    if (mixed) {
-        RUN(nt(P(OPOS), D, P(W_INQ), D, P(Q), D, P(B_IN), P(QSCALE), R, D, D, qdt, s));
-        RUN(svol_cast(P(Q), qdt, P(QC), dt, R * D, s));
-    } else {
-        RUN(nt(P(OPOS), D, P(W_KV), D, P(QC), D, P(B_IN), P(QSCALE), R, D, D, dt, s));
-    }
+    if (phase != 2) {
+        if (fuse) {
+            RUN(svol_gemm_nt_f32_c16(P(OPOS), D, P(W_INQ), D, P(Q), D, f32(P(B_IN)), f32(P(QSCALE)), P(QC), D, dt, R, D, D, s));
+        } else if (mixed) {
+            RUN(nt(P(OPOS), D, P(W_INQ), D, P(Q), D, P(B_IN), P(QSCALE), R, D, D, qdt, s));
+            RUN(svol_cast(P(Q), qdt, P(QC), dt, R * D, s));
+        } else {
+            RUN(nt(P(OPOS), D, P(W_KV), D, P(QC), D, P(B_IN), P(QSCALE), R, D, D, dt, s));
+        }
+    }
+    if (phase == 1) return SVOL_OK;
     RUN(nt(P(MPOS), D, at(P(W_KV), D * D, dt), D, P(KV), 2 * D, f32(P(B_IN)) + D, nullptr, M, D, D, dt, s));
     if (P(WV_HILO))
         RUN(svol_gemm_nt_split(P(MV), D, P(WV_HILO), 2 * D, at(P(KV), D, dt), 2 * D, f32(P(B_IN)) + 2 * D, M, D, D, s));
     else
         RUN(nt(P(MV), D, at(P(W_KV), 2 * D * D, dt), D, at(P(KV), D, dt), 2 * D, f32(P(B_IN)) + 2 * D, nullptr, M, D, D, dt, s));
-    RUN(svol_attn_fwd(P(QC), D, P(KV), 2 * D, at(P(KV), D, dt), 2 * D, P(OA), D, f32(P(LSE)), f32(P(KBIAS)), d.B, d.H, d.N, d.L, dh,
-                      attn_scale(dh), attn_premul(dh, dt), P(ATTN_WS), d.ws_bytes, dt, s));
     const void* oq = P(OA);
-    if (mixed) {
-        RUN(svol_cast(P(OA), dt, P(OAQ), qdt, R * D, s));
+    if (fuse) {
+        RUN(svol_attn_fwd_o32(P(QC), D, P(KV), 2 * D, at(P(KV), D, dt), 2 * D, P(OA), D, f32(P(OAQ)), f32(P(LSE)), f32(P(KBIAS)), d.B, d.H,
+                              d.N, d.L, dh, attn_scale(dh), attn_premul(dh, dt), P(ATTN_WS), d.ws_bytes, dt, s));
         oq = P(OAQ);
+    } else {
+        RUN(svol_attn_fwd(P(QC), D, P(KV), 2 * D, at(P(KV), D, dt), 2 * D, P(OA), D, f32(P(LSE)), f32(P(KBIAS)), d.B, d.H, d.N, d.L, dh,
+                          attn_scale(dh), attn_premul(dh, dt), P(ATTN_WS), d.ws_bytes, dt, s));
+        if (mixed) {
+            RUN(svol_cast(P(OA), dt, P(OAQ), qdt, R * D, s));
+            oq = P(OAQ);
+        }
     }
     RUN(nt_res(oq, D, P(W_O), D, P(S5), P(B_O), P(O32), R, D, D, qdt, s));
     RUN(svol_layernorm_fwd(P(S5), xf, f32(P(G5)), f32(P(BT5)), f32(P(Y5_32)), P(Y5), nullptr, nullptr, 0, f32(P(MEAN5)), f32(P(RSTD5)), R,
@@ -351,6 +363,8 @@
                            0.f, 0, nullptr, qdt, s));
     return SVOL_OK;
 }
+
+int svol_query_cross_fwd(const int64_t* dims, void* const* p, void* s) { return svol_query_cross_fwd_phase(dims, p, 0, s); }
 
 int svol_query_cross_bwd(const int64_t* dims, void* const* p, void* s) {
     if (!dims || !p) return SVOL_E_INVALID;
@@ -368,14 +382,21 @@
     RUN(svol_layernorm_bwd(f32(P(DS32_6)), P(DY5), nullptr, P(S5), xf, f32(P(G5)), f32(P(MEAN5)), f32(P(RSTD5)), f32(P(DO32)), P(G5D),
                            f32(P(DG5)), f32(P(DBT5)), f32(P(DB_O)), R, D, 0.f, 0, nullptr, qdt, s));
     RUN(nt(P(G5D), D, P(W_O_T), D, P(DOAQ), D, nullptr, nullptr, R, D, D, qdt, s));
-    const void* d_o = P(DOAQ);
-    if (mixed) {
-        RUN(svol_cast(P(DOAQ), qdt, P(DOA), dt, R * D, s));
-        d_o = P(DOA);
-    }
-    RUN(svol_attn_bwd(P(QC), D, P(KV), 2 * D, at(P(KV), D, dt), 2 * D, P(OA), D, d_o, D, f32(P(LSE)), f32(P(DELTA)), f32(P(KBIAS)), P(DQC), D,
-                      P(DKV), 2 * D, at(P(DKV), D, dt), 2 * D, d.B, d.H, d.N, d.L, dh, attn_scale(dh), attn_premul(dh, dt), P(ATTN_WS),
-                      d.ws_bytes, dt, s));
+    const bool fuse = mixed && qdt == SVOL_F32;
+    if (fuse) {
+        RUN(svol_attn_bwd_x32(P(QC), D, P(KV), 2 * D, at(P(KV), D, dt), 2 * D, P(OA), D, f32(P(DOAQ)), P(DOA), D, f32(P(LSE)), f32(P(DELTA)),
+                              f32(P(KBIAS)), P(DQC), D, f32(P(DQ)), P(DKV), 2 * D, at(P(DKV), D, dt), 2 * D, d.B, d.H, d.N, d.L, dh,
+                              attn_scale(dh), attn_premul(dh, dt), P(ATTN_WS), d.ws_bytes, dt, s));
+    } else {
+        const void* d_o = P(DOAQ);
+        if (mixed) {
+            RUN(svol_cast(P(DOAQ), qdt, P(DOA), dt, R * D, s));
+            d_o = P(DOA);
+        }
+        RUN(svol_attn_bwd(P(QC), D, P(KV), 2 * D, at(P(KV), D, dt), 2 * D, P(OA), D, d_o, D, f32(P(LSE)), f32(P(DELTA)), f32(P(KBIAS)), P(DQC),
+                          D, P(DKV), 2 * D, at(P(DKV), D, dt), 2 * D, d.B, d.H, d.N, d.L, dh, attn_scale(dh), attn_premul(dh, dt), P(ATTN_WS),
+                          d.ws_bytes, dt, s));
+    }
     if (P(DMPOS)) {
         RUN(nt(P(DKV), 2 * D, at(P(W_KV_T), D, dt), 3 * D, P(DMPOS), D, nullptr, nullptr, M, D, D, dt, s));
         RUN(nt(at(P(DKV), D, dt), 2 * D, at(P(W_KV_T), 2 * D, dt), 3 * D, P(DMV), D, nullptr, nullptr, M, D, D, dt, s));
@@ -383,7 +404,9 @@
         RUN(nt(P(DKV), 2 * D, at(P(W_KV_T), D, dt), 3 * D, P(DMV), D, nullptr, nullptr, M, D, 2 * D, dt, s));
     }
     const void* dq = P(DQC);
-    if (mixed) {
+    if (fuse) {
+        dq = P(DQ);
+    } else if (mixed) {
         RUN(svol_cast(P(DQC), dt, P(DQ), qdt, R * D, s));
         dq = P(DQ);
     }
diff --git a/svol_amd/csrc/common.h b/svol_amd/csrc/common.h
--- a/svol_amd/csrc/common.h
+++ b/svol_amd/csrc/common.h
@@ -38,6 +38,7 @@
 #define svol_gemm_n256_bf16 svol_gemm_n256_f16
 #define svol_attn_fwd_bf16_launch svol_attn_fwd_f16_launch
 #define svol_attn_bwd_bf16_launch svol_attn_bwd_f16_launch
+#define svol_attn_x32_fused_bf16 svol_attn_x32_fused_f16
 #define svol_attn_ws_floats_bf16 svol_attn_ws_floats_f16
 #define svol_attn_sp_image_bytes_bf16 svol_attn_sp_image_bytes_f16
 #define svol_attn_sp_zero_bf16_launch svol_attn_sp_zero_f16_launch
diff --git a/svol_amd/csrc/gemm.hip b/svol_amd/csrc/gemm.hip
--- a/svol_amd/csrc/gemm.hip
+++ b/svol_amd/csrc/gemm.hip
@@ -412,6 +412,7 @@
     const float* bias; const float* colscale; float* pre; const float* res; const float* aux; float* colsum;
     int64_t lda, ldb, ldc, ldp, ldr, ldaux;
     int M, N, K, act, epi;
+    void* c16; int64_t ldc16; int dt16;
 };
 constexpr int SKF_T = 32, SKF_LD = SKF_T + 4;
 
@@ -516,6 +517,25 @@
         }
     }
     if (mv) *reinterpret_cast<f32x4*>(p.C + (int64_t)m * p.ldc + n0) = v;
+    if (mv && p.c16) {
+#pragma unroll
+        for (int e = 0; e < 4; ++e) {
+            float t = v[e];
+            asm volatile("" : "+v"(t));
+            v[e] = t;
+        }
+        if (p.dt16 == SVOL_BF16) {
+            bf16x4 o;
+#pragma unroll
+            for (int e = 0; e < 4; ++e) o[e] = (bf16_t)v[e];
+            *reinterpret_cast<bf16x4*>(static_cast<bf16_t*>(p.c16) + (int64_t)m * p.ldc16 + n0) = o;
+        } else {
+            f16x4 o;
+#pragma unroll
+            for (int e = 0; e < 4; ++e) o[e] = (f16_t)v[e];
+            *reinterpret_cast<f16x4*>(static_cast<f16_t*>(p.c16) + (int64_t)m * p.ldc16 + n0) = o;
+        }
+    }
 }
 
 inline bool skinny_f32_ok(const GemmCall& c) {
@@ -602,7 +622,7 @@
     }
     if (dtype == SVOL_F32 && !A2 && skinny_f32_ok(c)) {
         SkArgs q{(const float*)c.A, (const float*)c.B, (float*)c.C, c.bias, c.colscale, (float*)c.pre, (const float*)c.res, (const float*)c.aux,
-                 c.colsum, c.lda, c.ldb, c.ldc, c.ldp, c.ldr, c.ldaux, (int)M, (int)N, (int)K, c.act, c.epi};
+                 c.colsum, c.lda, c.ldb, c.ldc, c.ldp, c.ldr, c.ldaux, (int)M, (int)N, (int)K, c.act, c.epi, nullptr, 0, 0};
         hipLaunchKernelGGL(gemm_nt_f32_skinny, dim3((unsigned)(N / 32), (unsigned)((M + 31) / 32)), dim3(256), 0, c.stream, q);
         SVOL_CHECK_LAUNCH();
         return SVOL_OK;
@@ -634,6 +654,28 @@
     c.bias = bias; c.colscale = colscale; c.act = act; c.out_f32 = out_f32; c.M = M; c.N = N; c.K = K; c.kwrap = K;
     c.stream = reinterpret_cast<hipStream_t>(stream);
     return gemm_nt_dispatch(c, A2, n_split, dtype);
+}
+
+int svol_gemm_nt_f32_c16(const void* A, int64_t lda, const void* B, int64_t ldb, void* C, int64_t ldc, const float* bias,
+                         const float* colscale, void* C16, int64_t ldc16, int dtype16, int64_t M, int64_t N, int64_t K, void* stream) {
+    if (!C16 || !svol_is16(dtype16)) return SVOL_E_INVALID;
+    GemmCall c{};
+    c.A = A; c.lda = lda; c.B = B; c.ldb = ldb; c.C = C; c.ldc = ldc; c.bias = bias; c.colscale = colscale;
+    c.M = M; c.N = N; c.K = K; c.kwrap = K;
+    c.stream = reinterpret_cast<hipStream_t>(stream);
+    const bool fused = A && B && C && M > 0 && N > 0 && K > 0 && skinny_f32_ok(c) && ldc16 % 4 == 0 && ldc16 >= N &&
+                       (reinterpret_cast<uintptr_t>(C16) & 7u) == 0;
+    if (!fused) {
+        if (const int rc = gemm_nt_dispatch(c, nullptr, 0, SVOL_F32)) return rc;
+        if (M == 0 || N == 0) return SVOL_OK;
+        if (ldc != N || ldc16 != N) return SVOL_E_UNSUPPORTED;
+        return svol_cast(C, SVOL_F32, C16, dtype16, M * N, stream);
+    }
+    SkArgs q{(const float*)A, (const float*)B, (float*)C, bias, colscale, nullptr, nullptr, nullptr, nullptr, lda, ldb, ldc, 0, 0, 0,
+             (int)M, (int)N, (int)K, SVOL_ACT_NONE, 0, C16, ldc16, dtype16};
+    hipLaunchKernelGGL(gemm_nt_f32_skinny, dim3((unsigned)(N / 32), (unsigned)((M + 31) / 32)), dim3(256), 0, c.stream, q);
+    SVOL_CHECK_LAUNCH();
+    return SVOL_OK;
 }
 
 int svol_gemm_nt_split(const void* A, int64_t lda, const void* W_hilo, int64_t ldw, void* C, int64_t ldc, const float* bias,
diff --git a/svol_amd/csrc/norm.hip b/svol_amd/csrc/norm.hip
--- a/svol_amd/csrc/norm.hip
+++ b/svol_amd/csrc/norm.hip
@@ -4,7 +4,23 @@
 
 constexpr int LN_MAX_PASSES = 4;
 
-template <typename T, typename TX, int NP>
+template <typename T, typename TX, bool RX> struct LnRow { typedef Vec4<TX> type; };
+template <typename T> struct LnRow<T, float, true> { typedef Vec4<T> type; };
+template <typename T, typename TX, bool RX>
+__device__ __forceinline__ typename LnRow<T, TX, RX>::type ln_row(const Vec4<TX>& t) {
+    if constexpr (RX) {
+        Vec4<T> r;
+#pragma unroll
+        for (int e = 0; e < 4; ++e) r.set(e, t.get(e));
+        uint64_t bits = __builtin_bit_cast(uint64_t, r.v);
+        asm("" : "+v"(bits));
+        r.v = __builtin_bit_cast(decltype(r.v), bits);
+        return r;
+    } else {
+        return t;
+    }
+}
+template <typename T, typename TX, int NP, bool RX = false>
 __global__ __launch_bounds__(256) void ln_fwd_kernel(const TX* __restrict__ x, const float* __restrict__ gamma,
                                                      const float* __restrict__ beta, float* __restrict__ y32,
                                                      T* __restrict__ y, T* __restrict__ ypos, const T* __restrict__ pos,
@@ -19,18 +35,25 @@
     float v[NP][4];
     float s = 0.f;
     const T* pr = pos ? pos + (row % pos_rows) * D : nullptr;
-    Vec4<TX> t[NP];
+    typename LnRow<T, TX, RX>::type t[NP];
+    Vec4<TX> traw[RX ? NP : 1];
     Vec4<T> pv[NP];
     Vec4<float> gv[NP], bv[NP];
 #pragma unroll
     for (int j = 0; j < NP; ++j) {
         const int c = (lane + 64 * j) * 4;
         if (c < D) {
-            t[j].load(xr + c);
+            if constexpr (RX) traw[j].load(xr + c);
+            else t[j].load(xr + c);
             if (pr) pv[j].load(pr + c);
             gv[j].load(gamma + c);
             bv[j].load(beta + c);
         }
+    }
+    if constexpr (RX) {
+#pragma unroll
+        for (int j = 0; j < NP; ++j)
+            if ((lane + 64 * j) * 4 < D) t[j] = ln_row<T, TX, RX>(traw[j]);
     }
 #pragma unroll
     for (int j = 0; j < NP; ++j) {
@@ -74,7 +97,7 @@
     }
 }
 
-template <typename T, typename TX, int NP>
+template <typename T, typename TX, int NP, bool RX = false>
 __global__ __launch_bounds__(256) void ln_bwd_kernel(const float* __restrict__ dy32, const T* __restrict__ dy,
                                                      const T* __restrict__ dy2, const TX* __restrict__ x,
                                                      const float* __restrict__ gamma, const float* __restrict__ mean,
@@ -121,11 +144,12 @@
         for (int j = 0; j < NP; ++j) {
             const int c = (lane + 64 * j) * 4;
             if (c < D) {
+                const auto xr = ln_row<T, TX, RX>(cur.xv[j]);
 #pragma unroll
                 for (int e = 0; e < 4; ++e) {
                     float d = (dy32 ? cur.a32[j].get(e) : 0.f) + (dy ? cur.a[j].get(e) : 0.f) + (dy2 ? cur.b[j].get(e) : 0.f);
                     if (p > 0.f) d *= dropout_scale(seed, (uint64_t)row, (uint32_t)(c + e), p, inv_keep);
-                    const float h = (cur.xv[j].get(e) - mu) * rs;
+                    const float h = (xr.get(e) - mu) * rs;
                     xh[j][e] = h;
                     dg[j][e] += d * h;
                     db[j][e] += d;
@@ -271,11 +295,11 @@
 }
 }
 
-extern "C" {
-
-int svol_layernorm_fwd(const void* x, int x_f32, const float* gamma, const float* beta, float* y32, void* y,
+static int ln_fwd_impl(const void* x, int x_mode, const float* gamma, const float* beta, float* y32, void* y,
                        void* ypos, const void* pos, int64_t pos_rows, float* mean, float* rstd, int64_t M, int64_t D,
                        float dropout_p, uint64_t seed, const int64_t* seed_offset_dev, int dtype, void* stream) {
+    const int x_f32 = x_mode != 0;
+    if (x_mode == 2 && (!svol_is16(dtype) || !aligned16(x))) return SVOL_E_INVALID;
     if (!x || !gamma || !beta || (!y && !y32) || !mean || !rstd || M < 0 || D <= 0) return SVOL_E_INVALID;
     if (!aligned16(gamma) || !aligned16(beta)) return SVOL_E_INVALID;
     if ((ypos != nullptr) != (pos != nullptr)) return SVOL_E_INVALID;
@@ -287,30 +311,34 @@
     const float inv_keep = 1.f / (1.f - dropout_p);
     const unsigned grid = (unsigned)((M + 3) / 4);
     hipStream_t s = reinterpret_cast<hipStream_t>(stream);
-#define SVOL_LNF(TT, TXX, NPP)                                                                                              \
-    hipLaunchKernelGGL((ln_fwd_kernel<TT, TXX, NPP>), dim3(grid), dim3(256), 0, s, (const TXX*)x, gamma, beta, y32, (TT*)y,      \
+#define SVOL_LNF(TT, TXX, NPP, RXX)                                                                                         \
+    hipLaunchKernelGGL((ln_fwd_kernel<TT, TXX, NPP, RXX>), dim3(grid), dim3(256), 0, s, (const TXX*)x, gamma, beta, y32, (TT*)y, \
                        (TT*)ypos, (const TT*)pos, pos_rows, mean, rstd, M, (int)D, dropout_p, inv_keep, seed, seed_offset_dev)
-#define SVOL_LNF_NP(TT, TXX)                     \
-    do {                                         \
-        if (D <= 256) SVOL_LNF(TT, TXX, 1);      \
-        else if (D <= 512) SVOL_LNF(TT, TXX, 2); \
-        else SVOL_LNF(TT, TXX, 4);               \
+#define SVOL_LNF_NP(TT, TXX, RXX)                     \
+    do {                                              \
+        if (D <= 256) SVOL_LNF(TT, TXX, 1, RXX);      \
+        else if (D <= 512) SVOL_LNF(TT, TXX, 2, RXX); \
+        else SVOL_LNF(TT, TXX, 4, RXX);               \
     } while (0)
-    if (dtype == SVOL_BF16 && x_f32) SVOL_LNF_NP(bf16_t, float);
-    else if (dtype == SVOL_BF16) SVOL_LNF_NP(bf16_t, bf16_t);
-    else if (dtype == SVOL_F16 && x_f32) SVOL_LNF_NP(f16_t, float);
-    else if (dtype == SVOL_F16) SVOL_LNF_NP(f16_t, f16_t);
-    else SVOL_LNF_NP(float, float);
+    if (dtype == SVOL_BF16 && x_mode == 2) SVOL_LNF_NP(bf16_t, float, true);
+    else if (dtype == SVOL_F16 && x_mode == 2) SVOL_LNF_NP(f16_t, float, true);
+    else if (dtype == SVOL_BF16 && x_f32) SVOL_LNF_NP(bf16_t, float, false);
+    else if (dtype == SVOL_BF16) SVOL_LNF_NP(bf16_t, bf16_t, false);
+    else if (dtype == SVOL_F16 && x_f32) SVOL_LNF_NP(f16_t, float, false);
+    else if (dtype == SVOL_F16) SVOL_LNF_NP(f16_t, f16_t, false);
+    else SVOL_LNF_NP(float, float, false);
 #undef SVOL_LNF_NP
 #undef SVOL_LNF
     SVOL_CHECK_LAUNCH();
     return SVOL_OK;
 }
 
-int svol_layernorm_bwd(const float* dy32, const void* dy, const void* dy2, const void* x, int x_f32, const float* gamma,
+static int ln_bwd_impl(const float* dy32, const void* dy, const void* dy2, const void* x, int x_mode, const float* gamma,
                        const float* mean, const float* rstd, float* dx32, void* dx, float* dgamma, float* dbeta,
                        float* dx_colsum, int64_t M, int64_t D, float dropout_p, uint64_t seed, const int64_t* seed_offset_dev,
                        int dtype, void* stream) {
+    const int x_f32 = x_mode != 0;
+    if (x_mode == 2 && (!svol_is16(dtype) || !aligned16(x))) return SVOL_E_INVALID;
     if ((!dy32 && !dy && !dy2) || !x || !gamma || !mean || !rstd || (!dx && !dx32) || !dgamma || !dbeta || M < 0 || D <= 0)
         return SVOL_E_INVALID;
     if (D % 4 || D > LN_MAX_PASSES * 256) return SVOL_E_UNSUPPORTED;
@@ -326,21 +354,23 @@
     const bool det_mode = svol_deterministic();
     DetScratch det(det_mode ? (size_t)grid * 3 * (size_t)D : 0, s);
     if (det_mode && !det.p) return SVOL_E_LAUNCH;
-#define SVOL_LNB(TT, TXX, NPP)                                                                                                      \
-    hipLaunchKernelGGL((ln_bwd_kernel<TT, TXX, NPP>), dim3(grid), dim3(256), 0, s, dy32, (const TT*)dy, (const TT*)dy2, (const TXX*)x, \
+#define SVOL_LNB(TT, TXX, NPP, RXX)                                                                                                      \
+    hipLaunchKernelGGL((ln_bwd_kernel<TT, TXX, NPP, RXX>), dim3(grid), dim3(256), 0, s, dy32, (const TT*)dy, (const TT*)dy2, (const TXX*)x, \
                        gamma, mean, rstd, dx32, (TT*)dx, dgamma, dbeta, dx_colsum, M, (int)D, dropout_p, inv_keep, seed,              \
                        seed_offset_dev, (int)rpw, det.p)
-#define SVOL_LNB_NP(TT, TXX)                  \
-    do {                                      \
-        if (D <= 256) SVOL_LNB(TT, TXX, 1);   \
-        else if (D <= 512) SVOL_LNB(TT, TXX, 2); \
-        else SVOL_LNB(TT, TXX, 4);            \
+#define SVOL_LNB_NP(TT, TXX, RXX)                  \
+    do {                                           \
+        if (D <= 256) SVOL_LNB(TT, TXX, 1, RXX);   \
+        else if (D <= 512) SVOL_LNB(TT, TXX, 2, RXX); \
+        else SVOL_LNB(TT, TXX, 4, RXX);            \
     } while (0)
-    if (dtype == SVOL_BF16 && x_f32) SVOL_LNB_NP(bf16_t, float);
-    else if (dtype == SVOL_BF16) SVOL_LNB_NP(bf16_t, bf16_t);
-    else if (dtype == SVOL_F16 && x_f32) SVOL_LNB_NP(f16_t, float);
-    else if (dtype == SVOL_F16) SVOL_LNB_NP(f16_t, f16_t);
-    else SVOL_LNB_NP(float, float);
+    if (dtype == SVOL_BF16 && x_mode == 2) SVOL_LNB_NP(bf16_t, float, true);
+    else if (dtype == SVOL_F16 && x_mode == 2) SVOL_LNB_NP(f16_t, float, true);
+    else if (dtype == SVOL_BF16 && x_f32) SVOL_LNB_NP(bf16_t, float, false);
+    else if (dtype == SVOL_BF16) SVOL_LNB_NP(bf16_t, bf16_t, false);
+    else if (dtype == SVOL_F16 && x_f32) SVOL_LNB_NP(f16_t, float, false);
+    else if (dtype == SVOL_F16) SVOL_LNB_NP(f16_t, f16_t, false);
+    else SVOL_LNB_NP(float, float, false);
 #undef SVOL_LNB_NP
 #undef SVOL_LNB
     if (det_mode) {
@@ -350,6 +380,33 @@
     }
     SVOL_CHECK_LAUNCH();
     return SVOL_OK;
+}
+
+extern "C" {
+
+int svol_layernorm_fwd(const void* x, int x_f32, const float* gamma, const float* beta, float* y32, void* y,
+                       void* ypos, const void* pos, int64_t pos_rows, float* mean, float* rstd, int64_t M, int64_t D,
+                       float dropout_p, uint64_t seed, const int64_t* seed_offset_dev, int dtype, void* stream) {
+    return ln_fwd_impl(x, x_f32 ? 1 : 0, gamma, beta, y32, y, ypos, pos, pos_rows, mean, rstd, M, D, dropout_p, seed, seed_offset_dev,
+                       dtype, stream);
+}
+int svol_layernorm_fwd_x32r(const float* x32, const float* gamma, const float* beta, float* y32, void* y, void* ypos, const void* pos,
+                            int64_t pos_rows, float* mean, float* rstd, int64_t M, int64_t D, float dropout_p, uint64_t seed,
+                            const int64_t* seed_offset_dev, int dtype, void* stream) {
+    return ln_fwd_impl(x32, 2, gamma, beta, y32, y, ypos, pos, pos_rows, mean, rstd, M, D, dropout_p, seed, seed_offset_dev, dtype, stream);
+}
+int svol_layernorm_bwd(const float* dy32, const void* dy, const void* dy2, const void* x, int x_f32, const float* gamma,
+                       const float* mean, const float* rstd, float* dx32, void* dx, float* dgamma, float* dbeta,
+                       float* dx_colsum, int64_t M, int64_t D, float dropout_p, uint64_t seed, const int64_t* seed_offset_dev,
+                       int dtype, void* stream) {
+    return ln_bwd_impl(dy32, dy, dy2, x, x_f32 ? 1 : 0, gamma, mean, rstd, dx32, dx, dgamma, dbeta, dx_colsum, M, D, dropout_p, seed,
+                       seed_offset_dev, dtype, stream);
+}
+int svol_layernorm_bwd_x32r(const float* dy32, const void* dy, const void* dy2, const float* x32, const float* gamma, const float* mean,
+                            const float* rstd, float* dx32, void* dx, float* dgamma, float* dbeta, float* dx_colsum, int64_t M, int64_t D,
+                            float dropout_p, uint64_t seed, const int64_t* seed_offset_dev, int dtype, void* stream) {
+    return ln_bwd_impl(dy32, dy, dy2, x32, 2, gamma, mean, rstd, dx32, dx, dgamma, dbeta, dx_colsum, M, D, dropout_p, seed,
+                       seed_offset_dev, dtype, stream);
 }
 
 int svol_dropout_sd(const void* x, void* y, int64_t n, int64_t row_len, float p, uint64_t seed, const int64_t* seed_step_dev, int dtype,
diff --git a/svol_amd/layers.py b/svol_amd/layers.py
--- a/svol_amd/layers.py
+++ b/svol_amd/layers.py
@@ -42,6 +42,32 @@
 
 def layer_norm(x, gamma, beta, p=0.0, seed=0, seed_dev=None):
     return LayerNormFn.apply(x, gamma, beta, p, seed, seed_dev)
+
+
+class LayerNormX32Fn(torch.autograd.Function):
+
+    @staticmethod
+    def forward(ctx, x32, gamma, beta, p, seed, seed_dev, dtype):
+        shp = x32.shape
+        x2 = x32.reshape(-1, shp[-1]).contiguous()
+        _, y, _, mean, rstd = layernorm_fwd(x2, gamma, beta, dtype, None, p, seed, seed_dev=seed_dev, x32r=True)
+        ctx.save_for_backward(x2, gamma, mean, rstd, seed_dev)
+        ctx.p, ctx.seed, ctx.shp, ctx.dtype = p, seed, shp, dtype
+        ctx.sinks = (claim(gamma, ctx.needs_input_grad[1]), claim(beta, ctx.needs_input_grad[2]))
+        return y.view(shp)
+
+    @staticmethod
+    def backward(ctx, dy):
+        x2, gamma, mean, rstd, seed_dev = ctx.saved_tensors
+        sg, sb = ctx.sinks
+        _, dx, dg, db = layernorm_bwd(None, dy, None, x2, gamma, mean, rstd, ctx.dtype, ctx.p, ctx.seed, seed_dev=seed_dev,
+                                      dg_out=sink_view(sg), db_out=sink_view(sb), x32r=True)
+        dx32 = cast(dx, torch.float32).view(ctx.shp) if ctx.needs_input_grad[0] else None
+        return dx32, unless_sunk(sg, dg), unless_sunk(sb, db), None, None, None, None
+
+
+def layer_norm_x32(x32, gamma, beta, dtype, p=0.0, seed=0, seed_dev=None):
+    return LayerNormX32Fn.apply(x32, gamma, beta, p, seed, seed_dev, dtype)
 
 
 class LinearFn(torch.autograd.Function):
diff --git a/svol_amd/modeling/cross_modal_transformer.py b/svol_amd/modeling/cross_modal_transformer.py
--- a/svol_amd/modeling/cross_modal_transformer.py
+++ b/svol_amd/modeling/cross_modal_transformer.py
@@ -184,12 +184,15 @@
         o32, o, opos = out
         return layers.self_attn_ln(o32, o, opos, *mha(self.token_self_attn), *n(self.norm4), qpos, self.nhead)
 
-    def query_cross(self, out, m, mpos, qpos, kbias):
+    def query_cross_q(self, out, qpos, dt):
+        return blocks.query_cross_q(self, out, dt, qpos.dtype) if blocks.ENABLED else None
+
+    def query_cross(self, out, m, mpos, qpos, kbias, pre=None):
         n = lambda m_: (m_.weight, m_.bias)
         mha = lambda m_: (m_.in_proj_weight, m_.in_proj_bias, m_.out_proj.weight, m_.out_proj.bias)
         mlp = lambda m_: (m_.fc1.weight, m_.fc1.bias, m_.fc2.weight, m_.fc2.bias)
         if blocks.ENABLED:
-            return blocks.query_cross(self, out, m, mpos, kbias, qpos, m.dtype, qpos.dtype)
+            return blocks.query_cross(self, out, m, mpos, kbias, qpos, m.dtype, qpos.dtype, pre)
         o32, o, opos = out
         o32, o = layers.cross_attn_ln(o32, o, opos, mpos, m, *mha(self.content_token_cross_attn), *n(self.norm5), None, self.nhead,
                                    kbias)
@@ -240,6 +243,7 @@
         for li, (layer, u) in enumerate(zip(self.layers, us)):
             with torch.cuda.stream(side):
                 out_sa = layer.query_self(out, qpos, vid_pos.dtype)
+                pre = layer.query_cross_q(out_sa, qpos, vid_pos.dtype)
             if blocks.ENABLED and blocks.GATE_SCORES_FUSE and li + 1 < len(us):
                 m32, m, mpos, sc = layer.video_half(mem32, src_skch32, vid_pos, u, us[li + 1], sc)
             elif sc is not None:
@@ -250,7 +254,7 @@
             m.record_stream(side)
             mpos.record_stream(side)
             with torch.cuda.stream(side):
-                out = layer.query_cross(out_sa, m, mpos, qpos, kbias)
+                out = layer.query_cross(out_sa, m, mpos, qpos, kbias, pre)
                 outputs.append(out[0])
             mem32 = m32
         main.wait_stream(side)
diff --git a/svol_amd/modeling/svanet.py b/svol_amd/modeling/svanet.py
--- a/svol_amd/modeling/svanet.py
+++ b/svol_amd/modeling/svanet.py
@@ -42,9 +42,15 @@
             self.LayerNorm = nn.LayerNorm(in_hsz)
         self.net = nn.Sequential(nn.Dropout(dropout), nn.Linear(in_hsz, out_hsz))
 
-    def forward(self, x, seed=0, out_f32=False, seed_dev=None):
+    def takes_x32(self, x, dt):
+        return (self.layer_norm and dt in (torch.bfloat16, torch.float16) and x.dtype == torch.float32 and x.shape[-1] % 4 == 0
+                and x.shape[-1] <= 1024)
+
+    def forward(self, x, seed=0, out_f32=False, seed_dev=None, x32_dt=None):
         p = self.p if self.training else 0.0
-        if self.layer_norm:
+        if x32_dt is not None:
+            x = layers.layer_norm_x32(x, self.LayerNorm.weight, self.LayerNorm.bias, x32_dt, p, seed, seed_dev)
+        elif self.layer_norm:
             x = layers.layer_norm(x, self.LayerNorm.weight, self.LayerNorm.bias, p, seed, seed_dev)
         elif p > 0.0:
             raise NotImplementedError('dropout without LayerNorm is not on the reference path')
@@ -86,12 +92,18 @@
         self.base_seed = 1
         self.step_dev = None
 
-    def _proj(self, seq, x, salt):
+    def _proj(self, seq, x, salt, x32_dt=None):
         n = len(seq)
         for j, layer in enumerate(seq):
             x = layer(x, seed=(self.base_seed << 32) + (self._step << 8) + salt * 16 + j, out_f32=(j == n - 1),
-                      seed_dev=self.step_dev)
+                      seed_dev=self.step_dev, x32_dt=x32_dt if j == 0 else None)
         return x
+
+    def _proj_video(self, src_video, dt):
+        xv = src_video.float()
+        if self.input_video_proj[0].takes_x32(xv, dt):
+            return self._proj(self.input_video_proj, xv, 0, x32_dt=dt)
+        return self._proj(self.input_video_proj, layers.cast_ag(xv, dt), 0)
 
     def forward(self, src_sketch, src_sketch_mask, src_video, src_video_mask):
         if not src_video.is_cuda:
@@ -120,16 +132,15 @@
             with torch.cuda.stream(side):
                 params.weights.new_epoch()
                 casts_done = side.record_event()
-            xv = layers.cast_ag(src_video.float(), dt)
             with torch.cuda.stream(side):
                 pos_video, skch, kbias, us = mask_side(True)
             main.wait_event(casts_done)
-            vid = self._proj(self.input_video_proj, xv, 0)
+            vid = self._proj_video(src_video, dt)
             main.wait_stream(side)
             for t in [pos_video, skch, kbias] + list(us or []):
                 t.record_stream(main)
         else:
-            vid = self._proj(self.input_video_proj, layers.cast_ag(src_video.float(), dt), 0)
+            vid = self._proj_video(src_video, dt)
             pos_video, skch, kbias, us = mask_side(False)
         hs = (self.transformer(vid, skch, kbias, pos_video, self.query_embed.weight, us) if us is not None else
               self.transformer(vid, skch, kbias, pos_video, self.query_embed.weight))
diff --git a/svol_amd/ops.py b/svol_amd/ops.py
--- a/svol_amd/ops.py
+++ b/svol_amd/ops.py
@@ -212,11 +212,11 @@
     return out
 
 
-def layernorm_fwd(x, gamma, beta, dtype, pos=None, p=0.0, seed=0, want32=False, want_t=True, seed_dev=None):
+def layernorm_fwd(x, gamma, beta, dtype, pos=None, p=0.0, seed=0, want32=False, want_t=True, seed_dev=None, x32r=False):
     x = x.contiguous()
     M, D = x.shape
     x_f32 = 1 if (x.dtype == torch.float32 and dtype != torch.float32) else 0
-    assert x.dtype in (dtype, torch.float32)
+    assert x.dtype in (dtype, torch.float32) and (not x32r or x_f32)
     y32 = torch.empty((M, D), dtype=torch.float32, device=x.device) if want32 else None
     y = torch.empty((M, D), dtype=dtype, device=x.device) if want_t else None
     ypos = torch.empty((M, D), dtype=dtype, device=x.device) if pos is not None else None
@@ -225,15 +225,17 @@
     if pos is not None:
         pos = pos.contiguous()
         assert pos.dtype == dtype and pos.shape[-1] == D
-    rc = _lib.lib().svol_layernorm_fwd(_ptr(x), x_f32, _ptr(gamma), _ptr(beta), _ptr(y32), _ptr(y), _ptr(ypos),
-                                       _ptr(pos), pos.numel() // D if pos is not None else 0, _ptr(mean), _ptr(rstd),
-                                       M, D, float(p), int(seed), _ptr(seed_dev), _DT[dtype], _stream())
-    _lib.check(rc, 'svol_layernorm_fwd')
+    tail = (_ptr(gamma), _ptr(beta), _ptr(y32), _ptr(y), _ptr(ypos), _ptr(pos), pos.numel() // D if pos is not None else 0, _ptr(mean),
+            _ptr(rstd), M, D, float(p), int(seed), _ptr(seed_dev), _DT[dtype], _stream())
+    if x32r:
+        _lib.check(_lib.lib().svol_layernorm_fwd_x32r(_ptr(x), *tail), 'svol_layernorm_fwd_x32r')
+    else:
+        _lib.check(_lib.lib().svol_layernorm_fwd(_ptr(x), x_f32, *tail), 'svol_layernorm_fwd')
     return y32, y, ypos, mean, rstd
 
 
 def layernorm_bwd(dy32, dy, dy2, x, gamma, mean, rstd, dtype, p=0.0, seed=0, want32=False, want_t=True,
-                  want_colsum=False, seed_dev=None, dg_out=None, db_out=None, cs_out=None):
+                  want_colsum=False, seed_dev=None, dg_out=None, db_out=None, cs_out=None, x32r=False):
     M, D = x.shape
     x_f32 = 1 if (x.dtype == torch.float32 and dtype != torch.float32) else 0
     cont = lambda t: None if t is None else t.reshape(M, D).contiguous()
@@ -248,10 +250,13 @@
         dg = red[0] if dg is None else dg
         db = red[1] if db is None else db
         cs = (red[2] if cs is None else cs) if want_colsum else None
-    rc = _lib.lib().svol_layernorm_bwd(_ptr(dy32), _ptr(dy), _ptr(dy2), _ptr(x), x_f32, _ptr(gamma), _ptr(mean),
-                                       _ptr(rstd), _ptr(dx32), _ptr(dx), _ptr(dg), _ptr(db), _ptr(cs), M, D, float(p),
-                                       int(seed), _ptr(seed_dev), _DT[dtype], _stream())
-    _lib.check(rc, 'svol_layernorm_bwd')
+    tail = (_ptr(gamma), _ptr(mean), _ptr(rstd), _ptr(dx32), _ptr(dx), _ptr(dg), _ptr(db), _ptr(cs), M, D, float(p), int(seed),
+            _ptr(seed_dev), _DT[dtype], _stream())
+    if x32r:
+        assert x_f32 and x.is_contiguous()
+        _lib.check(_lib.lib().svol_layernorm_bwd_x32r(_ptr(dy32), _ptr(dy), _ptr(dy2), _ptr(x), *tail), 'svol_layernorm_bwd_x32r')
+    else:
+        _lib.check(_lib.lib().svol_layernorm_bwd(_ptr(dy32), _ptr(dy), _ptr(dy2), _ptr(x), x_f32, *tail), 'svol_layernorm_bwd')
     if want_colsum:
         return dx32, dx, dg, db, cs
     return dx32, dx, dg, db
```

Result: no change. 15040 (-0.1%).
